# noahares/raxtax

Measured on AMD Instinct MI355X. Metric: classified queries/sec (whole node), higher is better.
Workload: dtype u32 bit-planes + f64

## Files before the change

### include/raxtax_hip.h

```cpp
#ifndef RAXTAX_HIP_H
#define RAXTAX_HIP_H

#include <stddef.h>
#include <stdint.h>

#ifdef __cplusplus
extern "C" {
#endif

#define RTX_ABI_VERSION 6
#define RTX_NUM_KMERS 65536u
#define RTX_MAX_DEPTH 32u

#define RTX_OK 0
#define RTX_ERR_INVALID (-1)
#define RTX_ERR_HIP (-2)
#define RTX_ERR_NO_DEVICE (-3)
#define RTX_ERR_OOM (-4)
#define RTX_ERR_PARSE (-5)
#define RTX_ERR_DEPTH (-6)
#define RTX_ERR_STATE (-7)
#define RTX_ERR_TOO_LONG (-8)
#define RTX_ERR_SENDER (-9)
#define RTX_RETRY_CHUNK 1
// ... 76 lines not shown
                                    uint32_t n_nodes, const uint32_t *node_begin, const uint32_t *node_end,
                                    const uint32_t *node_first_child, const uint32_t *node_n_children,
                                    const uint8_t *node_type, rtx_index **out);
int rtx_index_create_from_tree(int device, const rtx_tree *tree, rtx_index **out);
void rtx_index_destroy(rtx_index *index);
uint64_t rtx_index_num_refs(const rtx_index *index);
uint64_t rtx_index_device_bytes(const rtx_index *index);
uint64_t rtx_index_workspace_bytes(const rtx_index *index);
int rtx_index_workspace_parts(const rtx_index *index, uint64_t out[9]);
int rtx_index_set_batch(rtx_index *index, uint32_t sub_batch);
#define RTX_OPT_SUB_BATCH 1
#define RTX_OPT_PROB_MODE 2
#define RTX_OPT_STAGE_TIMING 6
#define RTX_OPT_DEBUG_TAPS 14
#define RTX_OPT_DEVICE_EXACT 15
#define RTX_OPT_CLUSTER 7
#define RTX_OPT_PACKED_COUNTS 8
#define RTX_OPT_HIT_PAIR 11
#define RTX_OPT_TILE_SKIP 10
#define RTX_OPT_LOCATOR 12
#define RTX_OPT_TILE_PRUNE 13
#define RTX_OPT_FINE_BOUNDS 17
#define RTX_OPT_RECORDS 18
#define RTX_OPT_OVERLAP 19
#define RTX_OPT_MIN_SUB_BATCHES 20
#define RTX_OPT_TWO_LEVEL_BOUNDS 21
#define RTX_OPT_PRUNE_SELF_SAMPLE 22
#define RTX_OPT_RUN_AHEAD 23
#define RTX_OPT_DEVICE_TEXT 24
#define RTX_OPT_STRAND 25
#define RTX_OPT_NEAREST 26
#define RTX_NO_REF 0xFFFFFFFFu
#define RTX_OPT_IDENTITY 28
#define RTX_NO_DIST 0xFFFFFFFFu
#define RTX_IDENTITY_MAX_QUERY 4096u
#define RTX_OPT_DEREP 27
int rtx_index_set_option(rtx_index *index, int option, uint64_t value);

int rtx_index_self_sample(rtx_index *index, const uint8_t *seq_bytes, const uint64_t *seq_off, uint64_t n_refs, uint32_t n_sample, double *live_fraction);
int rtx_index_prune_verdict(const rtx_index *index, int *pruning, double *live_fraction);
int rtx_index_run_ahead_stats(const rtx_index *index, uint64_t *enqueued_ahead, uint64_t *abandoned);
#define RTX_DEFAULT_SEGMENT_CLASSES 1
#define RTX_DEFAULT_EXACT_HASH_MASK 2
#define RTX_DEFAULT_DEREP_HASH_MASK 3
int rtx_set_default_option(int option, uint64_t value);

typedef struct {
    uint32_t n_queries;
    uint64_t n_rows;
    const uint32_t *t;
    const uint8_t *status;
    const double *global_signal;
    const uint64_t *row_begin;
    const uint32_t *row_count;
    const uint32_t *row_lineage;
    const uint32_t *row_node;
    const uint32_t *row_depth;
    const double *row_conf;
    const double *row_local_signal;
    uint32_t row_conf_stride;
    const uint8_t *row_depth_u8;
    const uint8_t *row_conf_hundredths;
} rtx_result_view;

int rtx_batch_prefetch(rtx_index *index, uint64_t n_queries, const uint8_t *bases, const uint64_t *base_off,
                       const uint32_t *exact_ids, const uint64_t *exact_off);
// ... 431 lines not shown
int rtx_shard_prob(rtx_index *index, uint32_t sub_batch_idx);
int rtx_shard_walk(rtx_index *index, uint32_t sub_batch_idx, const double *prefix_global );
int rtx_shard_info(const rtx_index *index, uint64_t *ref_lo, uint64_t *ref_hi, uint32_t *n_bnd_global,
                   uint32_t *n_bnd_local, uint32_t *first_bnd);
int rtx_device_buffer(rtx_index *index, int which, void **device_ptr, uint64_t *row_stride_elems);
#define RTX_BUF_COUNTS 3
#define RTX_BUF_BEST 4
int rtx_shard_buffer(rtx_index *index, uint32_t sub_batch_idx, int which, void **device_ptr, uint64_t *row_stride_elems);
int rtx_shard_rehist(rtx_index *index, uint32_t sub_batch_idx);
int rtx_index_stream(rtx_index *index, void **hip_stream);

#define RTX_STAGE_KMER_EXTRACT 0
#define RTX_STAGE_HIT_COUNT 1
#define RTX_STAGE_PROB_TABLE 2
#define RTX_STAGE_TAXON_PREFIX 3
#define RTX_STAGE_LINEAGE_WALK 4
#define RTX_STAGE_TILE_BOUNDS 5
#define RTX_STAGE_TILE_PRUNE 6
#define RTX_STAGE_EXACT_MATCH 7
#define RTX_STAGE_ORDER 8
#define RTX_STAGE_PAIR_UNION 9
#define RTX_NUM_STAGES 10
int rtx_batch_stage_times(rtx_index *index, float ms[RTX_NUM_STAGES], uint32_t launches[RTX_NUM_STAGES]);
int rtx_batch_work(rtx_index *index, uint64_t *sum_hits, uint64_t *sum_query_bytes,
                   uint64_t *bitmap_bytes_read);
int rtx_batch_work_split(rtx_index *index, uint64_t *live_bytes, uint64_t *bounds_bytes);
int rtx_batch_prob_work(rtx_index *index, uint64_t *sum_grid_points, uint64_t *sum_distinct_counts);

int rtx_debug_kmers(rtx_index *index, uint64_t query, uint16_t *kmers , uint32_t *t);
int rtx_debug_hit_counts(rtx_index *index, uint64_t query, uint16_t *counts );
int rtx_debug_prob_table(rtx_index *index, uint64_t query, double *table_over_z , double *z);
int rtx_debug_probs(rtx_index *index, uint64_t query, double *probs );
int rtx_debug_tile_bounds(rtx_index *index, uint64_t query, uint16_t *tile_ub );
int rtx_debug_order(rtx_index *index, uint32_t *perm );
int rtx_batch_sub_batch(const rtx_index *index, uint32_t *sub_batch, uint32_t *n_sub_batches);
int rtx_batch_last_sub_batch(const rtx_index *index, uint64_t *first, uint32_t *n);
int rtx_batch_classes(const rtx_index *index, uint32_t *n_classes, uint64_t out[20]);
int rtx_debug_prune_stats(rtx_index *index, uint64_t *out );
int rtx_debug_pruned_prob_table(rtx_index *index, uint64_t query, double *table_over_z , double *z, uint32_t *threshold);
int rtx_debug_run_counts(rtx_index *index, uint64_t query, uint16_t *counts , uint8_t *tile_live ,
                         uint32_t *hist , uint32_t *threshold, uint32_t *i1);
int rtx_debug_run_mode(rtx_index *index, uint64_t query, uint32_t *n_segments);
int rtx_debug_prune_detail(rtx_index *index, uint64_t query, uint32_t *out );
int rtx_debug_evaluate(rtx_index *index, const double *probs , rtx_result_view *out);
int rtx_debug_evaluate_mode(rtx_index *index, const double *probs , uint32_t mode, rtx_result_view *out, uint32_t *table_in_lds);
int rtx_debug_ln_factorial(uint32_t n, double *out );
int rtx_debug_prob_hist(rtx_index *index, uint32_t n_q, const uint32_t *t , const uint32_t *hist , uint32_t hstride,
                        uint64_t n_refs, uint32_t kernel, const uint16_t *prune_thr , const uint16_t *prune_i1 ,
                        double *table_over_z , double *z , double *gs , uint8_t *status ,
                        uint32_t *ndist );

int64_t rtx_format_query(const rtx_tree *tree, const rtx_result_view *res, uint64_t q,
                         const char *label, const uint8_t *seq, uint64_t seq_len,
                         const uint32_t *exact_ids, uint64_t n_exact, uint32_t flags, char *out_buf,
                         uint64_t out_cap, char *tsv_buf, uint64_t tsv_cap, int64_t *tsv_len);

int64_t rtx_result_pack(const rtx_result_view *res, uint8_t *buf, uint64_t cap);

#define RTX_NEED_BASE 1024
int64_t rtx_records_format(const rtx_tree *tree, const uint8_t *records, uint64_t n_bytes, const char *const *labels,
                           const uint32_t *exact_one, uint32_t flags, char *out, uint64_t cap, uint64_t *line_off, uint32_t threads);

typedef int (*rtx_sender_fn)(void *ctx, const char *label, const char *out_lines, const char *tsv_lines);
int rtx_raxtax(rtx_index *index, const rtx_tree *tree, uint64_t n_queries, const char *const *labels,
               const uint8_t *bases, const uint64_t *base_off, int skip_exact_matches, int raw_confidence,
               uint64_t chunk_size, rtx_sender_fn sender, void *sender_ctx, int tsv);
// ... 65 lines not shown
```

### raxtax_amd/_lib.py

```python
from __future__ import annotations

import ctypes as C
from pathlib import Path

import numpy as np

PKG = Path(__file__).resolve().parent
import os as _os

LIB_PATH = Path(_os.environ.get("RTX_LIB_PATH") or PKG / "libraxtax_hip.so")

RTX_MAX_DEPTH = 32
RTX_NUM_KMERS = 65536
RTX_OK = 0
RTX_ERR_INVALID, RTX_ERR_HIP, RTX_ERR_NO_DEVICE, RTX_ERR_OOM = -1, -2, -3, -4
RTX_ERR_PARSE, RTX_ERR_DEPTH, RTX_ERR_STATE, RTX_ERR_TOO_LONG = -5, -6, -7, -8
RTX_SKIP_EXACT_MATCHES = 1
RTX_RAW_CONFIDENCE = 2
RTX_TEXT_TSV = 4
RTX_Q_OK, RTX_Q_NO_KMERS, RTX_Q_ALL_KMERS = 0, 1, 2
RTX_OPT_DEREP = 27
RTX_DEFAULT_DEREP_HASH_MASK = 3
RTX_DEFAULT_TALLY_HASH_MASK = 4
RTX_DEFAULT_OTU_HASH_MASK = 5
RTX_DEFAULT_CHIMERA_SLICE = 6
RTX_DEFAULT_UNOISE_SLICE = 8
RTX_UNOISE_MAX_DIFFS = 16
RTX_UNOISE_ZOTU, RTX_UNOISE_ABSORBED, RTX_UNOISE_LEFT, RTX_UNOISE_LONG = 0, 1, 2, 3
RTX_OTU_MAX_LEN = 4096
RTX_LIN_UNCLASSIFIABLE, RTX_LIN_UNCLASSIFIED, RTX_LIN_CLASSIFIED = 0, 1, 2
STAGES = ("kmer_extract", "hit_count", "prob_table", "taxon_prefix", "lineage_walk", "tile_bounds", "tile_prune", "exact_match", "order", "pair_union")

RTX_TRIM_5P, RTX_TRIM_3P = 0, 1
RTX_TRIM_MAX_PATTERNS, RTX_TRIM_MAX_PATTERN, RTX_TRIM_MAX_WINDOW, RTX_TRIM_NO_PATTERN = 8, 64, 256, 0xFF

RTX_DEMUX_MAX_TAGS, RTX_DEMUX_MAX_TAG, RTX_DEMUX_MAX_OFFSET, RTX_DEMUX_MAX_MISMATCHES = 1024, 32, 15, 8
RTX_DEMUX_NO_TAG, RTX_DEMUX_NONE = 0xFFFF, 0xFFFFFFFF
RTX_PROFILE_MAX_SAMPLE_COUNTERS = 1 << 28
RTX_DEMUX_NAMES = ("ok", "no_tag5", "no_tag3", "ambiguous", "unknown_pair")

RTX_QUAL_MAX_READ, RTX_QUAL_TABLE = 1 << 20, 94
RTX_QC_NAMES = ("bad_quality", "short_for_trunc_len", "too_short", "too_long", "too_many_n", "max_ee", "max_ee_rate")

RTX_SCREEN_K, RTX_SCREEN_NONE, RTX_SCREEN_MAX_READ, RTX_SCREEN_MAX_BASES, RTX_SCREEN_CONTAMINANT = 16, 0xFFFFFFFF, 1 << 20, 1 << 26, 1

RTX_MERGE_MAX_READ, RTX_MERGE_MISMATCH_COST = 1024, 5
RTX_MG_NAMES = ("bad_quality", "too_long", "too_short", "no_overlap")

RTX_CHIMERA_MAX_QUERY, RTX_CHIMERA_MAX_SEGMENTS, RTX_CHIMERA_DEFAULT_SEGMENTS, RTX_CHIMERA_DEFAULT_MINDELTA = 4096, 32, 16, 24
RTX_CHIM_OK, RTX_CHIM_NO_KMER, RTX_CHIM_TOO_LONG = 0, 1, 2
RTX_DENOVO_NO_PARENT = 3
RTX_DENOVO_DEFAULT_ABSKEW = 2
RTX_DENOVO_DEFAULT_MAX_PARENTS = 262144
# ... 186 lines not shown
    "rtx_index_num_refs": (C.c_uint64, [C.c_void_p]),
    "rtx_index_device_bytes": (C.c_uint64, [C.c_void_p]),
    "rtx_index_workspace_bytes": (C.c_uint64, [C.c_void_p]),
    "rtx_index_workspace_parts": (C.c_int, [C.c_void_p, u64p]),
    "rtx_index_set_batch": (C.c_int, [C.c_void_p, C.c_uint32]),
    "rtx_set_default_option": (C.c_int, [C.c_int, C.c_uint64]),
    "rtx_index_set_option": (C.c_int, [C.c_void_p, C.c_int, C.c_uint64]),
    "rtx_index_self_sample": (C.c_int, [C.c_void_p, C.c_void_p, C.c_void_p, C.c_uint64, C.c_uint32, C.POINTER(C.c_double)]),
    "rtx_index_prune_verdict": (C.c_int, [C.c_void_p, C.POINTER(C.c_int), C.POINTER(C.c_double)]),
    "rtx_index_run_ahead_stats": (C.c_int, [C.c_void_p, C.POINTER(C.c_uint64), C.POINTER(C.c_uint64)]),
    "rtx_classify_batch": (C.c_int, [C.c_void_p, C.c_uint64, u8p, u64p, u32p, u64p, C.c_uint32,
                                     C.POINTER(ResultView)]),
    "rtx_index_has_exact_lookup": (C.c_int, [C.c_void_p]),
    "rtx_batch_exact_matches": (C.c_int, [C.c_void_p, C.POINTER(u64p), C.POINTER(u32p)]),
    "rtx_batch_upload": (C.c_int, [C.c_void_p, C.c_uint64, u8p, u64p, u32p, u64p]),
    "rtx_batch_run": (C.c_int, [C.c_void_p, C.c_uint32]),
    "rtx_batch_sync": (C.c_int, [C.c_void_p]),
    "rtx_batch_download": (C.c_int, [C.c_void_p, C.POINTER(ResultView)]),
    "rtx_batch_download_then_run": (C.c_int, [C.c_void_p, C.POINTER(ResultView), C.c_uint32]),
    "rtx_index_text_setup": (C.c_int, [C.c_void_p, C.c_void_p, C.c_uint32]),
    "rtx_batch_prefetch_labels": (C.c_int, [C.c_void_p, C.c_uint64, C.POINTER(C.c_char_p)]),
    "rtx_batch_text": (C.c_int, [C.c_void_p, C.POINTER(TextView)]),
    "rtx_batch_stage_times": (C.c_int, [C.c_void_p, f32p, u32p]),
    "rtx_batch_work": (C.c_int, [C.c_void_p, u64p, u64p, u64p]),
    "rtx_batch_prob_work": (C.c_int, [C.c_void_p, u64p, u64p]),
    "rtx_batch_work_split": (C.c_int, [C.c_void_p, u64p, u64p]),
    "rtx_debug_kmers": (C.c_int, [C.c_void_p, C.c_uint64, u16p, u32p]),
    "rtx_debug_hit_counts": (C.c_int, [C.c_void_p, C.c_uint64, u16p]),
    "rtx_debug_prob_table": (C.c_int, [C.c_void_p, C.c_uint64, f64p, f64p]),
    "rtx_debug_pruned_prob_table": (C.c_int, [C.c_void_p, C.c_uint64, f64p, f64p, u32p]),
    "rtx_debug_probs": (C.c_int, [C.c_void_p, C.c_uint64, f64p]),
    "rtx_debug_order": (C.c_int, [C.c_void_p, u32p]),
    "rtx_debug_tile_bounds": (C.c_int, [C.c_void_p, C.c_uint64, u16p]),
    "rtx_debug_prune_stats": (C.c_int, [C.c_void_p, u64p]),
    "rtx_debug_run_counts": (C.c_int, [C.c_void_p, C.c_uint64, u16p, u8p, u32p, u32p, u32p]),
    "rtx_debug_run_mode": (C.c_int, [C.c_void_p, C.c_uint64, u32p]),
    "rtx_batch_last_sub_batch": (C.c_int, [C.c_void_p, u64p, u32p]),
    "rtx_batch_classes": (C.c_int, [C.c_void_p, u32p, u64p]),
    "rtx_debug_prune_detail": (C.c_int, [C.c_void_p, C.c_uint64, u32p]),
    "rtx_debug_evaluate": (C.c_int, [C.c_void_p, f64p, C.POINTER(ResultView)]),
    "rtx_debug_evaluate_mode": (C.c_int, [C.c_void_p, f64p, C.c_uint32, C.POINTER(ResultView), u32p]),
    "rtx_debug_ln_factorial": (C.c_int, [C.c_uint32, f64p]),
    "rtx_debug_prob_hist": (C.c_int, [C.c_void_p, C.c_uint32, u32p, u32p, C.c_uint32, C.c_uint64, C.c_uint32, u16p, u16p, f64p, f64p, f64p, u8p, u32p]),
    "rtx_result_pack": (C.c_int64, [C.POINTER(ResultView), u8p, C.c_uint64]),
    "rtx_records_format": (C.c_int64, [C.c_void_p, u8p, C.c_uint64, C.POINTER(C.c_char_p), u32p, C.c_uint32, C.c_char_p, C.c_uint64, u64p, C.c_uint32]),
    "rtx_format_query": (C.c_int64, [C.c_void_p, C.POINTER(ResultView), C.c_uint64, C.c_char_p, u8p, C.c_uint64,
                                     u32p, C.c_uint64, C.c_uint32, C.c_char_p, C.c_uint64, C.c_char_p, C.c_uint64,
                                     C.POINTER(C.c_int64)]),
    "rtx_raxtax": (C.c_int, None),
    "rtx_raxtax_multi": (C.c_int, None),
    "rtx_raxtax_multi_ex": (C.c_int, None),
    "rtx_batch_strands": (C.c_int, [C.c_void_p, C.POINTER(u8p), C.POINTER(u32p)]),
    "rtx_revcomp": (C.c_int, [u8p, C.c_uint64, u8p]),
    "rtx_raxtax_multi_ex2": (C.c_int, None),
    "rtx_batch_nearest": (C.c_int, [C.c_void_p, C.POINTER(u32p), C.POINTER(u32p)]),
    "rtx_batch_nearest_time": (C.c_int, [C.c_void_p, C.POINTER(C.c_float), C.POINTER(C.c_uint32)]),
    "rtx_raxtax_multi_ex3": (C.c_int, None),
    "rtx_batch_identity": (C.c_int, [C.c_void_p, C.POINTER(u32p), C.POINTER(u32p)]),
    "rtx_batch_identity_time": (C.c_int, [C.c_void_p, C.POINTER(C.c_float), C.POINTER(C.c_uint32)]),
    "rtx_semiglobal_distance": (C.c_int, [u8p, C.c_uint64, u8p, C.c_uint64, C.POINTER(C.c_uint32)]),
    "rtx_index_profile_begin": (C.c_int, [C.c_void_p, C.c_uint32, C.c_uint32]),
    "rtx_index_profile_read": (C.c_int, [C.c_void_p, C.POINTER(ProfileView)]),
    "rtx_index_profile_reset": (C.c_int, [C.c_void_p]),
    "rtx_index_profile_end": (C.c_int, [C.c_void_p]),
    "rtx_index_profile_time": (C.c_int, [C.c_void_p, C.POINTER(C.c_float), C.POINTER(C.c_uint32)]),
    "rtx_profile_merge": (C.c_int, [C.POINTER(C.POINTER(ProfileView)), C.c_uint32, u64p, u64p, u64p, u64p]),
# ... 168 lines not shown
```

### raxtax_amd/api.py

```python
from __future__ import annotations

import ctypes as C
from dataclasses import dataclass
from typing import Callable, List, Optional, Sequence, Tuple

import numpy as np

from . import _lib
from ._lib import (RTX_MAX_DEPTH, RTX_RAW_CONFIDENCE, RTX_SKIP_EXACT_MATCHES, NodesView, ResultView, RtxError, check,
                   f32p, f64p, ptr, u8p, u16p, u32p, u64p)


def _flatten(seqs: Sequence[np.ndarray]) -> Tuple[np.ndarray, np.ndarray]:
    off = np.zeros(len(seqs) + 1, dtype=np.uint64)
    if len(seqs):
        off[1:] = np.cumsum([len(s) for s in seqs], dtype=np.uint64)
    flat = np.zeros(max(int(off[-1]), 1), dtype=np.uint8)
    for i, s in enumerate(seqs):
        flat[int(off[i]):int(off[i + 1])] = np.asarray(s, dtype=np.uint8)
    return flat, off


class Tree:

# ... 263 lines not shown
    check(_lib.load().rtx_sample_profile_merge(arr, len(views), ptr(direct if direct.size else np.zeros(1, np.uint64), u64p), ptr(totals, u64p)))
    return SampleProfile(profiles[0].cutoff, profiles[0].flags, direct, totals)


def sample_table_text(tree: Tree, names: Sequence[str], profile: SampleProfile) -> str:
    lib = _lib.load()
    direct = np.ascontiguousarray(profile.direct, dtype=np.uint64)
    totals = np.ascontiguousarray(profile.totals, dtype=np.uint64)
    if len(names) != direct.shape[0] or totals.shape != (direct.shape[0], 4):
        raise ValueError(f"sample_table_text: {len(names)} names, counters of shape {direct.shape} and {totals.shape}")
    cn = (C.c_char_p * max(len(names), 1))(*[n.encode() for n in names])
    args = [tree._h, len(names), cn, ptr(direct if direct.size else np.zeros(1, np.uint64), u64p), ptr(totals, u64p), int(profile.cutoff)]
    n = check(lib.rtx_sample_table_format(*args, None, 0))
    buf = C.create_string_buffer(max(n, 1))
    check(lib.rtx_sample_table_format(*args, buf, n))
    return buf.raw[:n].decode()


DEFAULT_SEGMENT_CLASSES = 1


class Index:

    identity_on = False
    nearest_on = False

    def __init__(self, tree: Tree, device: int = 0, sub_batch: int = 0, prob_mode: int = 0,
                 stage_timing: bool = False, cluster: Optional[bool] = None, segment_classes=None,
                 packed_counts: Optional[bool] = None,
                 tile_skip: Optional[bool] = None, hit_pair=None, locator: Optional[bool] = None, tile_prune: Optional[bool] = None,
                 debug_taps: bool = False, device_exact: Optional[bool] = None, fine_bounds: Optional[bool] = None,
                 records: Optional[int] = None, overlap: Optional[bool] = None, two_level: Optional[int] = None,
                 prune_self_sample: Optional[bool] = None, device_text: bool = False, strand: str = "plus",
                 nearest: bool = False, derep: bool = False, identity: bool = False, primers=None, quality=None, chimera=None, tags=None, contaminants=None, tally=None):
        self._lib = _lib.load()
        self.tree = tree
        self._tally = None
        if segment_classes is None:
            segment_classes = DEFAULT_SEGMENT_CLASSES
        check(self._lib.rtx_set_default_option(1, int(segment_classes)))
        h = C.c_void_p()
        check(self._lib.rtx_index_create_from_tree(device, tree._h, C.byref(h)))
        self._h = h
        self.n_refs = self._lib.rtx_index_num_refs(self._h)
        if sub_batch:
            check(self._lib.rtx_index_set_batch(self._h, sub_batch))
        if prob_mode:
            check(self._lib.rtx_index_set_option(self._h, 2, prob_mode))
        if stage_timing:
            check(self._lib.rtx_index_set_option(self._h, 6, 1))
        if cluster is not None:
            check(self._lib.rtx_index_set_option(self._h, 7, int(cluster)))
        if packed_counts is not None:
            check(self._lib.rtx_index_set_option(self._h, 8, int(packed_counts)))
        if tile_skip is not None:
            check(self._lib.rtx_index_set_option(self._h, 10, int(tile_skip)))
        if hit_pair is not None:
            check(self._lib.rtx_index_set_option(self._h, 11, int(hit_pair)))
        if locator is not None:
            check(self._lib.rtx_index_set_option(self._h, 12, int(locator)))
        if tile_prune is not None:
            check(self._lib.rtx_index_set_option(self._h, 13, int(tile_prune)))
            if tile_prune and prune_self_sample is None:
                check(self._lib.rtx_index_set_option(self._h, 22, 0))
        if debug_taps:
            check(self._lib.rtx_index_set_option(self._h, 14, 1))
        if device_exact is not None:
# ... 3 lines not shown
        if fine_bounds is not None:
            check(self._lib.rtx_index_set_option(self._h, 17, int(fine_bounds)))
        if records is not None:
            check(self._lib.rtx_index_set_option(self._h, 18, int(records)))
        if overlap is not None:
            check(self._lib.rtx_index_set_option(self._h, 19, int(overlap)))
        if two_level is not None:
            check(self._lib.rtx_index_set_option(self._h, 21, int(two_level)))
        if prune_self_sample is not None:
            check(self._lib.rtx_index_set_option(self._h, 22, int(prune_self_sample)))
        if strand not in ("plus", "both"):
            raise ValueError(f"strand must be 'plus' or 'both', not {strand!r}")
        self.strand = strand
        if strand == "both":
            check(self._lib.rtx_index_set_option(self._h, 25, 1))
        self.nearest_on = bool(nearest) or bool(identity)
        if self.nearest_on:
            check(self._lib.rtx_index_set_option(self._h, 26, 1))
        self.identity_on = bool(identity)
        if identity:
            check(self._lib.rtx_index_set_option(self._h, 28, 1))
        if derep:
            check(self._lib.rtx_index_set_option(self._h, _lib.RTX_OPT_DEREP, 1))
        if primers:
            self.set_primers(primers)
        if tags:
            self.set_tags(*tags)
        if quality is not None:
            self.set_quality(quality)
        if chimera is not None:
            self.set_chimera(ChimeraParams() if chimera is True else chimera)
        if contaminants is not None:
            self.set_screen(*(contaminants if isinstance(contaminants, tuple) else (contaminants,)))
        if tally is not None:
            self.set_tally(tally)
        self._view = ResultView()
        self._keep = None

    def set_tally(self, tally) -> None:
        check(self._lib.rtx_index_set_tally(self._h, tally._h if tally is not None else None))
        self._tally = tally

    @property
    def tally(self):
        return self._tally if self._lib.rtx_index_tally(self._h) else None

    def set_screen(self, sset, params=None) -> None:
        if sset is None:
            check(self._lib.rtx_index_set_screen(self._h, None, None))
        else:
            check(self._lib.rtx_index_set_screen(self._h, sset._h, C.byref((params or ScreenParams())._c())))

    @property
    def screen(self):
        c, on, fp = _lib.ScreenParams(), C.c_int(), C.c_uint64()
        check(self._lib.rtx_index_screen(self._h, C.byref(c), C.byref(on), C.byref(fp)))
        return (ScreenParams(c.min_hits, c.min_pct), int(fp.value)) if on.value else None

    def set_quality(self, params) -> None:
        check(self._lib.rtx_index_set_quality(self._h, C.byref(params._c()) if params is not None else None))

    @property
    def quality(self):
        c, on = _lib.QualParams(), C.c_int()
        check(self._lib.rtx_index_quality(self._h, C.byref(c), C.byref(on)))
        return QualParams._of(c) if on.value else None

    def set_chimera(self, params) -> None:
        check(self._lib.rtx_index_set_chimera(self._h, C.byref(params._c()) if params is not None else None))

# ... 275 lines not shown
        return out

    def debug_prune_detail(self, q: int) -> dict:
        out = np.zeros(72, dtype=np.uint32)
        check(self._lib.rtx_debug_prune_detail(self._h, q, ptr(out, u32p)))
        return dict(block=int(out[0]), M=int(out[1]), threshold=int(out[2]), i1=int(out[3]), largest_bound=int(out[4]), t=int(out[5]),
                    block_counts=out[8:72].copy())

    def debug_probs(self, q: int) -> np.ndarray:
        out = np.zeros(self.n_refs, dtype=np.float64)
        check(self._lib.rtx_debug_probs(self._h, q, ptr(out, f64p)))
        return out

    def sub_batch_size(self) -> int:
        b, n = C.c_uint32(), C.c_uint32()
        check(self._lib.rtx_batch_sub_batch(self._h, C.byref(b), C.byref(n)))
        return int(b.value)

    def last_sub_batch(self):
        first, n = C.c_uint64(), C.c_uint32()
        check(self._lib.rtx_batch_last_sub_batch(self._h, C.byref(first), C.byref(n)))
        return int(first.value), int(n.value)

    def batch_classes(self) -> list:
        n = C.c_uint32()
        out = np.zeros(20, dtype=np.uint64)
        check(self._lib.rtx_batch_classes(self._h, C.byref(n), ptr(out, u64p)))
        res = []
        for c in range(int(n.value)):
            f = int(out[4 * c + 3])
            res.append(dict(queries=int(out[4 * c]), longest=int(out[4 * c + 1]), sub_batch=int(out[4 * c + 2]), planes=f & 0xFF, tables=bool(f >> 8 & 1),
                            pair=bool(f >> 9 & 1), prune=bool(f >> 10 & 1), records=bool(f >> 11 & 1), global_memory_forms=bool(f >> 12 & 1)))
        return res

    def debug_order(self, n_queries: int) -> np.ndarray:
        out = np.zeros(n_queries, dtype=np.uint32)
        check(self._lib.rtx_debug_order(self._h, ptr(out, u32p)))
        return out

    def debug_prune_stats(self) -> dict:
        out = np.zeros(16, dtype=np.uint64)
        check(self._lib.rtx_debug_prune_stats(self._h, ptr(out, u64p)))
        pairs, nq = max(int(out[1]), 1), max(int(out[5]), 1)
        counted = int(out[12]) if int(out[11]) or int(out[12]) else int(out[0])
        return {"live_tiles_per_pair": counted / pairs, "live_tiles_per_pair_first_stage": int(out[0]) / pairs,
                "fine_blocks_per_pair": int(out[11]) / pairs, "fine_cleared_per_query": int(out[10]) / nq, "pairs": int(out[1]), "mean_best_hit_lower_bound": int(out[2]) / nq,
                "mean_threshold": int(out[3]) / nq, "mean_largest_tile_bound": int(out[4]) / nq, "bound_violations": int(out[6]), "live_tiles_per_query": int(out[7]) / nq,
                "tiles_above_threshold_per_query": int(out[8]) / max(int(out[9]), 1), "queries_with_threshold": int(out[9]),
                "record_queries": int(out[14]), "records_per_record_query": int(out[13]) / max(int(out[14]), 1), "record_slow_path_queries": int(out[15])}

    def debug_evaluate(self, probs, mode: int = 0) -> Result:
        probs = np.ascontiguousarray(probs, dtype=np.float64)
        assert len(probs) == self.n_refs
        in_lds = C.c_uint32()
        check(self._lib.rtx_debug_evaluate_mode(self._h, ptr(probs, f64p), mode, C.byref(self._view), C.byref(in_lds)))
        self.last_evaluate_table_in_lds = bool(in_lds.value)
        return Result(self._view)

    def debug_prob_hist(self, ts, hists, n_refs: int, kernel: int, thr=None, i1=None) -> dict:
        ts = np.ascontiguousarray(ts, dtype=np.uint32)
        hists = np.ascontiguousarray(hists, dtype=np.uint32)
        assert hists.ndim == 2 and hists.shape[0] == len(ts)
        n_q, hstride = hists.shape
        tz = np.zeros((n_q, hstride), dtype=np.float64)
        z = np.zeros(n_q, dtype=np.float64)
        gs = np.zeros(n_q, dtype=np.float64)
# ... 1275 lines not shown
```

### raxtax_amd/csrc/rtx_api_batch.hip

```cpp
#include "rtx_index.hpp"

#ifndef RTX_B2_HEAVY_PER_ATILE
#define RTX_B2_HEAVY_PER_ATILE 4u
#endif

namespace rtxi {

int bind(rtx_index *ix) {
    if (!ix) { set_error("null index handle"); return RTX_ERR_INVALID; }
    RTX_HIP(hipSetDevice(ix->device));
    return RTX_OK;
}

int ensure_events(rtx_index *ix, size_t count) {
    while (ix->events.size() < count) {
        hipEvent_t e;
        RTX_HIP(hipEventCreate(&e));
        ix->events.push_back(e);
    }
    return RTX_OK;
}


SubBatch sub_batch_of(rtx_index *ix, uint32_t sb, bool timed) {
// ... 55 lines not shown
    kp.list_len = ix->d_list_len.p;
    kp.row_len = ix->d_row_len.p;
    kp.zero_row = ix->n_rows;
    kp.kmers = sc.d_kmers.p;
    kp.kstride = k.kstride;
    kp.seginfo = ix->d_seginfo.p;
    kp.seg_stride = ix->seg_stride;
    kp.segcls = ix->d_segcls.p;
    kp.cls_stride = ix->cls_stride;
    kp.ntiles = ix->ntiles;
    kp.seg_dbits = ix->d_seg_dbits.p;
    kp.seg_sbits = ix->d_seg_sbits.p;
    kp.seg_sbase = ix->d_seg_sbase.p;
    kp.seg_blocks = ix->seg_blocks;
    kp.rows = sc.d_rows.p;
    kp.rstride = k.rstride;
    kp.dmask = sc.d_dmask.p;
    kp.srows = sc.d_srows.p;
    kp.nsparse = sc.d_nsparse.p;
    kp.t = sc.d_t.p;
    kp.nrows = sc.d_nrows.p;
    kp.hq = r.d_hq.p;
    kp.t_all = r.d_t_all.p;
    kp.nrows_all = r.d_nrows_all.p;
    kp.hist = sc.d_hist.p;
    kp.hstride = k.hstride;
    return kp;
}

static bool run_prunes(const rtx_index *ix, const rtx_index::BatchClass &k) { return k.prune && !ix->dbg_full_run; }
static bool on_records_path(const rtx_index *ix, const rtx_index::BatchClass &k, const rtx_index::Scratch &sc) { return run_prunes(ix, k) && k.rec && sc.d_rec.p != nullptr; }
static bool on_diet(const rtx_index *ix, const rtx_index::BatchClass &k, const rtx_index::Scratch &sc) { return on_records_path(ix, k, sc) && k.diet && sc.d_cnt_row.p != nullptr; }

static RecordRef record_ref(const rtx_index *ix, const rtx_index::Scratch &sc, const rtx_index::ResultSet &r) { return RecordRef{sc.d_rec_nslots.p, sc.d_rec_slots.p, sc.d_rec_cnt.p, sc.d_rec.p, ix->rec_slots(), ix->rec_seg_len, r.d_flags.p}; }
static ProbTables prob_tables(const rtx_index *ix) { return ProbTables{ix->d_tab_cmf.p, ix->d_tab_ratio.p, ix->d_tab_off.p, ix->d_tab_moff.p, ix->d_tab_ilo.p, ix->d_tab_sat.p, ix->tab_tmax}; }

int enqueue_kmer(rtx_index *ix, const SubBatch &b, hipStream_t s) {
    KmerParams kp = kmer_params(ix, b);
    kp.mode = run_prunes(ix, *b.cls) && ix->seg_blocks ? 1u : 0u;
    if (run_prunes(ix, *b.cls)) {
        rtx_index::Scratch &sc = ix->sc[b.set];
        const ItemsLayout items(b.nq, ix->ntiles);
        const FineItemsLayout fine(b.nq, ix->f_ntiles);
        if (sc.d_items.p) { kp.zero[0] = items.count(sc.d_items.p); kp.zero_n[0] = 9u; }
        if (sc.d_fine_items.p) { kp.zero[1] = fine.count(sc.d_fine_items.p); kp.zero_n[1] = 9u + ix->f_ntiles; }
        if (sc.d_cnt_cursor.p) { kp.zero[2] = sc.d_cnt_cursor.p; kp.zero_n[2] = 1u; }
    }
    if (b.timed_all) RTX_HIP(hipEventRecord(stage_event(ix, b, RTX_STAGE_KMER_EXTRACT, 0), s));
    launch_kmer_extract(s, kp, b.nq);
    if (b.timed_all) RTX_HIP(hipEventRecord(stage_event(ix, b, RTX_STAGE_KMER_EXTRACT, 1), s));
    return RTX_OK;
}

static HitParams hit_params(rtx_index *ix, const SubBatch &b, uint32_t flags) {
    rtx_index::Scratch &sc = ix->sc[b.set];
    rtx_index::ResultSet &r = ix->res();
    const rtx_index::BatchClass &k = *b.cls;
    HitParams hp{};
    hp.bitmap = ix->d_bitmap.p;
    hp.stride_bytes = ix->stride_bytes;
    hp.n_rows1 = ix->n_rows + 1;
    hp.n_refs = ix->n_refs;
    hp.ref_base = ix->ref_lo;
    hp.rows = sc.d_rows.p;
    hp.rstride = k.rstride;
    hp.dmask = sc.d_dmask.p;
    hp.nrows = sc.d_nrows.p;
    hp.zero_row = ix->n_rows;
    hp.srows = sc.d_srows.p;
    hp.nsparse = sc.d_nsparse.p;
    hp.segslots = ix->d_segslots.p;
    hp.ntiles = ix->ntiles;
    hp.t = sc.d_t.p;
    hp.counts = sc.d_counts.p;
    hp.counts_lo = ix->packs(k.planes) ? counts_lo(ix, sc) : nullptr;
    hp.counts_hi = ix->packs(k.planes) ? counts_hi(ix, k, sc) : nullptr;
    hp.npad = ix->npad;
    hp.hist = sc.d_hist.p;
    hp.hstride = k.hstride;
    hp.tile_max = sc.d_tilemax.p;
    hp.flags = flags;
    hp.q0 = b.q0;
    hp.perm = r.d_perm.p;
    hp.exact = ExactRef{ix->in[ix->cur_in].d_exact_ids.p, ix->in[ix->cur_in].d_exact_off.p, r.dev_exact ? r.d_exact_grp.p : nullptr, ix->d_em_goff.p, ix->d_em_gids.p};
    hp.nq = b.nq;
    hp.group_rows = k.pair ? ix->d_group_rows.p : nullptr;
    hp.group_base = b.sb * ix->groups_per_sub;
    hp.pair_urec = sc.d_urec.p;
    hp.pair_nu = sc.d_nu.p;
    hp.pair_ustride = 2u * k.rstride;
    return hp;
}

static HitParams bounds_params(const rtx_index *ix, const rtx_index::Scratch &sc, const HitParams &hp) {
    HitParams up = hp;
    up.bitmap = ix->d_ubitmap.p;
    up.stride_bytes = ix->u_stride_bytes;
    up.n_refs = ix->u_nblocks;
    up.dmask = nullptr;
    up.nsparse = nullptr;
    up.ntiles = ix->u_ntiles;
    up.counts = nullptr;
    up.counts_lo = nullptr;
    up.counts_hi = nullptr;
    up.hist = nullptr;
    up.tile_max = nullptr;
    up.bounds_tile_ub = sc.d_tile_ub.p;
    up.bounds_tile_stride = ix->ntiles;
    up.bounds_ntiles = ix->ntiles;
    up.bounds_best = sc.d_best_key.p;
    up.flags = 0;
    up.group_base = hp.group_base + ix->n_groups_run;
    return up;
}

static Bounds2Params bounds2_params(const rtx_index *ix, const rtx_index::Scratch &sc, const HitParams &up, bool heavy) {
    Bounds2Params bp{};
    bp.abitmap = ix->d_abitmap.p;
    bp.bbitmap = ix->d_bbitmap.p;
    bp.n_rows1 = ix->n_rows + 1;
    bp.n_atiles = ix->n_atiles;
    bp.ntiles = ix->ntiles;
    bp.zero_row = ix->n_rows;
    bp.pair_urec = sc.d_urec.p;
    bp.pair_nu = sc.d_nu.p;
    bp.pair_ustride = up.pair_ustride;
    bp.nq = up.nq;
    bp.t = sc.d_t.p;
    bp.tile_ub = sc.d_tile_ub.p;
    bp.tile_ub_stride = ix->ntiles;
    bp.best_key = sc.d_best_key.p;
    bp.delta_ct = ix->b2_delta[0];
    bp.delta_cm = ix->b2_delta[1];
    bp.delta_lo = ix->b2_delta[2];
    bp.delta_hi = ix->b2_delta[3];
    bp.group_rows = up.group_rows;
    bp.group_base = up.group_base;
    bp.heavy = heavy ? sc.d_heavy.p : nullptr;
    bp.heavy_max = std::max<uint32_t>(1u, std::min<uint32_t>(RTX_B2_HEAVY_PER_ATILE * ix->n_atiles, ix->n_btiles / 2u));
    return bp;
}

static PruneParams prune_params(rtx_index *ix, const SubBatch &b, uint32_t flags, int part, const ExactRef &exact) {
    rtx_index::Scratch &sc = ix->sc[b.set];
    const rtx_index::BatchClass &k = *b.cls;
    PruneParams pr{};
    pr.tile_ub = sc.d_tile_ub.p;
    pr.best_key = sc.d_best_key.p;
    pr.tile_ub_stride = ix->ntiles;
    pr.ntiles = ix->ntiles;
    pr.nq = b.nq;
    pr.n_refs = ix->n_refs;
    pr.n_total = ix->n_total;
    pr.ref_base = ix->ref_lo;
    pr.phase = (uint32_t)part;
    pr.best = part ? sc.d_best.p : nullptr;
    pr.bitmap = ix->d_bitmap.p;
    pr.cbitmap = part == 0 && (ix->two_level_used || (k.planes > kBounds2MaxPlanes && ix->two_level_opt && ix->n_refs == ix->n_total)) ? reinterpret_cast<const uint2 *>(ix->d_cbitmap.p) : nullptr;
    pr.n_rows1 = ix->n_rows + 1;
    pr.stride_bytes = ix->stride_bytes;
    pr.rows = sc.d_rows.p;
    pr.rstride = k.rstride;
    pr.nrows = sc.d_nrows.p;
    pr.t = sc.d_t.p;
    pr.flags = flags;
    pr.q0 = b.q0;
    pr.perm = ix->res().d_perm.p;
    pr.exact = exact;
    pr.lnfact = ix->d_lnfact.p;
    pr.inv = ix->d_inv.p;
    pr.nlf = std::min<uint32_t>(kLnFactLen, k.tmax + k.tmax / 2 + 2);
    pr.hist = sc.d_hist.p;
    pr.hstride = k.hstride;
    pr.live = sc.d_live.p;
    pr.live_words = LiveLayout{ix->ntiles}.words();
    pr.pair_live = ItemsLayout(b.nq, ix->ntiles).pair_live(sc.d_items.p);
    pr.thr_out = sc.d_prune_thr.p;
    pr.i1_out = sc.d_prune_i1.p;
    pr.stats = ix->d_prune_stats.p;
    pr.detail = ix->debug_taps && ix->d_prune_detail.n >= (size_t)b.nq * kPruneDetailWords ? ix->d_prune_detail.p : nullptr;
    return pr;
}
// ... 27 lines not shown
    HitParams hp = hit_params(ix, b, flags);
    const bool prune = run_prunes(ix, k);
    if (k.pair && part != 2) {
        if (b.timed_all) RTX_HIP(hipEventRecord(stage_event(ix, b, RTX_STAGE_PAIR_UNION, 0), s));
        launch_pair_union(s, sc.d_rows.p, sc.d_nrows.p, k.rstride, b.nq, sc.d_urec.p, sc.d_nu.p, 2u * k.rstride);
        if (b.timed_all) RTX_HIP(hipEventRecord(stage_event(ix, b, RTX_STAGE_PAIR_UNION, 1), s));
    }
    if (b.timed && !prune) RTX_HIP(hipEventRecord(stage_event(ix, b, RTX_STAGE_HIT_COUNT, 0), s));
    if (part != 0 && !prune) { set_error("internal: a split run without tile pruning"); return RTX_ERR_STATE; }
    if (prune) {
        if (part != 2) {
            const HitParams up = bounds_params(ix, sc, hp);
            if (b.timed) RTX_HIP(hipEventRecord(stage_event(ix, b, RTX_STAGE_TILE_BOUNDS, 0), s));
            ix->two_level_used = part == 0 && ix->two_level_opt && ix->d_abitmap.p && ix->d_bbitmap.p && ix->n_refs == ix->n_total && k.planes <= kBounds2MaxPlanes;
            if (ix->two_level_used) {
                const bool heavy_ok = sc.d_heavy.p && sc.d_heavy_items.p && sc.d_heavy_items.n >= HeavyItemsLayout(b.nq, ix->u_ntiles).total();
                launch_bounds2(s, bounds2_params(ix, sc, up, heavy_ok), b.nq, k.planes, up, ix->u_ntiles, heavy_ok ? sc.d_heavy_items.p : nullptr);
            } else {
                RTX_HIP(hipMemsetAsync(sc.d_best_key.p, 0, (size_t)b.nq * 4, s));
                launch_hit_count_pair_bounds(s, up, b.nq, ix->u_ntiles, k.planes);
            }
            if (b.timed) RTX_HIP(hipEventRecord(stage_event(ix, b, RTX_STAGE_TILE_BOUNDS, 1), s));
        }
        if (s_mid && s_mid != s && part == 0) {
            RTX_HIP(hipEventRecord(ix->ev_mid[b.sb], s));
            RTX_HIP(hipStreamWaitEvent(s_mid, ix->ev_mid[b.sb], 0));
            s = s_mid;
        }
        if (b.timed && part != 1) RTX_HIP(hipEventRecord(stage_event(ix, b, RTX_STAGE_TILE_PRUNE, 0), s));
        PruneParams pr = prune_params(ix, b, flags, part, hp.exact);
        const bool records = part == 0 && on_records_path(ix, k, sc), diet = part == 0 && on_diet(ix, k, sc);
        const RecordRef rr = record_ref(ix, sc, r);
        if (records) { pr.rec = rr; pr.rec_max_slots = rr.stride; }
        if (k.diet && !diet) { set_error("internal: the counts buffer is on its diet without the records path"); return RTX_ERR_STATE; }
        if (diet) {
            pr.cnt_row = sc.d_cnt_row.p;
            pr.cnt_cursor = sc.d_cnt_cursor.p;
            pr.cnt_cap = k.cnt_rows;
            pr.dense_q = sc.d_dense_q.p;
            pr.flags_out = r.d_flags.p;
            hp.cnt_row = sc.d_cnt_row.p;
        }
        launch_prune(s, pr, prob_tables(ix), b.nq);
        if (part == 1) { RTX_HIP(hipGetLastError()); return RTX_OK; }
        if (part == 0 && ix->fine_opt && ix->d_fbitmap.p && k.pair && sc.d_fine_items.p) {
            const FineItemsLayout fine(b.nq, ix->f_ntiles);
            uint32_t *const fi = sc.d_fine_items.p;
            launch_fine_bounds(s, fine_params(ix, sc, hp), b.nq, ix->f_ntiles, pr.pair_live, fine.cursors(fi), fine.items(fi), fine.count(fi), k.planes);
        }
        RTX_HIP(hipMemsetAsync(sc.d_tilemax.p, 0, (size_t)b.nq * ix->ntiles * 2, s));
        hp.live = sc.d_live.p;
        hp.live_words = pr.live_words;
        hp.prune_thr = sc.d_prune_thr.p;
        if (records) hp.rec = rr;
        if (k.pair) {
            const ItemsLayout items(b.nq, ix->ntiles);
            launch_live_items(s, sc.d_live.p, pr.live_words, b.nq, ix->ntiles, items.items(sc.d_items.p), items.count(sc.d_items.p),
                              ix->d_prune_stats.p ? ix->d_prune_stats.p + 2 * kPruneStatCopies * 8 : nullptr);
            hp.items = items.items(sc.d_items.p);
            hp.n_items = items.count(sc.d_items.p);
        }
        if (ix->seg_blocks) {
            KmerParams kp = kmer_params(ix, b);
            kp.mode = 2u;
            kp.live = sc.d_live.p;
            kp.live_words = pr.live_words;
            launch_kmer_extract(s, kp, b.nq);
        }
        if (b.timed) {
            RTX_HIP(hipEventRecord(stage_event(ix, b, RTX_STAGE_TILE_PRUNE, 1), s));
            RTX_HIP(hipEventRecord(stage_event(ix, b, RTX_STAGE_HIT_COUNT, 0), s));
        }
    }
    if (k.pair) launch_hit_count_pair(s, hp, b.nq, ix->ntiles, k.planes);
    else launch_hit_count(s, hp, b.nq, ix->ntiles, k.planes);
    if (b.timed) RTX_HIP(hipEventRecord(stage_event(ix, b, RTX_STAGE_HIT_COUNT, 1), s));
    ix->hit_stream = s;
    return RTX_OK;
}

int enqueue_count(rtx_index *ix, const SubBatch &b, uint32_t flags, hipStream_t s_mid) {
    int rc = enqueue_kmer(ix, b, b.s);
    return rc ? rc : enqueue_hit(ix, b, flags, b.s, 0, s_mid);
}

static WalkParams walk_params(rtx_index *ix, const SubBatch &b, const double *prefix);
static int reset_sub_alloc(rtx_index *ix, hipStream_t s);
// ... 782 lines not shown
        for (uint32_t c = 0; c < ix->n_cls; c++) any_side = any_side || ix->cls[c].side;
        if (any_side) { if ((rc = alloc_scratch_set(ix, kSideSet))) return rc; }
        else ix->sc[kSideSet].release_all();
    }
    for (uint32_t k = 1; k <= 2u; k++) {
        if (k < n_sets && ix->n_sub_total() > 1) {
            if (alloc_scratch_set(ix, k)) ix->sc[k].d_kmers.release();
        } else if (ix->n_refs == ix->n_total) {
            ix->sc[k].release_all();
        }
    }
    return RTX_OK;
}

int alloc_scratch_set(rtx_index *ix, uint32_t k) {
    int rc;
    rtx_index::Scratch &sc = ix->sc[k];
    const ScratchNeed n = scratch_set_need(ix, k);
    if ((rc = sc.d_kmers.alloc(n.kmers)) || (rc = sc.d_rows.alloc(n.rows)) || (rc = sc.d_dmask.alloc(n.dmask)) || (rc = sc.d_nsparse.alloc(n.nsparse)) || (rc = sc.d_srows.alloc(n.srows)) ||
        (rc = sc.d_t.alloc(n.t)) || (rc = sc.d_nrows.alloc(n.nrows)) || (rc = sc.d_counts.alloc(n.counts)) || (rc = sc.d_hist.alloc(n.hist)) || (rc = sc.d_table_z.alloc(n.hist)) ||
        (rc = sc.d_prefix.alloc(n.prefix)) || (rc = sc.d_order.alloc(n.order)) || (rc = sc.d_tilemax.alloc(n.tilemax)) || (rc = sc.d_urec.alloc(n.urec)) || (rc = sc.d_nu.alloc(n.nu)))
        return rc;
    if (n.prob_scratch && (rc = ix->d_prob_scratch.alloc(std::max(n.prob_scratch, ix->d_prob_scratch.n)))) return rc;
    if (ix->pruning() && ix->d_ubitmap.p && (ix->n_refs == ix->n_total || ix->shard_prune_opt)) {
        if ((rc = sc.d_tile_ub.alloc(n.tile_ub)) || (rc = sc.d_best_key.alloc(n.best_key)) || (rc = sc.d_prune_thr.alloc(n.prune_thr)) || (rc = sc.d_prune_i1.alloc(n.prune_i1)) ||
            (rc = sc.d_best.alloc(n.best)) || (rc = sc.d_live.alloc(n.live)) || (rc = sc.d_items.alloc(n.items)))
            return rc;
        if (ix->d_abitmap.p && (sc.d_heavy.alloc(n.heavy) || sc.d_heavy_items.alloc(n.heavy_items))) { sc.d_heavy.release(); sc.d_heavy_items.release(); }
        if (ix->d_fbitmap.p && sc.d_fine_items.alloc(n.fine_items)) sc.d_fine_items.release();
        if (ix->rec_opt && ix->n_refs == ix->n_total) {
            if (sc.d_rec_nslots.alloc(n.rec_nslots) || sc.d_rec_slots.alloc(n.rec_slots) || sc.d_rec_cnt.alloc(n.rec_cnt) ||
                sc.d_rec.alloc(n.rec) || sc.d_cnt_row.alloc(n.cnt_row) || sc.d_cnt_cursor.alloc(n.cnt_cursor) || sc.d_dense_q.alloc(n.dense_q))
                sc.d_rec.release();
        }
    }
    return RTX_OK;
}

}

extern "C" {

int rtx_batch_prefetch(rtx_index *ix, uint64_t n_queries, const uint8_t *bases, const uint64_t *base_off,
                       const uint32_t *exact_ids, const uint64_t *exact_off) {
    int rc = bind(ix);
    if (rc) return rc;
    rtx_index::Inputs &in = ix->in[ix->cur_in ^ 1u];
    const bool with_labels = in.labels_pending && in.n_labels == n_queries;
    in.labels_pending = in.has_labels = false;
    const bool with_weights = in.weights_pending && in.n_weights == n_queries;
    in.weights_pending = in.has_weights = false;
    const bool with_samples = in.samples_pending && in.n_samples == n_queries;
    in.samples_pending = in.has_samples = false;
    if (n_queries == 0 || !base_off || (!bases && base_off[n_queries])) {
        set_error("rtx_batch_upload: invalid argument");
        return RTX_ERR_INVALID;
    }
    const bool both = ix->strand_opt != 0u;
    if (both) {
        if (exact_off || exact_ids) { set_error("RTX_OPT_STRAND: exact-match ids cannot be passed in (those of the reverse complements must come from the same lookup: pass NULL)"); return RTX_ERR_INVALID; }
        if (!rtx_index_has_exact_lookup(ix) || ix->n_refs != ix->n_total) { set_error("RTX_OPT_STRAND needs the exact-match lookup of the device (a handle built from the reference sequences, RTX_OPT_DEVICE_EXACT on)"); return RTX_ERR_STATE; }
        if (n_queries > 0x7FFFFFFFull) { set_error("RTX_OPT_STRAND: too many queries in one batch"); return RTX_ERR_INVALID; }
    }
    const uint64_t n_dev = both ? 2 * n_queries : n_queries;
    if (!ix->h2d_stream) RTX_HIP(hipStreamCreateWithFlags(&ix->h2d_stream, hipStreamNonBlocking));
    if (!in.ready) RTX_HIP(hipEventCreateWithFlags(&in.ready, hipEventDisableTiming));
// ... 130 lines not shown
```

### raxtax_amd/csrc/rtx_api_debug.hip

```cpp
#include "rtx_index.hpp"

extern "C" {

int rtx_batch_stage_times(rtx_index *ix, float ms[RTX_NUM_STAGES], uint32_t launches[RTX_NUM_STAGES]) {
    int rc = bind(ix);
    if (rc) return rc;
    if (!ix->synced) { set_error("rtx_batch_stage_times: batch not synchronised"); return RTX_ERR_STATE; }
    for (int s = 0; s < RTX_NUM_STAGES; s++) { ms[s] = 0.f; launches[s] = 0; }
    for (uint32_t sb = 0; sb < ix->n_sub_last; sb++) {
        const rtx_index::BatchClass &kc = ix->cls[ix->plan[sb].cls];
        for (int s = 0; s < RTX_NUM_STAGES; s++) {
            if (s == RTX_STAGE_EXACT_MATCH) {
                if (sb != 0 || !ix->dev_exact_used || !ix->stage_timing) continue;
            } else if (s == RTX_STAGE_ORDER) {
                if (sb != 0 || !ix->stage_timing) continue;
            } else if (s == RTX_STAGE_PAIR_UNION) {
                if (!kc.pair || !ix->stage_timing) continue;
            } else if (s == RTX_STAGE_TILE_BOUNDS || s == RTX_STAGE_TILE_PRUNE ? !kc.prune : (s != RTX_STAGE_HIT_COUNT && !ix->stage_timing)) continue;
            float t = 0.f;
            RTX_HIP(hipEventElapsedTime(&t, ix->events[((size_t)sb * RTX_NUM_STAGES + s) * 2],
                                        ix->events[((size_t)sb * RTX_NUM_STAGES + s) * 2 + 1]));
            ms[s] += t;
            launches[s]++;
        }
// ... 296 lines not shown
int rtx_debug_run_mode(rtx_index *ix, uint64_t query, uint32_t *n_segments) {
    uint32_t slot;
    int rc = debug_slot_as_run(ix, query, &slot);
    if (rc) return rc;
    if (!n_segments) { set_error("null argument"); return RTX_ERR_INVALID; }
    uint16_t n_seg = 0;
    rtx_index::Scratch &sc = ix->sc[ix->last_set];
    if (ix->last_cls().prune && ix->last_cls().rec && sc.d_rec_nslots.p) RTX_HIP(hipMemcpy(&n_seg, sc.d_rec_nslots.p + slot, 2, hipMemcpyDeviceToHost));
    *n_segments = n_seg;
    return RTX_OK;
}

int rtx_debug_prune_detail(rtx_index *ix, uint64_t query, uint32_t *out) {
    uint32_t slot;
    int rc = debug_slot_as_run(ix, query, &slot);
    if (rc) return rc;
    if (!out) { set_error("null argument"); return RTX_ERR_INVALID; }
    if (!ix->last_cls().prune || !ix->debug_taps || ix->d_prune_detail.n < (size_t)(slot + 1) * kPruneDetailWords) {
        set_error("rtx_debug_prune_detail: the last run did not prune, or RTX_OPT_DEBUG_TAPS was off");
        return RTX_ERR_STATE;
    }
    RTX_HIP(hipMemcpy(out, ix->d_prune_detail.p + (size_t)slot * kPruneDetailWords, kPruneDetailWords * 4, hipMemcpyDeviceToHost));
    return RTX_OK;
}

int rtx_debug_tile_bounds(rtx_index *ix, uint64_t query, uint16_t *tile_ub) {
    uint32_t slot;
    int rc = debug_slot_as_run(ix, query, &slot);
    if (rc) return rc;
    if (!tile_ub) { set_error("null argument"); return RTX_ERR_INVALID; }
    rtx_index::Scratch &sc = ix->sc[ix->last_set];
    if (!ix->last_cls().prune || sc.d_tile_ub.n < (size_t)(slot + 1) * ix->ntiles) { set_error("rtx_debug_tile_bounds: the last run did not prune"); return RTX_ERR_STATE; }
    RTX_HIP(hipMemcpy(tile_ub, sc.d_tile_ub.p + (size_t)slot * ix->ntiles, (size_t)ix->ntiles * 2, hipMemcpyDeviceToHost));
    return RTX_OK;
}

int rtx_debug_prune_stats(rtx_index *ix, uint64_t *out) {
    if (!ix || !out) { set_error("null argument"); return RTX_ERR_INVALID; }
    std::memset(out, 0, 128);
    if (!ix->any_prune || !ix->d_prune_stats.p) return RTX_OK;
    RTX_HIP(hipStreamSynchronize(ix->stream));
    unsigned long long h[kPruneStatCopies * 32];
    RTX_HIP(hipMemcpy(h, ix->d_prune_stats.p, sizeof(h), hipMemcpyDeviceToHost));
    for (uint32_t c = 0; c < kPruneStatCopies; c++) {
        for (uint32_t k = 0; k < 8; k++) out[k] += h[c * 8 + k];
        for (uint32_t k = 0; k < 2; k++) out[8 + k] += h[(kPruneStatCopies + c) * 8 + k];
        for (uint32_t k = 0; k < 3; k++) out[10 + k] += h[(2 * kPruneStatCopies + c) * 8 + k];
        out[13] += h[(3 * kPruneStatCopies + c) * 8 + 0];
        out[14] += h[(3 * kPruneStatCopies + c) * 8 + 1];
        out[15] += h[(3 * kPruneStatCopies + c) * 8 + 3];
    }
    return RTX_OK;
}

int rtx_batch_sub_batch(const rtx_index *ix, uint32_t *sub_batch, uint32_t *n_sub) {
    if (!ix) { set_error("null index handle"); return RTX_ERR_INVALID; }
    if (!ix->uploaded || ix->n_cls == 0 || ix->cls[ix->n_cls - 1].sub_batch == 0) { set_error("rtx_batch_sub_batch: no batch has been uploaded"); return RTX_ERR_STATE; }
    if (sub_batch) *sub_batch = ix->cls[ix->n_cls - 1].sub_batch;
    if (n_sub) *n_sub = ix->n_sub_total();
    return RTX_OK;
}

int rtx_batch_last_sub_batch(const rtx_index *ix, uint64_t *first, uint32_t *n) {
    if (!ix) { set_error("null index handle"); return RTX_ERR_INVALID; }
    if (!ix->uploaded) { set_error("rtx_batch_last_sub_batch: no batch has been uploaded"); return RTX_ERR_STATE; }
    if (first) *first = ix->plan.back().q0;
// ... 229 lines not shown
```

### raxtax_amd/csrc/rtx_api_index.hip

```cpp
#include "rtx_stage.hpp"

namespace rtx {
int index_device(const rtx_index *index) { return index ? index->device : -1; }
void index_set_shared_device(rtx_index *index, bool shared) { if (index) index->shared_device = shared; }
uint32_t index_swap_min_subs(rtx_index *index, uint32_t v) { if (!index) return 0; const uint32_t old = index->min_subs; index->min_subs = v; return old; }
bool index_strand(const rtx_index *index) { return index && index->strand_opt != 0u; }
bool index_nearest(const rtx_index *index) { return index && index->nearest_opt != 0u; }
bool index_identity(const rtx_index *index) { return index && index->identity_opt != 0u; }
bool index_profile(const rtx_index *index, uint32_t *cutoff_hundredths, uint32_t *flags) {
    if (!index || !index->prof.on) return false;
    if (cutoff_hundredths) *cutoff_hundredths = index->prof.cutoff;
    if (flags) *flags = index->prof.flags;
    return true;
}
bool index_device_text(const rtx_index *index) { return index && index->device_text_opt != 0u; }
bool index_derep(const rtx_index *index) { return index && index->derep_opt != 0u; }
uint32_t index_swap_run_ahead(rtx_index *index, uint32_t v) {
    if (!index) return 0;
    const uint32_t old = index->run_ahead_opt;
    (void)rtx_index_set_option(index, RTX_OPT_RUN_AHEAD, v);
    return old;
}
}

// ... 119 lines not shown
        auto up = [&](void *d, const void *h, size_t bytes) { if (e == hipSuccess) e = hipMemcpy(d, h, bytes, hipMemcpyHostToDevice); };
        up(ix->d_noderec.p, noderec.data(), (size_t)n_nodes * sizeof(uint4));
        up(ix->d_bnd_bits.p, bits.data(), nchunk);
        up(ix->d_bnd_rank.p, rank.data(), nchunk * 4);
        if (e != hipSuccess) { set_error("taxonomy upload failed: %s", hipGetErrorString(e)); return fail(RTX_ERR_HIP); }
    }
    {
        std::vector<double> lf;
        fill_ln_factorial(lf);
        if ((rc = ix->d_lnfact.alloc(lf.size()))) return fail(rc);
        if (hipMemcpy(ix->d_lnfact.p, lf.data(), lf.size() * 8, hipMemcpyHostToDevice) != hipSuccess) {
            set_error("lnfact upload failed");
            return fail(RTX_ERR_HIP);
        }
        std::vector<double> inv(lf.size(), 0.0);
        for (size_t x = 1; x < inv.size(); x++) inv[x] = 1.0 / (double)x;
        if ((rc = ix->d_inv.alloc(inv.size()))) return fail(rc);
        if (hipMemcpy(ix->d_inv.p, inv.data(), inv.size() * 8, hipMemcpyHostToDevice) != hipSuccess) {
            set_error("reciprocal table upload failed");
            return fail(RTX_ERR_HIP);
        }
    }
    ix->stride_bytes = (uint32_t)align_up((n_refs + 7) / 8, 1024);
    ix->npad = (uint64_t)ix->stride_bytes * 8;
    ix->ntiles = (ix->stride_bytes + 1023) / 1024;
    if ((rc = ix->res().d_cursor.alloc(2)) || (rc = ix->res().d_flags.alloc(1))) return fail(rc);
    *out = ix;
    return RTX_OK;
}

static bool prepare_union_bitmap(rtx_index *ix);
static bool prepare_fine_bitmap(rtx_index *ix);
static void build_two_level(rtx_index *ix);

static uint64_t g_em_hash_mask = ~0ull;
static uint64_t em_hash_bytes(const uint8_t *s, uint64_t len) {
    uint64_t sum = 0;
    for (uint64_t j = 0; j * 8 < len; j++) {
        uint64_t w = 0;
        std::memcpy(&w, s + 8 * j, (size_t)std::min<uint64_t>(8, len - 8 * j));
        sum += em_mix_word(w, j);
    }
    return em_finish(sum, len);
}
static void build_exact_table(rtx_index *ix, const uint8_t *seq_bytes, const uint64_t *seq_off,
                              std::vector<const std::vector<uint32_t> *> &groups) {
    if (ix->n_refs != ix->n_total || groups.empty()) return;
    std::sort(groups.begin(), groups.end(), [](const std::vector<uint32_t> *a, const std::vector<uint32_t> *b) { return (*a)[0] < (*b)[0]; });
    const uint32_t G = (uint32_t)groups.size();
    uint32_t bits = 4;
    while ((1ull << bits) < 2ull * G) bits++;
    std::vector<uint64_t> rep_off(G + 1, 0);
    std::vector<uint32_t> goff(G + 1, 0), gids;
    gids.reserve(ix->n_total);
    for (uint32_t g = 0; g < G; g++) {
        const uint32_t rep = (*groups[g])[0];
        rep_off[g + 1] = rep_off[g] + (seq_off[rep + 1] - seq_off[rep]);
        gids.insert(gids.end(), groups[g]->begin(), groups[g]->end());
        goff[g + 1] = (uint32_t)gids.size();
    }
    std::vector<uint8_t> rep_bytes(rep_off[G] + 16, 0);
    std::vector<uint64_t> hashes(G);
    {
        const unsigned nt = rtx::host_threads(8u);
        std::vector<std::thread> th;
        for (unsigned k = 0; k < nt; k++)
// ... 173 lines not shown
        ix->n_rows = nr;
        const size_t words = (size_t)(nr + 1) * (ix->stride_bytes / 4);
        const uint64_t total = offsets[RTX_NUM_KMERS];
        DevBuf<uint64_t> d_off;
        DevBuf<uint32_t> d_post;
        if ((rc = ix->d_bitmap.alloc(words)) || (rc = ix->d_row_of.alloc(RTX_NUM_KMERS)) ||
            (rc = ix->d_list_len.alloc(RTX_NUM_KMERS)) || (rc = d_off.alloc(RTX_NUM_KMERS + 1)) ||
            (rc = d_post.alloc(total)))
            return fail(rc);
        hipError_t e = hipMemset(ix->d_bitmap.p, 0, words * 4);
        if (e == hipSuccess) e = hipMemcpy(ix->d_row_of.p, row_of.data(), RTX_NUM_KMERS * 4, hipMemcpyHostToDevice);
        if (e == hipSuccess) e = hipMemcpy(ix->d_list_len.p, list_len.data(), RTX_NUM_KMERS * 4, hipMemcpyHostToDevice);
        if (e == hipSuccess) e = hipMemcpy(d_off.p, offsets, (RTX_NUM_KMERS + 1) * 8, hipMemcpyHostToDevice);
        if (e == hipSuccess && total) e = hipMemcpy(d_post.p, postings, total * 4, hipMemcpyHostToDevice);
        if (e == hipSuccess) {
            launch_bitmap_build(ix->stream, d_off.p, d_post.p, ix->d_row_of.p, ix->d_bitmap.p, ix->stride_bytes / 4, nr + 1,
                                (uint32_t)ref_lo, (uint32_t)ref_hi);
            e = hipStreamSynchronize(ix->stream);
        }
        if (e != hipSuccess) { set_error("bitmap build failed: %s", hipGetErrorString(e)); return fail(RTX_ERR_HIP); }
        if (prepare_union_bitmap(ix)) {
            launch_bitmap_build(ix->stream, d_off.p, d_post.p, ix->d_row_of.p, ix->d_ubitmap.p, ix->u_stride_bytes / 4, nr + 1, (uint32_t)ref_lo,
                                (uint32_t)ref_hi, kPruneShift);
            if (hipStreamSynchronize(ix->stream) != hipSuccess) { (void)hipGetLastError(); ix->d_ubitmap.release(); }
            build_two_level(ix);
        }
        if (prepare_fine_bitmap(ix)) {
            launch_bitmap_build(ix->stream, d_off.p, d_post.p, ix->d_row_of.p, ix->d_fbitmap.p, ix->f_stride_bytes / 4, nr + 1, (uint32_t)ref_lo,
                                (uint32_t)ref_hi, kFineShift);
            if (hipStreamSynchronize(ix->stream) != hipSuccess) { (void)hipGetLastError(); ix->d_fbitmap.release(); }
        }
    }
    if ((rc = build_segments(ix))) return fail(rc);
    *out = ix;
    return RTX_OK;
}

static bool prepare_union_bitmap(rtx_index *ix) {
    if (ix->ntiles < RTX_PRUNE_MIN_TILES) return false;
    ix->u_nblocks = (ix->n_refs + (1ull << kPruneShift) - 1) >> kPruneShift;
    if (ix->u_nblocks > 0xFFFFFull) return false;
    ix->u_ntiles = (uint32_t)((ix->u_nblocks + 8191) / 8192);
    ix->u_stride_bytes = ix->u_ntiles * 1024u;
    const size_t words = (size_t)(ix->n_rows + 1) * (ix->u_stride_bytes / 4);
    if (ix->d_ubitmap.alloc(words)) { ix->d_ubitmap.release(); return false; }
    if (hipMemsetAsync(ix->d_ubitmap.p, 0, words * 4, ix->stream) != hipSuccess) { (void)hipGetLastError(); ix->d_ubitmap.release(); return false; }
    return true;
}

static bool prepare_fine_bitmap(rtx_index *ix) {
    if (!ix->d_ubitmap.p || ix->ntiles < kFineMinTiles || ix->n_refs != ix->n_total) return false;
    ix->f_nblocks = (ix->n_refs + (1ull << kFineShift) - 1) >> kFineShift;
    ix->f_ntiles = (uint32_t)((ix->f_nblocks + 8191) / 8192);
    ix->f_stride_bytes = ix->f_ntiles * 1024u;
    const size_t words = (size_t)(ix->n_rows + 1) * (ix->f_stride_bytes / 4);
    if (ix->d_fbitmap.alloc(words)) { ix->d_fbitmap.release(); return false; }
    if (hipMemsetAsync(ix->d_fbitmap.p, 0, words * 4, ix->stream) != hipSuccess) { (void)hipGetLastError(); ix->d_fbitmap.release(); return false; }
    return true;
}

static void build_two_level(rtx_index *ix) {
    if (!ix->d_ubitmap.p || ix->n_refs != ix->n_total || ix->ntiles < kTwoLevelMinTiles) return;
    static_assert(kPruneShift == 6, "level B of the two-level bounds pass holds the blocks of the union bitmap");
    ix->n_btiles = (uint32_t)((ix->u_nblocks + 511) / 512);
    ix->n_atiles = (uint32_t)((ix->u_nblocks + 8191) / 8192);
    const size_t rows1 = (size_t)ix->n_rows + 1;
    if (rows1 * 256u > 0xFFFFFFFFull) return;
    if ((uint64_t)ix->u_ntiles * rows1 * 256u > 0xFFFFFFFFull) return;
    if ((size_t)ix->n_atiles * 256u + 32768u > 160u * 1024u) { ix->n_atiles = ix->n_btiles = 0; return; }
    if (ix->d_abitmap.alloc((size_t)ix->n_atiles * rows1 * 64) || ix->d_bbitmap.alloc((size_t)ix->n_btiles * rows1 * 64)) {
        ix->d_abitmap.release();
        ix->d_bbitmap.release();
        return;
    }
    hipError_t e = hipMemsetAsync(ix->d_abitmap.p, 0, (size_t)ix->n_atiles * rows1 * 256, ix->stream);
    if (e == hipSuccess) e = hipMemsetAsync(ix->d_bbitmap.p, 0, (size_t)ix->n_btiles * rows1 * 64, ix->stream);
    if (e == hipSuccess) {
        launch_bounds2_build(ix->stream, ix->d_ubitmap.p, (uint32_t)rows1, ix->u_ntiles, ix->d_bbitmap.p, ix->d_abitmap.p);
        e = hipGetLastError();
        if (e == hipSuccess) e = hipStreamSynchronize(ix->stream);
    }
    if (e != hipSuccess) { (void)hipGetLastError(); ix->d_abitmap.release(); ix->d_bbitmap.release(); return; }
    const size_t cbytes = (size_t)((ix->n_refs + 63) / 64) * rows1 * 8;
    size_t free_b = 0, total_b = 0;
    if (hipMemGetInfo(&free_b, &total_b) != hipSuccess || cbytes > free_b / 4 || cbytes > total_b / 16 || ix->d_cbitmap.alloc(cbytes)) {
        (void)hipGetLastError();
        ix->d_cbitmap.release();
        return;
    }
    e = hipMemsetAsync(ix->d_cbitmap.p, 0, cbytes, ix->stream);
    if (e == hipSuccess) {
        launch_block_major_build(ix->stream, ix->d_bitmap.p, (uint32_t)rows1, ix->ntiles, ix->stride_bytes, ix->d_cbitmap.p);
        e = hipGetLastError();
        if (e == hipSuccess) e = hipStreamSynchronize(ix->stream);
    }
    if (e != hipSuccess) { (void)hipGetLastError(); ix->d_cbitmap.release(); }
}

static void build_locator(rtx_index *ix, const uint8_t *d_seq, const uint64_t *d_off, uint64_t n_refs) {
    if (ix->n_refs != ix->n_total || n_refs < 256) return;
    DevBuf<uint32_t> d_cnt;
    if (ix->d_loc_table.alloc(kLocTableEntries) || d_cnt.alloc(kLocTableEntries)) { ix->d_loc_table.release(); return; }
    hipError_t e = hipMemsetAsync(ix->d_loc_table.p, 0xFF, (size_t)kLocTableEntries * 4, ix->stream);
    if (e == hipSuccess) e = hipMemsetAsync(d_cnt.p, 0, (size_t)kLocTableEntries * 4, ix->stream);
    if (e == hipSuccess) {
        launch_loc_mark(ix->stream, d_seq, d_off, n_refs, ix->d_loc_table.p, d_cnt.p);
        launch_loc_finish(ix->stream, ix->d_loc_table.p, d_cnt.p);
        e = hipStreamSynchronize(ix->stream);
    }
    if (e != hipSuccess) { (void)hipGetLastError(); ix->d_loc_table.release(); }
}

static thread_local bool g_from_tree = false;

int rtx_index_create_from_sequences(int device, uint64_t n_refs, const uint8_t *seq_bytes, const uint64_t *seq_off,
                                    uint32_t n_nodes, const uint32_t *node_begin, const uint32_t *node_end,
                                    const uint32_t *node_first_child, const uint32_t *node_n_children,
                                    const uint8_t *node_type, rtx_index **out) {
    if (!seq_off || (!seq_bytes && n_refs && seq_off[n_refs])) { set_error("rtx_index_create_from_sequences: null sequences"); return RTX_ERR_INVALID; }
    rtx_index *ix = nullptr;
    int rc = create_common(device, n_refs, 0, n_refs, nullptr, 0, n_nodes, node_begin, node_end, node_first_child,
                           node_n_children, node_type, &ix);
    if (rc) return rc;
    auto fail = [&](int code) { delete ix; return code; };
    const uint64_t total = seq_off[n_refs] - seq_off[0];
    DevBuf<uint8_t> d_seq;
    DevBuf<uint64_t> d_off;
    DevBuf<uint32_t> d_present;
    if ((rc = d_seq.alloc(total + 16)) || (rc = d_off.alloc(n_refs + 1)) || (rc = d_present.alloc(2048)) ||
// ... 7 lines not shown
    if (e == hipSuccess) {
        launch_ref_kmer_mark(ix->stream, d_seq.p, d_off.p, n_refs, d_present.p);
        e = hipStreamSynchronize(ix->stream);
    }
    std::vector<uint32_t> present(2048, 0), row_of(RTX_NUM_KMERS, kEmptyRow);
    if (e == hipSuccess) e = hipMemcpy(present.data(), d_present.p, 2048 * 4, hipMemcpyDeviceToHost);
    if (e != hipSuccess) { set_error("k-mer marking failed: %s", hipGetErrorString(e)); return fail(RTX_ERR_HIP); }
    uint32_t nr = 0;
    for (uint32_t k = 0; k < RTX_NUM_KMERS; k++)
        if (present[k >> 5] & (1u << (k & 31u))) row_of[k] = nr++;
    ix->n_rows = nr;
    const size_t words = (size_t)(nr + 1) * (ix->stride_bytes / 4);
    if ((rc = ix->d_bitmap.alloc(words))) return fail(rc);
    e = hipMemset(ix->d_bitmap.p, 0, words * 4);
    if (e == hipSuccess) e = hipMemcpy(ix->d_row_of.p, row_of.data(), RTX_NUM_KMERS * 4, hipMemcpyHostToDevice);
    if (e == hipSuccess) {
        launch_ref_bitmap_set(ix->stream, d_seq.p, d_off.p, n_refs, ix->d_row_of.p, ix->d_bitmap.p, ix->stride_bytes / 4, nr + 1);
        launch_row_popcount(ix->stream, ix->d_row_of.p, ix->d_bitmap.p, ix->stride_bytes / 4, nr + 1, ix->d_list_len.p);
        e = hipStreamSynchronize(ix->stream);
    }
    if (e != hipSuccess) { set_error("bitmap build from sequences failed: %s", hipGetErrorString(e)); return fail(RTX_ERR_HIP); }
    if ((rc = build_segments(ix))) return fail(rc);
    build_locator(ix, d_seq.p, d_off.p, n_refs);
    if (!g_from_tree) build_exact_table_from_sequences(ix, n_refs, seq_bytes, seq_off);
    if (prepare_union_bitmap(ix)) {
        launch_ref_bitmap_set(ix->stream, d_seq.p, d_off.p, n_refs, ix->d_row_of.p, ix->d_ubitmap.p, ix->u_stride_bytes / 4, nr + 1, kPruneShift);
        if (hipStreamSynchronize(ix->stream) != hipSuccess) { (void)hipGetLastError(); ix->d_ubitmap.release(); }
        build_two_level(ix);
    }
    if (prepare_fine_bitmap(ix)) {
        launch_ref_bitmap_set(ix->stream, d_seq.p, d_off.p, n_refs, ix->d_row_of.p, ix->d_fbitmap.p, ix->f_stride_bytes / 4, nr + 1, kFineShift);
        if (hipStreamSynchronize(ix->stream) != hipSuccess) { (void)hipGetLastError(); ix->d_fbitmap.release(); }
    }
    *out = ix;
    if (!g_from_tree) (void)rtx_index_self_sample(ix, seq_bytes, seq_off, n_refs, 0, nullptr);
    return RTX_OK;
}

static void exact_table_from_tree(rtx_index *ix, const rtx_tree *tree) {
    if (tree->seq_off.size() != tree->num_tips + 1) return;
    std::vector<const std::vector<uint32_t> *> groups;
    groups.reserve(tree->sequences.size());
    for (const auto &kv : tree->sequences)
        if (!kv.second.empty()) groups.push_back(&kv.second);
    build_exact_table(ix, tree->seq_bytes.data(), tree->seq_off.data(), groups);
}

int rtx_index_create_from_tree(int device, const rtx_tree *tree, rtx_index **out) {
    if (!tree || !out) { set_error("null argument"); return RTX_ERR_INVALID; }
    const FlatNodes &f = tree->flat;
    if (tree->csr_off.empty()) {
        g_from_tree = true;
        const int rc = rtx_index_create_from_sequences(device, tree->num_tips, tree->seq_bytes.data(), tree->seq_off.data(), f.size(),
                                                       f.begin.data(), f.end.data(), f.first_child.data(), f.n_children.data(),
                                                       f.type.data(), out);
        g_from_tree = false;
        if (rc == RTX_OK) {
            exact_table_from_tree(*out, tree);
            (void)rtx_index_self_sample(*out, tree->seq_bytes.data(), tree->seq_off.data(), tree->num_tips, 0, nullptr);
        }
        return rc;
    }
    int rc = rtx_index_create(device, tree->num_tips, tree->csr_off.data(), tree->postings.data(), f.size(), f.begin.data(),
                              f.end.data(), f.first_child.data(), f.n_children.data(), f.type.data(), out);
    if (rc != RTX_OK) return rc;
    exact_table_from_tree(*out, tree);
// ... 44 lines not shown
    ix->debug_taps = taps_was;
    ix->uploaded = ix->ran = ix->synced = false;
    if (rc != RTX_OK) return RTX_OK;
    if (st[5] != 0) {
        ix->self_live = (double)st[7] / ((double)st[5] * (double)ix->ntiles);
        ix->prune_pays = ix->self_live < kSelfSampleOff;
    }
    if (live_fraction) *live_fraction = ix->self_live;
    return RTX_OK;
}
int rtx_index_prune_verdict(const rtx_index *ix, int *pruning, double *live_fraction) {
    if (!ix) { set_error("null index handle"); return RTX_ERR_INVALID; }
    if (pruning) *pruning = ix->pruning() ? 1 : 0;
    if (live_fraction) *live_fraction = ix->self_live;
    return RTX_OK;
}

int rtx_index_run_ahead_stats(const rtx_index *ix, uint64_t *enqueued_ahead, uint64_t *abandoned) {
    if (!ix) { set_error("null index handle"); return RTX_ERR_INVALID; }
    if (enqueued_ahead) *enqueued_ahead = ix->n_run_ahead;
    if (abandoned) *abandoned = ix->n_run_ahead_retry;
    return RTX_OK;
}

void rtx_index_destroy(rtx_index *index) {
    if (!index) return;
    (void)hipSetDevice(index->device);
    delete index;
}

uint64_t rtx_index_num_refs(const rtx_index *index) { return index ? index->n_total : 0; }
uint64_t rtx_index_device_bytes(const rtx_index *index) {
    if (!index) return 0;
    return index->d_seg_dbits.n * 8 + index->d_seg_sbits.n * 8 + index->d_seg_sbase.n * 4 + index->d_seginfo.n * 4 + index->d_segcls.n * 4 + index->d_segslots.n * 2 + index->d_bitmap.n * 4 + index->d_row_of.n * 4 + index->d_row_len.n * 8 + index->d_list_len.n * 4 + index->d_loc_table.n * 4 + index->d_ubitmap.n * 4 + index->d_fbitmap.n * 4 + index->d_abitmap.n * 4 + index->d_bbitmap.n + index->d_cbitmap.n + index->d_em_table.n * 8 + index->d_em_rep_off.n * 8 + index->d_em_rep_bytes.n + index->d_em_goff.n * 4 + index->d_em_gids.n * 4 + index->d_lnfact.n * 8 +
           index->d_noderec.n * 16 + index->d_bnd_bits.n + index->d_bnd_rank.n * 4;
}
uint64_t rtx_index_workspace_bytes(const rtx_index *ix) {
    if (!ix) return 0;
    uint64_t b = (ix->d_tab_cmf.n + ix->d_tab_ratio.n) * 8 + ix->d_tab_off.n * 8 + ix->d_tab_moff.n * 4 + (ix->d_tab_ilo.n + ix->d_tab_sat.n) * 2 + ix->d_node_depth.n + ix->d_node_sig0.n + ix->d_node_begin.n * 4 + ix->d_node_eb.n * 8;
    for (const auto &sc : ix->sc) b += sc.bytes();
    for (const auto &in : ix->in) b += in.d_packed.n + (in.d_base_off.n + in.d_exact_off.n) * 8 + in.d_exact_ids.n * 4;
    b += ix->d_bases.n + ix->d_prob_scratch.n * 8 + (ix->d_skey_in.n + ix->d_skey_out.n) * 8 + ix->d_sidx.n * 4 + ix->d_sort_tmp.n + ix->d_group_rows.n * 4;
    for (const auto &r : ix->rs) {
        const rtx_index::ResultSet::Bytes s = r.bytes();
        b += s.order + s.groups + s.rest;
    }
    return b;
}
int rtx_index_workspace_parts(const rtx_index *ix, uint64_t out[9]) {
    if (!ix || !out) { set_error("null argument"); return RTX_ERR_INVALID; }
    for (int i = 0; i < 9; i++) out[i] = 0;
    out[0] = (ix->d_tab_cmf.n + ix->d_tab_ratio.n) * 8 + ix->d_tab_off.n * 8 + ix->d_tab_moff.n * 4 + (ix->d_tab_ilo.n + ix->d_tab_sat.n) * 2;
    for (const auto &sc : ix->sc) {
        if (!sc.d_kmers.p) continue;
        out[8]++;
        out[1] += sc.d_counts.bytes();
        out[2] += sc.d_rec.bytes() + sc.d_rec_cnt.bytes() + sc.d_rec_nslots.bytes() + sc.d_rec_slots.bytes();
        out[3] += sc.d_prefix.bytes();
        out[4] += sc.d_dmask.bytes() + sc.d_srows.bytes() + sc.d_nsparse.bytes();
    }
    out[6] = ix->d_bases.n + (ix->d_skey_in.n + ix->d_skey_out.n) * 8 + ix->d_sidx.n * 4 + ix->d_sort_tmp.n;
    for (const auto &in : ix->in) out[6] += in.d_packed.n + (in.d_base_off.n + in.d_exact_off.n) * 8 + in.d_exact_ids.n * 4;
    for (const auto &r : ix->rs) {
        const rtx_index::ResultSet::Bytes s = r.bytes();
        out[6] += s.order;
        out[7] += s.rest;
    }
// ... 92 lines not shown
            index->uploaded = index->ran = index->synced = false;
            index->in[0].staged = index->in[1].staged = false;
            index->ws_valid = false;
            index->strand_opt = (uint32_t)value;
            return RTX_OK;
        case RTX_OPT_NEAREST:
            if (value > 1) break;
            if (value && index->n_refs != index->n_total) { set_error("RTX_OPT_NEAREST: not on a reference-shard handle (the peak of a query is spread over the shards)"); return RTX_ERR_INVALID; }
            if (!value && index->identity_opt) { set_error("RTX_OPT_NEAREST cannot be switched off while RTX_OPT_IDENTITY is on"); return RTX_ERR_STATE; }
            index->uploaded = index->ran = index->synced = false;
            index->in[0].staged = index->in[1].staged = false;
            index->ws_valid = false;
            index->nearest_opt = (uint32_t)value;
            return RTX_OK;
        case RTX_OPT_IDENTITY:
            if (value > 1) break;
            if (value && index->n_refs != index->n_total) { set_error("RTX_OPT_IDENTITY: not on a reference-shard handle"); return RTX_ERR_INVALID; }
            if (value && !index->nearest_opt) { set_error("RTX_OPT_IDENTITY needs RTX_OPT_NEAREST (the reference a query is aligned to)"); return RTX_ERR_STATE; }
            if (value && (!index->d_em_rep_bytes.p || !index->d_em_goff.p || !index->em_groups)) { set_error("RTX_OPT_IDENTITY needs the reference sequences on the device (a handle built from a tree or from sequences)"); return RTX_ERR_STATE; }
            if (value && !index->d_em_ref_grp.p) {
                int rc = bind(index);
                if (rc) return rc;
                if ((rc = index->d_em_ref_grp.alloc(index->n_refs))) return rc;
                RTX_HIP(hipMemsetAsync(index->d_em_ref_grp.p, 0, index->n_refs * 4, index->stream));
                rtx::launch_ref_group(index->stream, index->d_em_goff.p, index->d_em_gids.p, index->em_groups, (uint32_t)index->n_refs, index->d_em_ref_grp.p);
                RTX_HIP(hipGetLastError());
                RTX_HIP(hipStreamSynchronize(index->stream));
            }
            index->uploaded = index->ran = index->synced = false;
            index->in[0].staged = index->in[1].staged = false;
            index->ws_valid = false;
            index->identity_opt = (uint32_t)value;
            return RTX_OK;
        case RTX_OPT_TWO_LEVEL_BOUNDS:
            index->two_level_opt = value ? 1u : 0u;
            if (value > 1) {
                index->b2_delta[0] = (uint32_t)(value & 0xFFFFu);
                index->b2_delta[1] = (uint32_t)((value >> 16) & 0xFFFFu);
                index->b2_delta[2] = (uint32_t)((value >> 32) & 0xFFFFu);
                index->b2_delta[3] = (uint32_t)((value >> 48) & 0xFFFFu);
            }
            return RTX_OK;
        case RTX_OPT_MIN_SUB_BATCHES:
            if (value < 1 || value > 64) break;
            index->uploaded = index->ran = index->synced = false;
            index->min_subs = (uint32_t)value;
            return RTX_OK;
        case RTX_OPT_OVERLAP:
            index->uploaded = index->ran = index->synced = false;
            if (value > 2) break;
            index->overlap_opt = (uint32_t)value;
            return RTX_OK;
        case RTX_OPT_RECORDS:
            if (value > kRecMaxSlots) break;
            index->uploaded = index->ran = index->synced = false;
            index->rec_opt = (uint32_t)value;
            return RTX_OK;
        case RTX_OPT_PROB_MODE:
            if (value > 2) break;
            index->prob_mode = (int)value;
            return RTX_OK;
        default: break;
    }
    set_error("rtx_index_set_option: unknown option %d / value %llu", option, (unsigned long long)value);
    return RTX_ERR_INVALID;
}
// ... 3 lines not shown
```

### raxtax_amd/csrc/rtx_bounds2.hip

```cpp
#include <hip/hip_runtime.h>

#include <algorithm>
#include <type_traits>

#include "rtx_hit_common.hpp"

namespace rtx {

constexpr uint32_t kB2Pad = 256u;
constexpr uint32_t b2_cap(int planes) { return planes > 10 ? 2048u : 1024u; }
constexpr uint32_t b2_lds_dw(int planes) { return 3u * b2_cap(planes); }

template <int SHIFT>
__device__ __forceinline__ void load_unit(uint4 (&buf)[8], __amdgpu_buffer_rsrc_t rsrc, const uint32_t *unit, uint32_t grp, uint32_t col) {
    const uint4 i0 = reinterpret_cast<const uint4 *>(unit)[grp * 2u], i1 = reinterpret_cast<const uint4 *>(unit)[grp * 2u + 1u];
    const uint32_t id[8] = {i0.x, i0.y, i0.z, i0.w, i1.x, i1.y, i1.z, i1.w};
#pragma unroll
    for (int j = 0; j < 8; j++) {
        const u32x4_t v = __builtin_amdgcn_raw_buffer_load_b128(rsrc, (id[j] << SHIFT) + col, 0, 0);
        buf[j] = make_uint4(v.x, v.y, v.z, v.w);
    }
}

template <int NP, int MODE, int R, int NB, int SHIFT>
__device__ __forceinline__ void fold_list(uint32_t (&pa)[4][NP], uint32_t (&pb)[4][NP], uint4 (&buf)[4][8], const uint32_t *list, uint32_t ng,
                                          const uint32_t *next, uint32_t grp, uint32_t col, __amdgpu_buffer_rsrc_t rsrc) {
    constexpr uint32_t kUnit = 8u * (uint32_t)R, kGroup = kUnit * (uint32_t)NB;
    auto group = [&](auto load_tag, const uint32_t *src) {
        constexpr bool kLoad = decltype(load_tag)::value;
        uint4 c[NB];
#pragma unroll
        for (int b = 0; b < NB; b++) {
            c[b] = MODE == 1 ? tree8<NP>(pa, buf[b]) : tree8<NP>(pb, buf[b]);
            if constexpr (kLoad) load_unit<SHIFT>(buf[b], rsrc, src + (uint32_t)b * kUnit, grp, col);
        }
        if (MODE == 1) {
            if constexpr (NB == 4) ripple4<NP, 5>(pa, csa_plane<NP, 4>(pa, csa_plane<NP, 3>(pa, c[0], c[1]), csa_plane<NP, 3>(pa, c[2], c[3])));
            else ripple4<NP, 4>(pa, csa_plane<NP, 3>(pa, c[0], c[1]));
        } else {
            if constexpr (NB == 4) ripple4<NP, 5>(pb, csa_plane<NP, 4>(pb, csa_plane<NP, 3>(pb, c[0], c[1]), csa_plane<NP, 3>(pb, c[2], c[3])));
            else ripple4<NP, 4>(pb, csa_plane<NP, 3>(pb, c[0], c[1]));
        }
    };
    const uint32_t n_loop = next ? ng : ng - 1u;
    for (uint32_t g = 0; g < n_loop; g++) group(std::true_type{}, g + 1 < ng ? list + (g + 1) * kGroup : next);
    if (!next) group(std::false_type{}, nullptr);
}

template <int NP>
__device__ __forceinline__ void reduce_rows(const uint32_t (&pl)[4][NP], uint32_t lane, uint32_t (&out)[NP]) {
    const bool hi = (lane & 32u) != 0u, mid = (lane & 16u) != 0u;
    uint32_t k0[NP], k1[NP];
    {
        uint32_t s0[NP], s1[NP];
#pragma unroll
        for (int p = 0; p < NP; p++) {
            k0[p] = hi ? pl[2][p] : pl[0][p];
            k1[p] = hi ? pl[3][p] : pl[1][p];
            s0[p] = (uint32_t)__shfl_xor((int)(hi ? pl[0][p] : pl[2][p]), 32, 64);
            s1[p] = (uint32_t)__shfl_xor((int)(hi ? pl[1][p] : pl[3][p]), 32, 64);
        }
        planes_add<NP>(k0, s0);
        planes_add<NP>(k1, s1);
    }
    uint32_t s[NP];
#pragma unroll
    for (int p = 0; p < NP; p++) {
        out[p] = mid ? k1[p] : k0[p];
        s[p] = (uint32_t)__shfl_xor((int)(mid ? k0[p] : k1[p]), 16, 64);
    }
    planes_add<NP>(out, s);
}

__device__ __forceinline__ uint32_t umax(uint32_t a, uint32_t b) { return a > b ? a : b; }

template <int NP>
__global__ __launch_bounds__(64, 2) void bounds2_kernel(Bounds2Params p) {
    extern __shared__ uint32_t b2_lds[];
    const uint32_t lane = threadIdx.x;
    const uint32_t np8 = gridDim.x >> 3;
    const uint32_t pair = blockIdx.x < np8 * 8u ? (blockIdx.x & 7u) * np8 + (blockIdx.x >> 3) : blockIdx.x;
    const uint32_t qa = pair * 2u, qb = qa + 1u;
    const bool has_b = qb < p.nq;
    constexpr uint32_t kB2Cap = b2_cap(NP);
    uint32_t *l_both = b2_lds, *l_a = b2_lds + kB2Cap, *l_b = b2_lds + 2u * kB2Cap;
    uint16_t *l_keep = reinterpret_cast<uint16_t *>(b2_lds + b2_lds_dw(NP));

    const uint2 *urec = p.pair_urec + (size_t)pair * p.pair_ustride;
    const uint32_t n_u = std::min<uint32_t>(p.pair_nu[pair], p.pair_ustride);
    const unsigned long long lt_mask = (1ull << lane) - 1ull;
    uint32_t n_both = 0, n_a = 0, n_b = 0;
    for (uint32_t u0 = 0; u0 < n_u; u0 += 512u) {
        uint2 rec[8];
#pragma unroll
        for (int c = 0; c < 8; c++) {
            const uint32_t i = u0 + (uint32_t)c * 64u + lane;
            rec[c] = urec[i < p.pair_ustride ? i : p.pair_ustride - 1u];
        }
#pragma unroll
        for (int c = 0; c < 8; c++) {
            const uint32_t i = u0 + (uint32_t)c * 64u + lane;
            const bool in = i < n_u;
            const bool ia = in && (rec[c].x & (1u << 30)), ib = in && (rec[c].x & (1u << 31)) && has_b;
            const uint32_t row = rec[c].x & 0x3FFFFFFFu;
            const bool sh = ia && ib, oa = ia && !ib, ob = ib && !ia;
            const unsigned long long bs = __ballot(sh), ba = __ballot(oa), bo = __ballot(ob);
            const uint32_t ps = n_both + (uint32_t)__popcll(bs & lt_mask), pa_ = n_a + (uint32_t)__popcll(ba & lt_mask), pb_ = n_b + (uint32_t)__popcll(bo & lt_mask);
// ... 29 lines not shown
        const uint32_t g_both = (n_both + kGroup - 1u) / kGroup, g_a = need_a ? (n_a + kGroup - 1u) / kGroup : 0u, g_b = need_b ? (n_b + kGroup - 1u) / kGroup : 0u;
        const uint32_t *first = g_both ? l_both : (g_a ? l_a : (g_b ? l_b : nullptr));
        if (!first) return;
#pragma unroll
        for (int b = 0; b < NB; b++) load_unit<SHIFT>(buf[b], rsrc, first + (uint32_t)b * 8u * (uint32_t)R, grp, col);
        const uint32_t *after_a = g_b ? l_b : nullptr, *after_both = g_a ? l_a : after_a;
        if (g_both) {
            fold_list<NP, 1, R, NB, SHIFT>(pa, pb, buf, l_both, g_both, after_both, grp, col, rsrc);
#pragma unroll
            for (int w = 0; w < 4; w++)
#pragma unroll
                for (int b = 0; b < NP; b++) pb[w][b] = pa[w][b];
        }
        if (g_a) fold_list<NP, 1, R, NB, SHIFT>(pa, pb, buf, l_a, g_a, after_a, grp, col, rsrc);
        if (g_b) fold_list<NP, 2, R, NB, SHIFT>(pa, pb, buf, l_b, g_b, nullptr, grp, col, rsrc);
        n_instr += (g_both + g_a + g_b) * 8u * (uint32_t)NB;
    };

    uint32_t best_a = 0xFFFFFu, best_b = 0xFFFFFu;
    const uint32_t row4 = lane >> 4;
    uint32_t max_a = 0, max_b = 0;
    for (uint32_t at = 0; at < p.n_atiles; at++) {
        const char *base = reinterpret_cast<const char *>(p.abitmap) + (size_t)at * p.n_rows1 * 256u;
        const __amdgpu_buffer_rsrc_t rsrc = __builtin_amdgcn_make_buffer_rsrc(const_cast<char *>(base), 0, p.n_rows1 * 256u, 0x00027000);
        fold_level(std::integral_constant<int, 4>{}, std::integral_constant<int, 4>{}, std::integral_constant<int, 8>{}, rsrc, row4, (lane & 15u) * 16u, true, has_b);
        uint32_t ra[NP], rb[NP], cand;
        reduce_rows<NP>(pa, lane, ra);
        reduce_rows<NP>(pb, lane, rb);
        const uint32_t T = at * 64u + (lane & 15u) * 4u + row4;
        const uint32_t ma = planes_max<NP>(ra, cand), mb = planes_max<NP>(rb, cand);
        if (T < p.ntiles) {
            tub_a[T] = (uint16_t)ma;
            if (has_b) tub_b[T] = (uint16_t)mb;
        }
        max_a = umax(max_a, ma);
        max_b = umax(max_b, mb);
        l_keep[at * 128u + lane] = (uint16_t)ma;
        l_keep[at * 128u + 64u + lane] = (uint16_t)mb;
    }
    max_a = wave_max_u32(max_a);
    max_b = wave_max_u32(max_b);
    wave_lds_sync();
    auto delta_of = [&](uint32_t t, uint32_t mx) -> uint32_t {
        const uint32_t up = p.delta_ct * t, dn = p.delta_cm * mx;
        const uint32_t d = up > dn ? (up - dn) >> 8 : 0u, lo = (p.delta_lo * t) >> 8, hi = (p.delta_hi * t) >> 8;
        return d < lo ? lo : (d > hi ? hi : d);
    };
    const uint32_t dl_a = umax(delta_of(t_a, max_a), 1u), dl_b = umax(delta_of(t_b, max_b), 1u);

    const uint32_t sub4 = lane & 3u, grp16 = lane >> 2;
    auto wanted = [&](uint32_t at, uint32_t &mask_a, uint32_t &mask_b) {
        uint32_t ma = l_keep[at * 128u + lane], mb = l_keep[at * 128u + 64u + lane];
        ma = umax(ma, (uint32_t)__shfl_xor((int)ma, 16, 64));
        ma = umax(ma, (uint32_t)__shfl_xor((int)ma, 32, 64));
        mb = umax(mb, (uint32_t)__shfl_xor((int)mb, 16, 64));
        mb = umax(mb, (uint32_t)__shfl_xor((int)mb, 32, 64));
        mask_a = (uint32_t)(__ballot(ma + dl_a > max_a && ma != 0u && lane < 16u) & 0xFFFFull);
        mask_b = has_b ? (uint32_t)(__ballot(mb + dl_b > max_b && mb != 0u && lane < 16u) & 0xFFFFull) : 0u;
    };
    bool heavy_a = false, heavy_b = false;
    if (p.heavy) {
        uint32_t na = 0, nb = 0;
        for (uint32_t at = 0; at < p.n_atiles; at++) {
            uint32_t mask_a, mask_b;
            wanted(at, mask_a, mask_b);
            na += (uint32_t)__popc(mask_a);
            nb += (uint32_t)__popc(mask_b);
        }
        heavy_a = na > p.heavy_max;
        heavy_b = nb > p.heavy_max;
        if (lane == 0u) {
            p.heavy[qa] = heavy_a ? 1u : 0u;
            if (has_b) p.heavy[qb] = heavy_b ? 1u : 0u;
        }
    }
    for (uint32_t at = 0; at < p.n_atiles; at++) {
        uint32_t mask_a, mask_b;
        wanted(at, mask_a, mask_b);
        mask_a = heavy_a ? 0u : mask_a;
        mask_b = heavy_b ? 0u : mask_b;
        uint32_t todo = mask_a | mask_b;
        while (todo) {
            const uint32_t s = (uint32_t)__builtin_ctz(todo);
            todo &= todo - 1u;
            const uint32_t bt = at * 16u + s;
            if (bt * 4u >= p.ntiles) break;
            const bool for_a = (mask_a >> s) & 1u, for_b = (mask_b >> s) & 1u;
            const char *base = reinterpret_cast<const char *>(p.bbitmap) + (size_t)bt * p.n_rows1 * 64u;
            const __amdgpu_buffer_rsrc_t rsrc = __builtin_amdgcn_make_buffer_rsrc(const_cast<char *>(base), 0, p.n_rows1 * 64u, 0x00027000);
            fold_level(std::integral_constant<int, 16>{}, std::integral_constant<int, 2>{}, std::integral_constant<int, 6>{}, rsrc, grp16, sub4 * 16u, for_a, for_b);
            const uint32_t T = bt * 4u + sub4;
            const bool real = T < p.ntiles;
            auto finish = [&](const uint32_t (&pl)[4][NP], uint16_t *tub, uint32_t &best) {
                uint32_t r[NP];
                reduce_rows<NP>(pl, lane, r);
#pragma unroll
                for (int k = 0; k < 2; k++) {
                    uint32_t sh[NP];
#pragma unroll
                    for (int pp = 0; pp < NP; pp++)
                        sh[pp] = k == 0 ? (uint32_t)__builtin_amdgcn_update_dpp(0, (int)r[pp], 0x124, 0xF, 0xF, true)
                                        : (uint32_t)__builtin_amdgcn_update_dpp(0, (int)r[pp], 0x128, 0xF, 0xF, true);
                    planes_add<NP>(r, sh);
                }
                uint32_t c;
                const uint32_t w = planes_max<NP>(r, c);
                uint32_t key = (w << 8) | (127u - (row4 * 32u + (uint32_t)__builtin_ctz(c)));
                key = umax(key, (uint32_t)__shfl_xor((int)key, 16, 64));
                key = umax(key, (uint32_t)__shfl_xor((int)key, 32, 64));
                if (real && lane < 4u) tub[T] = (uint16_t)(key >> 8);
                const uint32_t g = real ? ((key >> 8) << 20) | (0xFFFFFu - (T * 128u + (127u - (key & 0xFFu)))) : 0u;
                best = umax(best, wave_max_u32(g));
            };
            if (for_a) finish(pa, tub_a, best_a);
            if (for_b) finish(pb, tub_b, best_b);
        }
    }
    if (lane == 0u) {
        p.best_key[qa] = heavy_a ? 0u : best_a;
        if (has_b) p.best_key[qb] = heavy_b ? 0u : best_b;
        if (p.group_rows) atomicAdd(&p.group_rows[p.group_base + pair], n_instr);
    }
}

__global__ __launch_bounds__(1024) void heavy_items_kernel(const uint8_t *__restrict__ heavy, uint32_t nq, uint32_t u_ntiles, uint32_t *__restrict__ items,
                                                           uint32_t *__restrict__ n_items) {
    __shared__ uint32_t wsum[2][16];
    const uint32_t tid = threadIdx.x, lane = tid & 63u, wave = tid >> 6, np = (nq + 1u) / 2u;
    constexpr uint32_t kPer = 32;
    uint32_t carry = 0, buf = 0;
    for (uint32_t base = 0; base < np; base += 1024u * kPer, buf ^= 1u) {
        const uint32_t p0 = base + tid * kPer;
        uint32_t bits = 0;
        if (p0 < np) {
            if (p0 + kPer <= np && 2u * (p0 + kPer) <= nq) {
                const uint4 *f = reinterpret_cast<const uint4 *>(heavy + (size_t)p0 * 2u);
                const uint4 v[4] = {f[0], f[1], f[2], f[3]};
#pragma unroll
                for (int k = 0; k < 4; k++) {
                    const uint32_t w[4] = {v[k].x, v[k].y, v[k].z, v[k].w};
#pragma unroll
                    for (int j = 0; j < 4; j++) {
                        if (w[j] & 0x0000FFFFu) bits |= 1u << (k * 8 + j * 2);
                        if (w[j] & 0xFFFF0000u) bits |= 1u << (k * 8 + j * 2 + 1);
                    }
                }
            } else {
                for (uint32_t j = 0; j < kPer && p0 + j < np; j++) {
// ... 74 lines not shown
```

### raxtax_amd/csrc/rtx_emul.cpp

```cpp
#include <algorithm>
#include <cmath>
#include <cstdint>
#include <cstring>
#include <array>
#include <vector>

#include "rtx_math.hpp"

using namespace rtx;

template <int NP>
static void emul_fold(uint32_t (&pl)[NP], const uint32_t *rows, uint32_t n_rows, int sched) {
    auto t8 = [&](const uint32_t *r) { return planes_tree8<NP>(pl, r[0], r[1], r[2], r[3], r[4], r[5], r[6], r[7]); };
    uint32_t r = 0;
    if (sched == 24) {
        std::vector<uint32_t> padded(rows, rows + n_rows);
        padded.resize((n_rows + 23u) / 24u * 24u, 0u);
        for (; r + 24 <= padded.size(); r += 24) {
            const uint32_t c3a = t8(&padded[r]), c3b = t8(&padded[r + 8]), c3c = t8(&padded[r + 16]);
            uint32_t c4a, c5;
            csa(pl[3], c3a, c3b, pl[3], c4a);
            const uint32_t c4b = pl[3] & c3c;
            pl[3] ^= c3c;
            csa(pl[4], c4a, c4b, pl[4], c5);
// ... 536 lines not shown
        };
        uint32_t lo2 = u_max, hi2 = h_min - 1u;
        while (lo2 < hi2) {
            const uint32_t mid = (lo2 + hi2 + 1u) >> 1;
            if (crit(mid)) lo2 = mid; else hi2 = mid - 1u;
        }
        u_max = lo2;
    }
    *u_out = u_max;
    *i1_out = u_max ? i1 : 0u;
}

void emul_prune_threshold(uint32_t t, uint64_t n_refs, const uint32_t *hm_in, const double *lf, uint32_t tab_tmax, uint32_t *u_out,
                          uint32_t *i1_out) {
    emul_prune_threshold_x(t, n_refs, hm_in, lf, tab_tmax, 0, nullptr, nullptr, u_out, i1_out);
}
void emul_prune_threshold_tiles(uint32_t t, uint64_t n_refs, const uint32_t *hm_in, const double *lf, uint32_t tab_tmax, uint32_t ntiles,
                                const uint16_t *tile_ub, uint32_t *u_out, uint32_t *i1_out) {
    const uint32_t per = (ntiles + 63u) / 64u, ng = (ntiles + per - 1u) / per;
    std::vector<uint32_t> gub(ng, 0);
    std::vector<uint64_t> gn(ng, 0);
    for (uint32_t T = 0; T < ntiles; T++) {
        const uint32_t g = T / per;
        gub[g] = std::max<uint32_t>(gub[g], tile_ub[T]);
        const uint64_t lo = (uint64_t)T * 8192u, hi = std::min<uint64_t>(lo + 8192u, n_refs);
        gn[g] += hi > lo ? hi - lo : 0u;
    }
    emul_prune_threshold_x(t, n_refs, hm_in, lf, tab_tmax, ng, gub.data(), gn.data(), u_out, i1_out);
}

void emul_ref_slot(uint32_t r, uint32_t stride_bytes, uint32_t *word, uint32_t *bit) { ref_slot(r, stride_bytes, *word, *bit); }
uint32_t emul_slot_ref(uint32_t tile, uint32_t lane, uint32_t g, uint32_t j, uint32_t stride_bytes) {
    return tile * 8192u + (g * tile_lanes(stride_bytes, tile) + lane) * 8u + j;
}

void emul_merge_bytes(const uint32_t *sb, uint32_t *st) {
    st[0] += (sb[0] & 0xFFu) | ((sb[0] & 0xFF00u) << 8);
    st[1] += ((sb[0] >> 16) & 0xFFu) | ((sb[0] >> 24) << 16);
    st[2] += (sb[1] & 0xFFu) | ((sb[1] & 0xFF00u) << 8);
    st[3] += ((sb[1] >> 16) & 0xFFu) | ((sb[1] >> 24) << 16);
}

void emul_transpose64(const unsigned long long *in, unsigned long long *out) {
    unsigned long long x[64], y[64];
    for (int l = 0; l < 64; l++) x[l] = in[l];
    for (int s = 32; s >= 1; s >>= 1) {
        const unsigned long long m = s == 32 ? 0x00000000FFFFFFFFull : s == 16 ? 0x0000FFFF0000FFFFull : s == 8 ? 0x00FF00FF00FF00FFull
                                   : s == 4 ? 0x0F0F0F0F0F0F0F0Full : s == 2 ? 0x3333333333333333ull : 0x5555555555555555ull;
        for (int l = 0; l < 64; l++) y[l] = x[l ^ s];
        for (int l = 0; l < 64; l++) x[l] = (l & s) ? (((y[l] >> s) & m) | (x[l] & ~m)) : ((x[l] & m) | ((y[l] & m) << s));
    }
    for (int l = 0; l < 64; l++) out[l] = x[l];
}

uint32_t emul_finalise_rows(uint32_t n, uint32_t D, const uint8_t *k, const uint32_t *depth, const uint32_t *size, double n_total, uint32_t *rank,
                            double *local) {
    const uint32_t kw = (D + 3u) / 4u;
    std::vector<uint32_t> words((size_t)n * kw, 0u);
    for (uint32_t r = 0; r < n; r++)
        for (uint32_t w = 0; w < kw; w++) {
            uint32_t v = 0;
            for (uint32_t b = 0; b < 4u; b++) {
                const uint32_t d = 4u * w + b;
                v |= (uint32_t)(d < depth[r] && d < D ? k[(size_t)r * D + d] : 0u) << (8u * b);
            }
            words[(size_t)r * kw + w] = fin_be32(v);
// ... 417 lines not shown
```

### raxtax_amd/csrc/rtx_hit_common.hpp

```cpp
#pragma once

#include <hip/hip_runtime.h>

#include "rtx_kernels.hpp"
#include "rtx_math.hpp"
#include "rtx_wave.hpp"

namespace rtx {

__device__ __forceinline__ void wave_lds_sync() {
    __builtin_amdgcn_fence(__ATOMIC_ACQ_REL, "wavefront");
    __builtin_amdgcn_wave_barrier();
}

typedef uint32_t u32x4_t __attribute__((ext_vector_type(4)));

__device__ __forceinline__ __amdgpu_buffer_rsrc_t tile_rsrc(const uint32_t *bitmap, uint32_t n_rows1, uint32_t tile) {
    const char *base = reinterpret_cast<const char *>(bitmap) + (size_t)tile * n_rows1 * 1024u;
    return __builtin_amdgcn_make_buffer_rsrc(const_cast<char *>(base), 0, n_rows1 * 1024u, 0x00027000);
}

__device__ __forceinline__ void load8v_at(uint4 (&buf)[8], __amdgpu_buffer_rsrc_t rsrc, uint32_t voff, uint32_t idv, int o) {
#pragma unroll
    for (int j = 0; j < 8; j++) {
// ... 99 lines not shown
    const uint32_t ng = n8 / NB, nt = n8 - ng * NB;
    uint32_t idv = list[lane];
    uint4 buf[NB][8];
#pragma unroll
    for (int b = 0; b < NB; b++) load8v_at(buf[b], rsrc, voff, idv, b * 8);
    for (uint32_t g = 0; g < ng; g++) {
        const uint32_t idn = list[(g + 1) * GR + lane];
        uint4 ca[NB], cb[NB];
#pragma unroll
        for (int b = 0; b < NB; b++) {
            ca[b] = tree8<NP>(pa, buf[b]);
            cb[b] = tree8<NP>(pb, buf[b]);
            load8v_at(buf[b], rsrc, voff, idn, b * 8);
        }
        {
            const uint4 c4a = csa_plane<NP, 3>(pa, ca[0], ca[1]);
            const uint4 c4b = NB == 3 ? half_plane<NP, 3>(pa, ca[2]) : csa_plane<NP, 3>(pa, ca[2], ca[NB - 1]);
            ripple4<NP, 5>(pa, csa_plane<NP, 4>(pa, c4a, c4b));
        }
        {
            const uint4 c4a = csa_plane<NP, 3>(pb, cb[0], cb[1]);
            const uint4 c4b = NB == 3 ? half_plane<NP, 3>(pb, cb[2]) : csa_plane<NP, 3>(pb, cb[2], cb[NB - 1]);
            ripple4<NP, 5>(pb, csa_plane<NP, 4>(pb, c4a, c4b));
        }
        idv = idn;
    }
#pragma unroll
    for (int b = 0; b < NB - 1; b++)
        if ((uint32_t)b < nt) {
            ripple4<NP, 3>(pa, tree8<NP>(pa, buf[b]));
            ripple4<NP, 3>(pb, tree8<NP>(pb, buf[b]));
        }
}

constexpr int kSparseIt = (kSegMaxSparseRows + 63) / 64, kSparseV = kSegSlotEntries / 8;

__device__ __forceinline__ void sparse_prefetch(const HitParams &p, uint32_t lane, uint32_t ns, const uint32_t *sid_src,
                                                uint4 (&pre)[kSparseIt][kSparseV]) {
    uint32_t sid[kSparseIt];
#pragma unroll
    for (int it = 0; it < kSparseIt; it++) sid[it] = (uint32_t)it * 64u + lane < ns ? sid_src[(uint32_t)it * 64u + lane] : 0xFFFFFFFFu;
#pragma unroll
    for (int it = 0; it < kSparseIt; it++)
#pragma unroll
        for (int i = 0; i < kSparseV; i++) {
            const uint32_t pw = seg_pad(2u * lane) | (seg_pad(2u * lane + 1u) << 16);
            pre[it][i] = make_uint4(pw, pw, pw, pw);
            if (sid[it] != 0xFFFFFFFFu) pre[it][i] = reinterpret_cast<const uint4 *>(p.segslots + (size_t)sid[it] * kSegSlotEntries)[i];
        }
}

__device__ __forceinline__ uint32_t pk_max_u16(uint32_t a, uint32_t b) {
    typedef unsigned short u16x2 __attribute__((ext_vector_type(2)));
    u16x2 x, y;
    __builtin_memcpy(&x, &a, 4);
    __builtin_memcpy(&y, &b, 4);
    const u16x2 m = __builtin_elementwise_max(x, y);
    uint32_t r;
    __builtin_memcpy(&r, &m, 4);
    return r;
}

template <int NP, bool kPacked, bool kPrefetch, bool kFullTile, bool kPreLoaded, bool kGlobalHist = false>
__device__ __forceinline__ void hit_epilogue_x(const HitParams &p, uint32_t (&pl)[4][NP], uint32_t q, uint32_t tile, uint32_t lane,
                                               uint32_t t, bool active, uint32_t *hist_lds, uint32_t *cnt8, uint32_t ns,
                                               const uint32_t *srows, uint4 (&pre)[kSparseIt][kSparseV], uint32_t h_thr) {
// ... 462 lines not shown
__device__ __forceinline__ void bounds_epilogue(const HitParams &p, uint32_t (&pl)[4][NP], uint32_t q, uint32_t utile, uint32_t lane) {
    static_assert(kPruneShift == 6, "128 blocks per tile of the database = one group of 8 per lane of a DPP row");
    typedef unsigned short u16x2 __attribute__((ext_vector_type(2)));
    auto pkmax = [](uint32_t a, uint32_t b) -> uint32_t {
        u16x2 x, y;
        __builtin_memcpy(&x, &a, 4);
        __builtin_memcpy(&y, &b, 4);
        const u16x2 m = __builtin_elementwise_max(x, y);
        uint32_t r;
        __builtin_memcpy(&r, &m, 4);
        return r;
    };
    uint32_t best = 0;
    uint16_t *tub = p.bounds_tile_ub + (size_t)q * p.bounds_tile_stride;
#pragma unroll
    for (int w = 0; w < 4; w++) {
#pragma unroll
        for (int g2 = 0; g2 < 4; g2++) {
            const uint32_t gi = (uint32_t)(w * 4 + g2);
            uint32_t lo0, hi0, lo1, hi1;
            planes_unpack8<NP>(pl[w], g2, lo0, hi0, lo1, hi1);
            const uint32_t vx = (__builtin_amdgcn_perm(hi0, lo0, 0x05010400u) << 3) | 0x00060007u;
            const uint32_t vy = (__builtin_amdgcn_perm(hi0, lo0, 0x07030602u) << 3) | 0x00040005u;
            const uint32_t vz = (__builtin_amdgcn_perm(hi1, lo1, 0x05010400u) << 3) | 0x00020003u;
            const uint32_t vw = (__builtin_amdgcn_perm(hi1, lo1, 0x07030602u) << 3) | 0x00000001u;
            const uint32_t m2 = pkmax(pkmax(vx, vy), pkmax(vz, vw));
            const uint32_t m = (m2 & 0xFFFFu) > (m2 >> 16) ? (m2 & 0xFFFFu) : (m2 >> 16);
            const uint32_t blk0 = utile * 8192u + gi * 512u + lane * 8u;
            const uint32_t key = ((m >> 3) << 20) | (0xFFFFFu - blk0 - 7u + (m & 7u));
            best = key > best ? key : best;
            const uint32_t tmax = row16_max_u32(m >> 3);
            const uint32_t T = utile * 64u + gi * 4u + (lane >> 4);
            if ((lane & 15u) == 0u && T < p.bounds_ntiles) tub[T] = (uint16_t)tmax;
        }
    }
    best = wave_max_u32(best);
    if (lane == 0) atomicMax(&p.bounds_best[q], best);
}

template <int NP>
__device__ __forceinline__ void fine_epilogue(const HitParams &p, uint32_t (&pl)[4][NP], uint32_t q, uint32_t utile, uint32_t lane, uint32_t bits) {
    const uint32_t u = (uint32_t)__builtin_amdgcn_readfirstlane((int)p.prune_thr[q]);
    if (u == 0u || bits == 0u) return;
    uint32_t above = 0;
#pragma unroll
    for (int w = 0; w < 4; w++) {
        uint32_t gt = 0, eq = 0xFFFFFFFFu;
#pragma unroll
        for (int b = NP - 1; b >= 0; b--) {
            const uint32_t cb = (u >> b) & 1u ? 0xFFFFFFFFu : 0u;
            gt |= eq & pl[w][b] & ~cb;
            eq &= ~(pl[w][b] ^ cb);
        }
        if (__ballot((gt & 0xFFFFu) != 0u) != 0ull) above |= 1u << (2 * w);
        if (__ballot((gt >> 16) != 0u) != 0ull) above |= 2u << (2 * w);
    }
    uint32_t clear = bits & ~above;
    if (clear == 0u || lane != 0u) return;
    const uint32_t T0 = utile * 8u;
    uint32_t refs = 0, n = 0;
    for (uint32_t k = 0; k < 8u; k++)
        if ((clear >> k) & 1u) {
            const uint64_t lo = (uint64_t)(T0 + k) << 13, hi = lo + 8192u < p.fine_n_refs ? lo + 8192u : p.fine_n_refs;
            refs += (uint32_t)(hi - lo);
            n++;
        }
// ... 16 lines not shown
```

### raxtax_amd/csrc/rtx_hit_pair.hip

```cpp
#include <hip/hip_runtime.h>

#include <algorithm>
#include <type_traits>

#include "rtx_hit_common.hpp"

namespace rtx {

constexpr uint32_t kPairCap = kHitListCap;
constexpr uint32_t kPairListDw = kPairCap + 192u;
constexpr uint32_t kPairMaskWords = 64u;
constexpr uint32_t kPairSidDw = 2u * kSparseIt * 64u;
constexpr uint32_t kPairLdsBytes = 3u * kPairListDw * 4u + 2u * kPairMaskWords * 8u + 32u * 4u + kPairSidDw * 4u;
#ifndef RTX_PAIR_NB
#define RTX_PAIR_NB 3
#endif
#ifndef RTX_PAIR_WAVES
#define RTX_PAIR_WAVES 2
#endif
constexpr int kPairNB = RTX_PAIR_NB;

constexpr uint32_t kUnionMaxRows = 2048u;
__device__ __forceinline__ uint32_t lower_bound_u16(const uint16_t *l, uint32_t n, uint32_t key) {
    uint32_t lo = 0;
// ... 60 lines not shown
    static_assert(NB >= 2 && NB <= 4, "groups of 16, 24 or 32 rows");
    constexpr uint32_t GR = 8u * (uint32_t)NB;
    auto group = [&](auto load_tag, const uint32_t *src) {
        constexpr bool kLoad = decltype(load_tag)::value;
        uint32_t idn = 0;
        if constexpr (kLoad) idn = src[lane < GR ? lane : 0u];
        uint4 ca[NB], cb[NB];
#pragma unroll
        for (int b = 0; b < NB; b++) {
            if (MODE != 2) ca[b] = tree8<NP>(pa, buf[b]);
            if (MODE != 1) cb[b] = tree8<NP>(pb, buf[b]);
            if constexpr (kLoad) load8v_at(buf[b], rsrc, voff, idn, b * 8);
        }
        if (MODE != 2) {
            const uint4 c4a = csa_plane<NP, 3>(pa, ca[0], ca[1]);
            if constexpr (NB == 2) ripple4<NP, 4>(pa, c4a);
            else {
                const uint4 c4b = NB == 3 ? half_plane<NP, 3>(pa, ca[NB - 1]) : csa_plane<NP, 3>(pa, ca[NB - 2], ca[NB - 1]);
                ripple4<NP, 5>(pa, csa_plane<NP, 4>(pa, c4a, c4b));
            }
        }
        if (MODE != 1) {
            const uint4 c4a = csa_plane<NP, 3>(pb, cb[0], cb[1]);
            if constexpr (NB == 2) ripple4<NP, 4>(pb, c4a);
            else {
                const uint4 c4b = NB == 3 ? half_plane<NP, 3>(pb, cb[NB - 1]) : csa_plane<NP, 3>(pb, cb[NB - 2], cb[NB - 1]);
                ripple4<NP, 5>(pb, csa_plane<NP, 4>(pb, c4a, c4b));
            }
        }
    };
    const uint32_t n_loop = next ? ng : ng - 1u;
    for (uint32_t g = 0; g < n_loop; g++) group(std::true_type{}, g + 1 < ng ? list + (g + 1) * GR : next);
    if (!next) group(std::false_type{}, nullptr);
}

template <int NP, bool kPacked, int kBounds>
__device__ __forceinline__ void pair_tile_block(const HitParams &p, uint32_t *lds_dw, const uint32_t pair, const uint32_t tile, const uint32_t lane) {
    const uint32_t qa = pair * 2u, qb = qa + 1u;
    bool has_a = true, has_b = qb < p.nq;
    uint32_t fine_a = 0, fine_b = 0;
    if (kBounds == 2) {
        const uint32_t T0 = tile * 8u;
        const uint32_t *lw = p.live + (size_t)qa * p.live_words + (T0 >> 5);
        fine_a = (lw[0] >> (T0 & 31u)) & 0xFFu;
        fine_b = has_b ? (lw[p.live_words] >> (T0 & 31u)) & 0xFFu : 0u;
        has_a = fine_a != 0u;
        has_b = fine_b != 0u;
        if (!has_a && !has_b) return;
    }
    if (kBounds == 1 && p.bounds_heavy) {
        has_a = p.bounds_heavy[qa] != 0u;
        has_b = has_b && p.bounds_heavy[qb] != 0u;
        if (!has_a && !has_b) return;
    }
    if (!kBounds && p.live) {
        const uint32_t *lw = p.live + (size_t)qa * p.live_words + (tile >> 5);
        has_a = (lw[0] >> (tile & 31u)) & 1u;
        has_b = has_b && ((lw[p.live_words] >> (tile & 31u)) & 1u);
        if (!has_a && !has_b) return;
    }
    uint32_t *l_both = lds_dw, *l_a = lds_dw + kPairListDw, *l_b = lds_dw + 2u * kPairListDw;
    unsigned long long *m_a = reinterpret_cast<unsigned long long *>(lds_dw + 3u * kPairListDw), *m_b = m_a + kPairMaskWords;
    constexpr bool kLookAhead = NP > 10;
    uint32_t *l_zero = reinterpret_cast<uint32_t *>(m_b + kPairMaskWords);
    if (kLookAhead && lane < 32u) l_zero[lane] = p.zero_row << 10;
    uint32_t *l_sid = l_zero + 32;
// ... 117 lines not shown
    }
    uint32_t *hist_lds = lds_dw;
    uint32_t *cnt8 = lds_dw + (NP > 10 ? 2048u : 1024u);
    uint4 pre_a[kSparseIt][kSparseV], pre_b[kSparseIt][kSparseV];
    auto thr_of = [&](uint32_t q) -> uint32_t { return p.prune_thr ? (uint32_t)__builtin_amdgcn_readfirstlane((int)p.prune_thr[q]) : 0u; };
    if (ns_a) sparse_prefetch(p, lane, ns_a, l_sid, pre_a);
    if (ns_b) sparse_prefetch(p, lane, ns_b, l_sid + kSparseIt * 64u, pre_b);
    if (has_a) {
        const uint32_t ka = rec_slot_of(p, qa, tile, lane);
        if (ka != 0xFFFFFFFFu) rec_epilogue<NP>(p, pa, qa, tile, lane, p.t[qa], active, hist_lds, cnt8, ns_a, pre_a, thr_of(qa), ka, p.rec.stride);
        else hit_epilogue_x<NP, kPacked, true, true, true>(p, pa, qa, tile, lane, p.t[qa], active, hist_lds, cnt8, ns_a, srows_a, pre_a, thr_of(qa));
    }
    if (has_b) {
        wave_lds_sync();
        const uint32_t kb = rec_slot_of(p, qb, tile, lane);
        if (kb != 0xFFFFFFFFu) rec_epilogue<NP>(p, pb, qb, tile, lane, p.t[qb], active, hist_lds, cnt8, ns_b, pre_b, thr_of(qb), kb, p.rec.stride);
        else hit_epilogue_x<NP, kPacked, true, true, true>(p, pb, qb, tile, lane, p.t[qb], active, hist_lds, cnt8, ns_b, srows_b, pre_b, thr_of(qb));
    }
}

template <int NP, bool kPacked, int kBounds, bool kItems>
__global__ __launch_bounds__(64, RTX_PAIR_WAVES) void hit_count_pair_kernel(HitParams p) {
    extern __shared__ uint32_t lds_dw[];
    const uint32_t lane = threadIdx.x;
    if (kItems) {
        const uint32_t n_items = (uint32_t)__builtin_amdgcn_readfirstlane((int)p.n_items[0]), g8 = gridDim.x >> 3, x = blockIdx.x & 7u;
        const uint32_t e8 = (n_items + 7u) >> 3, first = x * e8;
        const uint32_t end = first + e8 < n_items ? first + e8 : n_items;
        uint32_t j = first + (blockIdx.x >> 3);
        while (j < end) {
            const uint32_t item = (uint32_t)__builtin_amdgcn_readfirstlane((int)p.items[j]);
            uint32_t lane_v = lane;
            asm volatile("" : "+v"(lane_v));
            pair_tile_block<NP, kPacked, kBounds>(p, lds_dw, item / p.ntiles, item % p.ntiles, lane_v);
            wave_lds_sync();
            if (e8 <= g8) break;
            uint32_t nxt = 0;
            if (lane_v == 0u) nxt = atomicAdd(&p.n_items[1u + x], 1u);
            j = first + g8 + (uint32_t)__builtin_amdgcn_readfirstlane((int)nxt);
        }
        return;
    }
    const uint32_t np8 = gridDim.x >> 3;
    const uint32_t pair = blockIdx.x < np8 * 8u ? (blockIdx.x & 7u) * np8 + (blockIdx.x >> 3) : blockIdx.x;
    pair_tile_block<NP, kPacked, kBounds>(p, lds_dw, pair, blockIdx.y, lane);
}

__global__ __launch_bounds__(1024) void live_items_kernel(const uint32_t *__restrict__ live, uint32_t live_words, uint32_t nq, uint32_t ntiles,
                                                          uint32_t *__restrict__ items, uint32_t *__restrict__ n_items,
                                                          unsigned long long *__restrict__ stats) {
    extern __shared__ uint32_t tl[];
    const uint32_t tid = threadIdx.x, lane = tid & 63u;
    const uint32_t np = (nq + 1u) / 2u, g0 = blockIdx.x * 1024u, pair = g0 + tid;
    for (uint32_t T = tid; T < ntiles; T += 1024) tl[T] = 0;
    __syncthreads();
    const uint32_t nw = (ntiles + 31u) >> 5;
    const bool valid = pair < np;
    const uint32_t *wa = live + (size_t)((valid ? pair : 0u) * 2u) * live_words;
    const bool hb = valid && pair * 2u + 1u < nq;
    if (valid)
        for (uint32_t w = 0; w < nw; w++) {
            uint32_t bits = wa[w] | (hb ? wa[live_words + w] : 0u);
            while (bits) {
                atomicAdd(&tl[w * 32u + (uint32_t)__builtin_ctz(bits)], 1u);
                bits &= bits - 1u;
            }
        }
// ... 18 lines not shown
        uint32_t bits = wa[w] | (hb ? wa[live_words + w] : 0u);
        while (bits) {
            const uint32_t tile = w * 32u + (uint32_t)__builtin_ctz(bits);
            bits &= bits - 1u;
            items[base + atomicAdd(&tl[tile], 1u)] = pair * ntiles + tile;
        }
    }
}

void launch_pair_union(hipStream_t s, const uint32_t *rows, const uint32_t *nrows, uint32_t rstride, uint32_t nq, uint2 *urec,
                       uint32_t *nu, uint32_t ustride) {
    hipLaunchKernelGGL(pair_union_kernel, dim3((nq + 1u) / 2u), dim3(64), 0, s, rows, nrows, rstride, nq, urec, nu, ustride);
}

#ifndef RTX_ITEM_GRID_HALVES
#define RTX_ITEM_GRID_HALVES 4
#endif
template <int NP>
static void launch_hit_count_pair_np(hipStream_t s, const HitParams &p, uint32_t nq, uint32_t ntiles) {
    static_assert(3u * kPairListDw >= 1024u + 2048u + 64u, "histogram (t <= 1023) and byte counters (+ pad words) alias the lists");
    static_assert(kPairLdsBytes >= (2048u + 2048u + 64u) * 4u, "eleven planes: histogram (t <= 2047) and byte counters alias the whole prologue");
    static_assert(kSegMaxSparseRows + 1 >= kSparseIt * 64, "the slot id lists are read without a bound");
    const uint32_t np = (nq + 1u) / 2u;
    const dim3 grid = p.items ? dim3((uint32_t)((std::min<uint64_t>((uint64_t)np * ntiles, std::max<uint64_t>((uint64_t)RTX_ITEM_GRID_HALVES * np / 2u, 2048ull)) + 7u) & ~7ull)) : dim3(np, ntiles);
    if (NP <= 10 && p.counts_lo) {
        if (p.items) hipLaunchKernelGGL((hit_count_pair_kernel<(NP <= 10 ? NP : 10), true, false, true>), grid, dim3(64), kPairLdsBytes, s, p);
        else hipLaunchKernelGGL((hit_count_pair_kernel<(NP <= 10 ? NP : 10), true, false, false>), grid, dim3(64), kPairLdsBytes, s, p);
    } else {
        if (p.items) hipLaunchKernelGGL((hit_count_pair_kernel<NP, false, false, true>), grid, dim3(64), kPairLdsBytes, s, p);
        else hipLaunchKernelGGL((hit_count_pair_kernel<NP, false, false, false>), grid, dim3(64), kPairLdsBytes, s, p);
    }
}
void launch_hit_count_pair(hipStream_t s, const HitParams &p, uint32_t nq, uint32_t ntiles, int planes) {
    if (planes <= 8) launch_hit_count_pair_np<8>(s, p, nq, ntiles);
    else if (planes <= 10) launch_hit_count_pair_np<10>(s, p, nq, ntiles);
    else launch_hit_count_pair_np<11>(s, p, nq, ntiles);
}

void launch_live_items(hipStream_t s, const uint32_t *live, uint32_t live_words, uint32_t nq, uint32_t ntiles, uint32_t *items, uint32_t *n_items,
                       unsigned long long *stats) {
    const uint32_t np = (nq + 1u) / 2u;
    hipLaunchKernelGGL(live_items_kernel, dim3((np + 1023u) / 1024u), dim3(1024), ((size_t)ntiles + 1u) * 4, s, live, live_words, nq, ntiles, items, n_items, stats);
}

void launch_hit_count_pair_bounds(hipStream_t s, const HitParams &p, uint32_t nq, uint32_t u_ntiles, int planes) {
    if (planes <= 8) hipLaunchKernelGGL((hit_count_pair_kernel<8, true, 1, false>), dim3((nq + 1u) / 2u, u_ntiles), dim3(64), kPairLdsBytes, s, p);
    else if (planes <= 10) hipLaunchKernelGGL((hit_count_pair_kernel<10, true, 1, false>), dim3((nq + 1u) / 2u, u_ntiles), dim3(64), kPairLdsBytes, s, p);
    else hipLaunchKernelGGL((hit_count_pair_kernel<11, false, 1, false>), dim3((nq + 1u) / 2u, u_ntiles), dim3(64), kPairLdsBytes, s, p);
}

void launch_hit_count_pair_bounds_items(hipStream_t s, const HitParams &p, uint32_t nq, uint32_t u_ntiles, int planes) {
    const uint32_t np = (nq + 1u) / 2u;
    const dim3 grid((uint32_t)((std::min<uint64_t>((uint64_t)np * u_ntiles, 4096ull) + 7u) & ~7ull));
    if (planes <= 8) hipLaunchKernelGGL((hit_count_pair_kernel<8, true, 1, true>), grid, dim3(64), kPairLdsBytes, s, p);
    else if (planes <= 10) hipLaunchKernelGGL((hit_count_pair_kernel<10, true, 1, true>), grid, dim3(64), kPairLdsBytes, s, p);
    else hipLaunchKernelGGL((hit_count_pair_kernel<11, false, 1, true>), grid, dim3(64), kPairLdsBytes, s, p);
}

__device__ __forceinline__ uint32_t fine_pair_mask(const uint32_t *live, uint32_t live_words, uint32_t pair, uint32_t nq, uint32_t U) {
    const uint32_t T0 = U * 8u;
    const uint32_t *wa = live + (size_t)(pair * 2u) * live_words + (T0 >> 5);
    uint32_t m = (wa[0] >> (T0 & 31u)) & 0xFFu;
    if (pair * 2u + 1u < nq) m |= (wa[live_words] >> (T0 & 31u)) & 0xFFu;
    return m;
}
__global__ __launch_bounds__(256) void fine_count_kernel(const uint32_t *__restrict__ live, uint32_t live_words, const uint32_t *__restrict__ pair_live,
// ... 58 lines not shown
```

### raxtax_amd/csrc/rtx_index.hpp

```cpp
#pragma once

#include <hip/hip_runtime.h>

#include <algorithm>
#include <cmath>
#include <cstdlib>
#include <cstring>
#include <thread>

#include "host_screen.hpp"
#include "rtx_internal.hpp"
#include "rtx_kernels.hpp"
#include "rtx_math.hpp"

using namespace rtx;

namespace rtxi {


constexpr uint32_t kEmptyRow = 0xFFFFFFFFu;
constexpr uint32_t kLnFactLen = 98320;
constexpr size_t kProbTableLdsLimit = 160 * 1024 - 512;

#define RTX_HIP(call)                                                                          \
// ... 94 lines not shown
    const double *ext_prefix = nullptr;
    uint32_t n_rows = 0;
    uint32_t stride_bytes = 0;
    uint64_t npad = 0;
    uint32_t ntiles = 0;
    DevBuf<uint32_t> d_bitmap, d_row_of, d_list_len;
    DevBuf<uint2> d_row_len;
    DevBuf<uint32_t> d_seginfo, d_seg_sbase, d_segcls;
    uint32_t cls_stride = 0;
    DevBuf<unsigned long long> d_seg_dbits, d_seg_sbits;
    uint32_t seg_blocks = 0;
    DevBuf<uint16_t> d_segslots;
    uint64_t n_seg_slots = 0;
    uint32_t seg_stride = 0;
    DevBuf<double> d_lnfact, d_inv;
    int prob_mode = 0;
    uint32_t tab_tmax = 0;
    DevBuf<double> d_tab_cmf, d_tab_ratio;
    DevBuf<uint64_t> d_tab_off;
    DevBuf<uint32_t> d_tab_moff;
    DevBuf<uint16_t> d_tab_ilo, d_tab_sat;
    FlatNodes nodes;
    std::vector<uint32_t> bnd;
    uint32_t n_bnd = 0;
    DevBuf<uint4> d_noderec;
    DevBuf<uint8_t> d_node_depth, d_node_sig0;
    DevBuf<uint32_t> d_node_begin;
    DevBuf<double> d_node_eb;
    uint32_t fin_D = 1;
    DevBuf<uint32_t> d_bnd_rank;
    DevBuf<uint8_t> d_bnd_bits;
    uint32_t dev_exact_opt = 1;
    uint32_t nearest_opt = 0;
    uint32_t identity_opt = 0;
    DevBuf<uint32_t> d_em_ref_grp;
    uint32_t strand_opt = 0;
    bool strand_used = false;
    uint64_t n_user = 0;
    uint32_t em_groups = 0, em_bits = 0;
    uint64_t em_hash_mask = ~0ull;
    DevBuf<uint2> d_em_table;
    DevBuf<uint64_t> d_em_rep_off;
    DevBuf<uint8_t> d_em_rep_bytes;
    DevBuf<uint32_t> d_em_goff, d_em_gids;
    std::vector<uint32_t> h_em_goff, h_em_gids;
    bool dev_exact_used = false;
    struct HostExact {
        std::vector<uint32_t> grp;
        std::vector<uint64_t> off;
        std::vector<uint32_t> ids;
        bool csr_valid = false, valid = false;
    } host_exact[2];
    uint64_t n_q = 0;
    bool uploaded = false, ran = false, synced = false;
    uint32_t last_flags = 0;
    uint32_t cluster = 1;
    uint32_t packed_opt = 1;
    uint32_t tile_skip = 1;
    uint32_t pair_opt = 1;
    uint32_t prune_opt = 1;
    uint32_t self_sample_opt = 1;
    bool prune_pays = true;
    double self_live = -1.0;
    bool pruning() const { return prune_opt != 0u && (prune_pays || self_sample_opt == 0u); }
    bool dbg_full = false;
    bool dbg_full_run = false;
    DevBuf<uint32_t> d_ubitmap;
    uint32_t u_stride_bytes = 0, u_ntiles = 0;
    uint64_t u_nblocks = 0;
    DevBuf<uint32_t> d_fbitmap;
    uint32_t f_stride_bytes = 0, f_ntiles = 0;
    uint64_t f_nblocks = 0;
    uint32_t fine_opt = 1;
    DevBuf<uint32_t> d_abitmap;
    DevBuf<uint8_t> d_bbitmap;
    uint32_t n_atiles = 0, n_btiles = 0;
    DevBuf<uint8_t> d_cbitmap;
    uint32_t two_level_opt = 1;
    uint32_t b2_delta[4] = {283u, 205u, 92u, 128u};
    bool two_level_used = false;
    uint32_t rec_seg_len = 1024;
    uint32_t diet_shift = 3;
    uint32_t rec_opt = 4;
    uint32_t rec_slots() const { return std::min<uint32_t>(rec_opt, kRecMaxSlots); }
    uint32_t overlap_opt = 1;
    uint32_t overlap_used = 0;
    hipStream_t stream2 = nullptr, stream3 = nullptr, hit_stream = nullptr;
    std::vector<hipEvent_t> ev_front, ev_back, ev_mid;
    DevBuf<unsigned long long> d_prune_stats;
    uint32_t shard_prune_opt = 0;
    uint32_t debug_taps = 0;
    DevBuf<uint32_t> d_prune_detail;
    uint32_t locator_opt = 1;
    DevBuf<uint32_t> d_loc_table;
    DevBuf<uint32_t> d_group_rows;
    uint32_t n_groups_run = 0;
    uint32_t groups_per_sub = 0;
    bool packs(int pl) const { return packed_opt && pl <= 10; }
    DevBuf<uint64_t> d_skey_in, d_skey_out;
    DevBuf<uint32_t> d_sidx;
    DevBuf<uint8_t> d_sort_tmp;
    DevBuf<uint8_t> d_bases;
    struct Inputs {
        DevBuf<uint8_t> d_packed;
        DevBuf<uint64_t> d_base_off, d_exact_off;
        DevBuf<uint32_t> d_exact_ids;
        PinBuf<uint8_t> h_packed;
        PinBuf<uint64_t> h_base_off, h_exact_off;
        PinBuf<uint32_t> h_exact_ids;
        uint64_t n_q = 0, total = 0, max_len = 0, n_exact = 0;
// ... 21 lines not shown
    hipEvent_t ev_activated = nullptr;
    uint64_t sum_query_bytes = 0;
    uint32_t sub_batch_req = 0;
    uint32_t min_subs = 4;
    uint64_t ws_key[14] = {0};
    bool ws_valid = false;
    struct BatchClass {
        uint64_t pos0 = 0, n = 0, max_len = 0;
        uint32_t tmax = 0, kstride = 0, rstride = 0, hstride = 0, sub_batch = 0, sb0 = 0, n_sub = 0;
        int planes = 10;
        bool use_tables = false, pair = false, prune = false, rec = false, huge = false, will_prune = false;
        bool side = false;
        bool diet = false;
        uint32_t cnt_rows = 0;
    } cls[5];
    uint32_t n_cls = 0;
    uint64_t key_lim[4] = {~0ull, ~0ull, ~0ull, ~0ull};
    struct SubPlan { uint64_t q0; uint32_t nq, cls; };
    std::vector<SubPlan> plan;
    uint32_t n_sub_total() const { return (uint32_t)plan.size(); }
    uint32_t sub_batch_max = 0;
    bool any_prune = false;
    DevBuf<double> d_prob_scratch;
    struct Scratch {
        DevBuf<uint16_t> d_kmers, d_counts, d_tilemax;
        DevBuf<uint32_t> d_rows, d_t, d_nrows, d_hist, d_order, d_srows, d_nsparse;
        DevBuf<unsigned long long> d_dmask;
        DevBuf<double> d_table_z, d_prefix;
        DevBuf<uint2> d_urec;
        DevBuf<uint32_t> d_nu;
        DevBuf<uint32_t> d_live, d_best_key;
        DevBuf<uint32_t> d_items;
        DevBuf<uint16_t> d_tile_ub, d_prune_thr, d_prune_i1;
        DevBuf<uint32_t> d_best;
        DevBuf<uint8_t> d_heavy;
        DevBuf<uint32_t> d_heavy_items;
        DevBuf<uint32_t> d_fine_items;
        DevBuf<uint16_t> d_rec_nslots, d_rec_slots;
        DevBuf<uint32_t> d_rec_cnt, d_rec;
        DevBuf<uint32_t> d_cnt_row, d_cnt_cursor;
        DevBuf<uint32_t> d_dense_q;
        template <class S, class F>
        static void each(S &s, F &&f) {
            f(s.d_kmers); f(s.d_counts); f(s.d_tilemax); f(s.d_rows); f(s.d_t); f(s.d_nrows); f(s.d_hist); f(s.d_order); f(s.d_srows); f(s.d_nsparse);
            f(s.d_dmask); f(s.d_table_z); f(s.d_prefix); f(s.d_urec); f(s.d_nu); f(s.d_live); f(s.d_best_key); f(s.d_items); f(s.d_tile_ub); f(s.d_prune_thr);
            f(s.d_prune_i1); f(s.d_best); f(s.d_heavy); f(s.d_heavy_items); f(s.d_fine_items); f(s.d_rec_nslots); f(s.d_rec_slots); f(s.d_rec_cnt); f(s.d_rec);
            f(s.d_cnt_row); f(s.d_cnt_cursor); f(s.d_dense_q);
        }
        void release_all() { each(*this, [](auto &b) { b.release(); }); }
        uint64_t bytes() const {
            uint64_t b = 0;
            each(*this, [&](const auto &buf) { b += buf.bytes(); });
            return b - d_cnt_row.bytes() - d_cnt_cursor.bytes();
        }
    } sc[4];
    bool staged = false;
    uint32_t last_set = 0;
    const BatchClass &last_cls() const { return cls[staged ? 0u : plan.back().cls]; }
    DevBuf<double> d_probs_dbg;
    DevBuf<uint16_t> d_counts_dbg;
    DevBuf<unsigned long long> d_sub_alloc;
    struct ResultSet {
        DevBuf<uint8_t> d_status;
        DevBuf<uint32_t> d_t_all, d_nrows_all, d_n_rows, d_flags, d_ndist;
        DevBuf<double> d_gs, d_z;
        DevBuf<unsigned long long> d_hq, d_row_start, d_cursor;
        DevBuf<DevRow> d_arena;
        uint64_t arena_cap = 0;
        uint64_t side_base = 0;
        PinBuf<unsigned long long> h_side_base;
        DevBuf<uint32_t> d_fin_t, d_fin_row_count, d_fin_lineage, d_fin_node, d_fin_depth;
        DevBuf<uint8_t> d_fin_status, d_fin_depth8, d_fin_hund;
        DevBuf<double> d_fin_gs, d_fin_local, d_fin_conf;
        DevBuf<unsigned long long> d_fin_row_begin, d_fin_cursor;
        uint64_t fin_cap = 0;
        DevBuf<uint32_t> d_perm, d_iperm;
        DevBuf<uint32_t> d_exact_grp;
        DevBuf<uint32_t> d_peak2, d_peak, d_sel_t, d_sel_row_count;
        DevBuf<uint8_t> d_strand, d_sel_status;
        DevBuf<double> d_sel_gs;
// ... 193 lines not shown
    uint32_t *items(uint32_t *p) const { return p; }
    uint32_t *count(uint32_t *p) const { return p + cap(); }
};
struct ItemsLayout : ItemList {
    using ItemList::ItemList;
    size_t total() const { return end() + np; }
    uint32_t *pair_live(uint32_t *p) const { return p + end(); }
};
struct FineItemsLayout : ItemList {
    using ItemList::ItemList;
    size_t total() const { return end() + ntiles; }
    uint32_t *cursors(uint32_t *p) const { return p + end(); }
};
struct HeavyItemsLayout : ItemList {
    using ItemList::ItemList;
    size_t total() const { return end(); }
};
struct LiveLayout {
    uint32_t ntiles;
    uint32_t words() const { return (ntiles + 31u) / 32u + 1u; }
    size_t total(size_t B) const { return (B + 1u) * words(); }
};

inline size_t counts_elems(const rtx_index *ix, int planes, size_t rows) { return ix->packs(planes) ? rows * ix->npad * 5 / 8 : rows * ix->npad; }

struct ScratchNeed {
    size_t kmers = 0, rows = 0, dmask = 0, counts = 0, hist = 0 , prefix = 0, urec = 0;
    size_t prob_scratch = 0;
    size_t nsparse = 0, srows = 0, t = 0, nrows = 0, order = 0, tilemax = 0, nu = 0;
    size_t tile_ub = 0, best_key = 0, prune_thr = 0, prune_i1 = 0, best = 0, live = 0, items = 0;
    size_t heavy = 0, heavy_items = 0, fine_items = 0;
    size_t rec_nslots = 0, rec_slots = 0, rec_cnt = 0, rec = 0, cnt_row = 0, cnt_cursor = 0;
    size_t dense_q = 0;
    ScratchNeed &set_queries(const rtx_index *ix, size_t B) {
        const size_t nt = ix->ntiles;
        t = nrows = order = best_key = prune_thr = prune_i1 = rec_nslots = cnt_row = B;
        nsparse = tilemax = tile_ub = B * nt;
        srows = B * nt * (kSegMaxSparseRows + 1);
        nu = (B + 1u) / 2u;
        best = B * kPruneBestWords;
        live = LiveLayout{ix->ntiles}.total(B);
        items = ItemsLayout(B, nt).total();
        heavy = B + 1u;
        heavy_items = HeavyItemsLayout(B, ix->u_ntiles).total();
        fine_items = FineItemsLayout(B, ix->f_ntiles).total();
        rec_slots = rec_cnt = B * kRecMaxSlots;
        rec = B * ix->rec_slots() * ix->rec_seg_len;
        cnt_cursor = 4;
        return *this;
    }
    void add_class(const rtx_index *ix, const rtx_index::BatchClass &kc, size_t B, size_t cnt_rows) {
        auto up = [](size_t &a, size_t v) { a = std::max(a, v); };
        up(kmers, B * kc.kstride);
        up(rows, B * kc.rstride);
        up(dmask, B * ix->ntiles * (kc.rstride / 64));
        up(counts, counts_elems(ix, kc.planes, cnt_rows));
        up(prefix, cnt_rows * ix->n_bnd_local);
        up(dense_q, cnt_rows);
        up(hist, B * kc.hstride);
        up(urec, ((B + 1u) / 2u) * 2u * kc.rstride);
        if (kc.huge) up(prob_scratch, B * ((prob_table_lds_bytes(kc.tmax) + 7) / 8));
    }
};

inline ScratchNeed scratch_set_need(const rtx_index *ix, uint32_t k) {
    ScratchNeed n;
    size_t b_max = 1;
    for (uint32_t c = 0; c < ix->n_cls; c++) {
        const rtx_index::BatchClass &kc = ix->cls[c];
        if (kc.side != (k == kSideSet)) continue;
        const size_t B = kc.sub_batch;
        b_max = std::max(b_max, B);
        const bool diet = kc.will_prune && ix->rec_opt != 0u && ix->n_refs == ix->n_total && ix->n_bnd_local == ix->n_bnd;
        n.add_class(ix, kc, B, diet ? diet_rows(ix, (uint32_t)B) : B);
    }
    return n.set_queries(ix, b_max);
}

inline uint64_t class_per_q(const rtx_index *ix, const rtx_index::BatchClass &k) {
// ... 11 lines not shown
```

### raxtax_amd/csrc/rtx_kernels.hpp

```cpp
#pragma once

#include <hip/hip_runtime.h>

#include <cstdint>

#include "raxtax_hip.h"
#include "rtx_math.hpp"

namespace rtx {

#ifndef RTX_NODE_TYPES_DEFINED
#define RTX_NODE_TYPES_DEFINED
enum NodeType : uint8_t { kInner = 0, kTaxon = 1, kSequence = 2 };
#endif

constexpr uint32_t kWalkMaxRows = 208;
constexpr uint32_t kSegPad = 8192;
__host__ __device__ inline uint32_t seg_pad(uint32_t i) { return kSegPad + ((i & 63u) << 2); }
constexpr uint32_t kKmerFewLive = 8;
constexpr uint32_t kHitListCap = 1024;

struct DevRow {
    uint32_t node;
    uint8_t k[RTX_MAX_DEPTH];
// ... 164 lines not shown
    const unsigned long long *seg_dbits, *seg_sbits;
    const uint32_t *seg_sbase;
    uint32_t seg_blocks;
    const uint32_t *segcls;
    uint32_t cls_stride;
    uint32_t *rows;
    uint32_t rstride;
    unsigned long long *dmask;
    uint32_t *srows;
    uint32_t *nsparse;
    uint32_t *t;
    uint32_t *nrows;
    unsigned long long *hq;
    uint32_t *t_all;
    uint32_t *nrows_all;
    uint32_t *hist;
    uint32_t hstride;
    uint32_t mode;
    const uint32_t *live;
    uint32_t live_words;
    uint32_t *zero[3];
    uint32_t zero_n[3];
};

constexpr uint32_t kRecMaxSlots = 16;
struct RecordRef {
    uint16_t *nslots;
    uint16_t *slots;
    uint32_t *cnt;
    uint32_t *rec;
    uint32_t stride;
    uint32_t seg_len;
    uint32_t *flags_out;
};

struct HitParams {
    const uint32_t *bitmap;
    uint32_t n_rows1;
    uint32_t stride_bytes;
    uint64_t n_refs;
    uint32_t ref_base;
    const uint32_t *rows;
    uint32_t rstride;
    const unsigned long long *dmask;
    const uint32_t *nrows;
    uint32_t zero_row;
    uint32_t lds_cnt8_off;
    const uint32_t *srows;
    const uint32_t *nsparse;
    const uint16_t *segslots;
    uint32_t ntiles;
    const uint32_t *t;
    uint16_t *counts;
    uint8_t *counts_lo;
    uint16_t *counts_hi;
    uint64_t npad;
    uint32_t *hist;
    uint32_t hstride;
    uint16_t *tile_max;
    uint32_t flags;
    uint64_t q0;
    const uint32_t *perm;
    ExactRef exact;
    uint32_t nq;
    uint32_t *group_rows;
    uint32_t group_base;
    const uint2 *pair_urec;
    const uint32_t *pair_nu;
    uint32_t pair_ustride;
    const uint32_t *live;
    uint32_t live_words;
    const uint16_t *prune_thr;
    const uint32_t *items;
    uint32_t *n_items;
    uint16_t *bounds_tile_ub;
    uint32_t bounds_tile_stride, bounds_ntiles;
    uint32_t *bounds_best;
    const uint8_t *bounds_heavy;
    uint64_t fine_n_refs;
    uint32_t fine_ref_ntiles;
    unsigned long long *fine_stats;
    RecordRef rec;
    const uint32_t *cnt_row;
};
struct Bounds2Params {
    const uint32_t *abitmap;
    const uint8_t *bbitmap;
    uint32_t n_rows1, n_atiles, ntiles, zero_row;
    const uint2 *pair_urec;
    const uint32_t *pair_nu;
    uint32_t pair_ustride, nq;
    const uint32_t *t;
    uint16_t *tile_ub;
    uint32_t tile_ub_stride;
    uint32_t *best_key;
    uint32_t delta_ct, delta_cm, delta_lo, delta_hi;
    uint8_t *heavy;
    uint32_t heavy_max;
    uint32_t *group_rows;
    uint32_t group_base;
};
struct HitParams;
void launch_bounds2(hipStream_t s, const Bounds2Params &p, uint32_t nq, int planes, const HitParams &hp, uint32_t u_ntiles, uint32_t *items);
constexpr uint32_t kTwoLevelMinTiles = 16;
void launch_bounds2_build(hipStream_t s, const uint32_t *ubitmap, uint32_t n_rows1, uint32_t u_ntiles, uint8_t *bbitmap, uint32_t *abitmap);
constexpr uint32_t kFineShift = 3;
constexpr uint32_t kFineMinLive = 4;
constexpr uint32_t kFineMinTiles = 16;

constexpr uint32_t kPruneStatCopies = 64;
#ifndef RTX_PRUNE_SHIFT
#define RTX_PRUNE_SHIFT 6
#endif
constexpr uint32_t kPruneShift = RTX_PRUNE_SHIFT;
static_assert(kPruneShift >= 3 && kPruneShift <= 6, "blocks of 8 .. 64 references");
constexpr uint32_t kPruneBestWords = 66;
struct PruneParams {
    const uint16_t *tile_ub;
    const uint32_t *best_key;
    uint32_t tile_ub_stride, ntiles, nq;
    uint64_t n_refs;
    uint64_t n_total;
    uint32_t ref_base;
    uint32_t phase;
    uint32_t *best;
    const uint2 *cbitmap;
    const uint32_t *bitmap;
    uint32_t n_rows1, stride_bytes;
    const uint32_t *rows;
    uint32_t rstride;
    const uint32_t *nrows, *t;
    uint32_t flags;
    uint64_t q0;
    const uint32_t *perm;
    ExactRef exact;
    const double *lnfact, *inv;
    uint32_t nlf;
    uint32_t *hist;
    uint32_t hstride;
    uint32_t *live;
    uint32_t live_words;
    uint32_t *pair_live;
    uint16_t *thr_out;
    uint16_t *i1_out;
    unsigned long long *stats;
    uint32_t *detail;
    RecordRef rec;
    uint32_t rec_max_slots;
    uint32_t *cnt_row;
    uint32_t *cnt_cursor;
    uint32_t cnt_cap;
    uint32_t *dense_q;
    uint32_t *flags_out;
};
constexpr uint32_t kPruneDetailWords = 72;
struct ProbTables;
void launch_prune(hipStream_t s, const PruneParams &p, const ProbTables &tb, uint32_t nq);
void launch_block_major_build(hipStream_t s, const uint32_t *bitmap, uint32_t n_rows1, uint32_t ntiles, uint32_t stride_bytes, uint8_t *cbitmap);

struct ProbTables {
    double *cmf;
    double *ratio;
    const uint64_t *off;
    const uint32_t *moff;
    uint16_t *ilo;
    uint16_t *sat;
    uint32_t tmax;
};


struct ProbParams {
    const uint32_t *order;
    const uint32_t *t;
    const uint32_t *hist;
    uint32_t hstride;
    uint32_t tmax;
    uint32_t n1max;
    const double *lnfact;
    uint64_t n_refs;
    uint64_t q0;
    double *table_z;
    double *z;
    double *gs;
    uint8_t *status;
    uint32_t *ndist;
    const uint16_t *prune_thr;
    const uint16_t *prune_i1;
    double *gscratch;
    uint32_t gstride;
};

// ... 149 lines not shown
```

### raxtax_amd/csrc/rtx_math.hpp

```cpp
#pragma once

#include <cmath>
#include <cstdint>

#if defined(__HIPCC__)
#define RTX_HD __host__ __device__ __forceinline__
#else
#define RTX_HD inline
#endif

namespace rtx {

constexpr uint32_t kSegSlotEntries = 16, kSegSparseMax = 16, kSegMaxSparseRows = 255;


RTX_HD uint32_t tile_lanes(uint32_t stride_bytes, uint32_t tile) {
    const uint32_t rem = stride_bytes - tile * 1024u;
    return rem >= 1024u ? 64u : rem >> 4;
}
RTX_HD size_t bitmap_word(uint32_t row, uint32_t word, uint32_t n_rows1) {
    return ((size_t)(word >> 8) * n_rows1 + row) * 256u + (word & 255u);
}
RTX_HD void ref_slot(uint32_t r, uint32_t stride_bytes, uint32_t &word, uint32_t &bit) {
    const uint32_t tile = r >> 13, rl = r & 8191u;
    const uint32_t L = tile_lanes(stride_bytes, tile);
    const uint32_t c = rl >> 3, l = c % L, g = c / L;
    word = tile * 256u + l * 4u + (g >> 2);
    bit = (g & 3u) * 8u + (rl & 7u);
}

RTX_HD void packed_count_pos(uint32_t rl, uint32_t &byte, uint32_t &hi_word, uint32_t &hi_shift) {
    byte = rl;
    hi_word = rl >> 3;
    hi_shift = (rl & 7u) * 2u;
}
RTX_HD uint32_t nearest_lane_base(uint32_t step, uint32_t lane, uint32_t per_lane) { return (step * 64u + lane) * per_lane; }
RTX_HD uint32_t nearest_match16(const uint32_t (&lo)[4], uint32_t hi2, uint32_t peak, uint32_t base, uint32_t in_tile) {
    uint32_t m = 0;
    for (uint32_t j = 0; j < 16u; j++) {
        uint32_t byte, hw, hs;
        packed_count_pos(base + j, byte, hw, hs);
        byte -= base;
        hw -= base >> 3;
        const uint32_t c = ((lo[byte >> 2] >> ((byte & 3u) * 8u)) & 0xFFu) | (((hi2 >> (hw * 16u + hs)) & 3u) << 8);
        if (c == peak && base + j < in_tile) m |= 1u << j;
    }
    return m;
}
RTX_HD uint32_t nearest_match8(const uint32_t (&w)[4], uint32_t peak, uint32_t base, uint32_t in_tile) {
    uint32_t m = 0;
    for (uint32_t j = 0; j < 8u; j++) {
        const uint32_t c = (w[j >> 1] >> ((j & 1u) * 16u)) & 0xFFFFu;
        if (c == peak && base + j < in_tile) m |= 1u << j;
    }
    return m;
}

struct IdentityBlock {
    uint64_t pv, mv;
    uint64_t plane[4];
// ... 1280 lines not shown
```

### raxtax_amd/csrc/rtx_prune.hip

```cpp
#include <hip/hip_runtime.h>

#include "rtx_kernels.hpp"
#include "rtx_math.hpp"
#include "rtx_wave.hpp"

namespace rtx {

static constexpr double kPruneLnEps = kPruneLnEpsHD;
static constexpr double kPruneHalfEps = kPruneHalfEpsHD;
#ifndef RTX_PRUNE_WAVES
#define RTX_PRUNE_WAVES 4
#endif
#ifndef RTX_PRUNE_TURNS
#define RTX_PRUNE_TURNS 16
#endif
static constexpr uint32_t kPruneWavesPerBlock = 4;

__device__ __forceinline__ uint32_t wave_max_u32p(uint32_t v) { return wave_max_u32(v); }

__global__ __launch_bounds__(64 * kPruneWavesPerBlock, RTX_PRUNE_WAVES) void prune_kernel(PruneParams p, ProbTables tb) {
    extern __shared__ double prune_lds[];
    for (uint32_t i = threadIdx.x; i < p.nlf; i += 64u * kPruneWavesPerBlock) prune_lds[i] = p.lnfact[i];
    __syncthreads();
    const uint32_t lane = threadIdx.x & 63u, pair = blockIdx.x * kPruneWavesPerBlock + (threadIdx.x >> 6);
// ... 344 lines not shown
    if (p.phase == 1u) return;
    __builtin_amdgcn_fence(__ATOMIC_ACQ_REL, "wavefront");
    __builtin_amdgcn_wave_barrier();
    unsigned long long dead_refs[2] = {0, 0};
    uint32_t n_live = 0, n_qlive = 0;
    uint32_t n_rec[2] = {0u, 0u};
    for (uint32_t T0 = 0; T0 < p.ntiles; T0 += 64) {
        const uint32_t T = T0 + lane;
        bool la = false, lb = false;
        if (T < p.ntiles) {
            la = thr[0] == 0u || (uint32_t)ub_lds[T] > thr[0];
            lb = has_b && (thr[1] == 0u || (uint32_t)ub_lds[p.ntiles + T] > thr[1]);
        }
        const unsigned long long ba = __ballot(la), bb2 = __ballot(lb);
        if (lane == 0) {
            uint32_t *wa = p.live + (size_t)(pair * 2u) * p.live_words, *wb = wa + p.live_words;
            wa[T0 >> 5] = (uint32_t)ba;
            if ((T0 >> 5) + 1u < p.live_words) wa[(T0 >> 5) + 1u] = (uint32_t)(ba >> 32);
            if (has_b) {
                wb[T0 >> 5] = (uint32_t)bb2;
                if ((T0 >> 5) + 1u < p.live_words) wb[(T0 >> 5) + 1u] = (uint32_t)(bb2 >> 32);
            }
        }
        if (T < p.ntiles) {
            const uint64_t lo = (uint64_t)T * 8192u, hi = lo + 8192u < p.n_refs ? lo + 8192u : p.n_refs;
            if (!la) dead_refs[0] += hi - lo;
            if (!lb) dead_refs[1] += hi - lo;
        }
        if (p.rec.nslots) {
            const unsigned long long lt = (1ull << lane) - 1ull;
            const uint32_t ka = n_rec[0] + (uint32_t)__popcll(ba & lt), kb = n_rec[1] + (uint32_t)__popcll(bb2 & lt);
            if (la && ka < kRecMaxSlots) p.rec.slots[(size_t)(pair * 2u) * kRecMaxSlots + ka] = (uint16_t)T;
            if (lb && kb < kRecMaxSlots) p.rec.slots[(size_t)(pair * 2u + 1u) * kRecMaxSlots + kb] = (uint16_t)T;
            n_rec[0] += (uint32_t)__popcll(ba);
            n_rec[1] += (uint32_t)__popcll(bb2);
        }
        n_live += (uint32_t)__popcll(ba | bb2);
        n_qlive += (uint32_t)__popcll(ba) + (uint32_t)__popcll(bb2);
    }
    if (p.rec.nslots) {
        const uint32_t cap = p.rec_max_slots < kRecMaxSlots ? p.rec_max_slots : kRecMaxSlots;
        const bool ra = thr[0] != 0u && n_rec[0] != 0u && n_rec[0] <= cap, rb = has_b && thr[1] != 0u && n_rec[1] != 0u && n_rec[1] <= cap;
        if (lane < kRecMaxSlots) {
            p.rec.cnt[(size_t)(pair * 2u) * kRecMaxSlots + lane] = 0u;
            if (has_b) p.rec.cnt[(size_t)(pair * 2u + 1u) * kRecMaxSlots + lane] = 0u;
        }
        if (lane == 0) {
            p.rec.nslots[pair * 2u] = (uint16_t)(ra ? n_rec[0] : 0u);
            if (has_b) p.rec.nslots[pair * 2u + 1u] = (uint16_t)(rb ? n_rec[1] : 0u);
            if (p.cnt_row) {
                auto row_for = [&](bool records, uint32_t q) -> uint32_t {
                    if (records) return 0xFFFFFFFFu;
                    const uint32_t r = atomicAdd(p.cnt_cursor, 1u);
                    if (r < p.cnt_cap) {
                        if (p.dense_q) p.dense_q[r] = q;
                        return r;
                    }
                    atomicOr(p.flags_out, 4u);
                    return 0xFFFFFFFFu;
                };
                p.cnt_row[pair * 2u] = row_for(ra, pair * 2u);
                if (has_b) p.cnt_row[pair * 2u + 1u] = row_for(rb, pair * 2u + 1u);
            }
        }
    }
#pragma unroll
// ... 2 lines not shown
        p.hist[(size_t)(pair * 2u) * p.hstride] = (uint32_t)dead_refs[0];
        if (has_b) p.hist[(size_t)(pair * 2u + 1u) * p.hstride] = (uint32_t)dead_refs[1];
    }
    if (lane == 0 && p.pair_live) p.pair_live[pair] = n_live;
    st[7] = n_qlive;
    if (p.stats) {
        st[0] = n_live; st[1] = 1ull;
        unsigned long long mine = 0;
#pragma unroll
        for (int k = 0; k < 8; k++) mine = lane == (uint32_t)k ? st[k] : mine;
        if (lane < 8u && mine) atomicAdd(&p.stats[(size_t)(pair & (kPruneStatCopies - 1u)) * 8u + lane], mine);
    }
}

__global__ __launch_bounds__(256) void block_major_build_kernel(const uint32_t *__restrict__ bitmap, uint32_t n_rows1, uint32_t stride_bytes,
                                                                uint8_t *__restrict__ cbitmap) {
    const uint32_t row = blockIdx.x, tile = blockIdx.y, word = threadIdx.x;
    const uint32_t v = bitmap[((size_t)tile * n_rows1 + row) * 256u + word];
    if (v == 0u) return;
    const uint32_t l = word >> 2, wi = word & 3u, L = tile_lanes(stride_bytes, tile);
    if (l >= L) return;
#pragma unroll
    for (uint32_t k = 0; k < 4u; k++) {
        const uint32_t byte = (v >> (8u * k)) & 0xFFu;
        if (byte == 0u) continue;
        const uint32_t ref0 = tile * 8192u + ((wi * 4u + k) * L + l) * 8u;
        cbitmap[((size_t)(ref0 >> 6) * n_rows1 + row) * 8u + ((ref0 & 63u) >> 3)] = (uint8_t)byte;
    }
}
void launch_block_major_build(hipStream_t s, const uint32_t *bitmap, uint32_t n_rows1, uint32_t ntiles, uint32_t stride_bytes, uint8_t *cbitmap) {
    hipLaunchKernelGGL(block_major_build_kernel, dim3(n_rows1, ntiles), dim3(256), 0, s, bitmap, n_rows1, stride_bytes, cbitmap);
}

void launch_prune(hipStream_t s, const PruneParams &p, const ProbTables &tb, uint32_t nq) {
    const uint32_t pairs = (nq + 1u) / 2u;
    hipLaunchKernelGGL(prune_kernel, dim3((pairs + kPruneWavesPerBlock - 1u) / kPruneWavesPerBlock), dim3(64 * kPruneWavesPerBlock),
                       (size_t)p.nlf * sizeof(double) + (size_t)kPruneWavesPerBlock * 2 * p.ntiles * sizeof(uint16_t), s, p, tb);
}

}
```

Baseline: 13.29 million.

## Add quarter-tile bounds and quarter-major bitmap to skip dead tile quarters in pair counting

```diff
diff --git a/include/raxtax_hip.h b/include/raxtax_hip.h
--- a/include/raxtax_hip.h
+++ b/include/raxtax_hip.h
@@ -132,6 +132,7 @@
 #define RTX_OPT_NEAREST 26
 #define RTX_NO_REF 0xFFFFFFFFu
 #define RTX_OPT_IDENTITY 28
+#define RTX_OPT_QUARTERS 29
 #define RTX_NO_DIST 0xFFFFFFFFu
 #define RTX_IDENTITY_MAX_QUERY 4096u
 #define RTX_OPT_DEREP 27
@@ -629,6 +630,8 @@
 int rtx_debug_prob_table(rtx_index *index, uint64_t query, double *table_over_z , double *z);
 int rtx_debug_probs(rtx_index *index, uint64_t query, double *probs );
 int rtx_debug_tile_bounds(rtx_index *index, uint64_t query, uint16_t *tile_ub );
+int rtx_debug_quarter_bounds(rtx_index *index, uint64_t query, uint16_t *quarter_ub );
+int rtx_debug_quarter_stats(rtx_index *index, uint64_t out[2]);
 int rtx_debug_order(rtx_index *index, uint32_t *perm );
 int rtx_batch_sub_batch(const rtx_index *index, uint32_t *sub_batch, uint32_t *n_sub_batches);
 int rtx_batch_last_sub_batch(const rtx_index *index, uint64_t *first, uint32_t *n);
diff --git a/raxtax_amd/_lib.py b/raxtax_amd/_lib.py
--- a/raxtax_amd/_lib.py
+++ b/raxtax_amd/_lib.py
@@ -19,6 +19,7 @@
 RTX_RAW_CONFIDENCE = 2
 RTX_TEXT_TSV = 4
 RTX_Q_OK, RTX_Q_NO_KMERS, RTX_Q_ALL_KMERS = 0, 1, 2
+RTX_OPT_QUARTERS = 29
 RTX_OPT_DEREP = 27
 RTX_DEFAULT_DEREP_HASH_MASK = 3
 RTX_DEFAULT_TALLY_HASH_MASK = 4
@@ -271,6 +272,8 @@
     "rtx_debug_probs": (C.c_int, [C.c_void_p, C.c_uint64, f64p]),
     "rtx_debug_order": (C.c_int, [C.c_void_p, u32p]),
     "rtx_debug_tile_bounds": (C.c_int, [C.c_void_p, C.c_uint64, u16p]),
+    "rtx_debug_quarter_bounds": (C.c_int, [C.c_void_p, C.c_uint64, u16p]),
+    "rtx_debug_quarter_stats": (C.c_int, [C.c_void_p, u64p]),
     "rtx_debug_prune_stats": (C.c_int, [C.c_void_p, u64p]),
     "rtx_debug_run_counts": (C.c_int, [C.c_void_p, C.c_uint64, u16p, u8p, u32p, u32p, u32p]),
     "rtx_debug_run_mode": (C.c_int, [C.c_void_p, C.c_uint64, u32p]),
diff --git a/raxtax_amd/api.py b/raxtax_amd/api.py
--- a/raxtax_amd/api.py
+++ b/raxtax_amd/api.py
@@ -319,7 +319,8 @@
                  debug_taps: bool = False, device_exact: Optional[bool] = None, fine_bounds: Optional[bool] = None,
                  records: Optional[int] = None, overlap: Optional[bool] = None, two_level: Optional[int] = None,
                  prune_self_sample: Optional[bool] = None, device_text: bool = False, strand: str = "plus",
-                 nearest: bool = False, derep: bool = False, identity: bool = False, primers=None, quality=None, chimera=None, tags=None, contaminants=None, tally=None):
+                 nearest: bool = False, derep: bool = False, identity: bool = False, primers=None, quality=None, chimera=None, tags=None, contaminants=None, tally=None,
+                 quarters: Optional[bool] = None):
         self._lib = _lib.load()
         self.tree = tree
         self._tally = None
@@ -389,10 +390,15 @@
             self.set_chimera(ChimeraParams() if chimera is True else chimera)
         if contaminants is not None:
             self.set_screen(*(contaminants if isinstance(contaminants, tuple) else (contaminants,)))
+        if quarters is not None:
+            self.set_quarters(quarters)
         if tally is not None:
             self.set_tally(tally)
         self._view = ResultView()
         self._keep = None
+
+    def set_quarters(self, on: bool) -> None:
+        check(self._lib.rtx_index_set_option(self._h, _lib.RTX_OPT_QUARTERS, int(bool(on))))
 
     def set_tally(self, tally) -> None:
         check(self._lib.rtx_index_set_tally(self._h, tally._h if tally is not None else None))
@@ -734,6 +740,16 @@
             res.append(dict(queries=int(out[4 * c]), longest=int(out[4 * c + 1]), sub_batch=int(out[4 * c + 2]), planes=f & 0xFF, tables=bool(f >> 8 & 1),
                             pair=bool(f >> 9 & 1), prune=bool(f >> 10 & 1), records=bool(f >> 11 & 1), global_memory_forms=bool(f >> 12 & 1)))
         return res
+
+    def debug_quarter_bounds(self, q: int) -> np.ndarray:
+        out = np.zeros(4 * ((self.n_refs + 8191) // 8192), dtype=np.uint16)
+        check(self._lib.rtx_debug_quarter_bounds(self._h, q, ptr(out, u16p)))
+        return out.reshape(-1, 4)
+
+    def debug_quarter_stats(self) -> dict:
+        out = np.zeros(2, dtype=np.uint64)
+        check(self._lib.rtx_debug_quarter_stats(self._h, ptr(out, u64p)))
+        return {"quarter_items": int(out[0]), "quarters_folded": int(out[1])}
 
     def debug_order(self, n_queries: int) -> np.ndarray:
         out = np.zeros(n_queries, dtype=np.uint32)
diff --git a/raxtax_amd/csrc/rtx_api_batch.hip b/raxtax_amd/csrc/rtx_api_batch.hip
--- a/raxtax_amd/csrc/rtx_api_batch.hip
+++ b/raxtax_amd/csrc/rtx_api_batch.hip
@@ -111,7 +111,7 @@
 static bool on_records_path(const rtx_index *ix, const rtx_index::BatchClass &k, const rtx_index::Scratch &sc) { return run_prunes(ix, k) && k.rec && sc.d_rec.p != nullptr; }
 static bool on_diet(const rtx_index *ix, const rtx_index::BatchClass &k, const rtx_index::Scratch &sc) { return on_records_path(ix, k, sc) && k.diet && sc.d_cnt_row.p != nullptr; }
 
-static RecordRef record_ref(const rtx_index *ix, const rtx_index::Scratch &sc, const rtx_index::ResultSet &r) { return RecordRef{sc.d_rec_nslots.p, sc.d_rec_slots.p, sc.d_rec_cnt.p, sc.d_rec.p, ix->rec_slots(), ix->rec_seg_len, r.d_flags.p}; }
+static RecordRef record_ref(const rtx_index *ix, const rtx_index::Scratch &sc, const rtx_index::ResultSet &r) { return RecordRef{sc.d_rec_nslots.p, sc.d_rec_slots.p, sc.d_rec_cnt.p, sc.d_rec.p, ix->rec_slots(), ix->rec_seg_len, r.d_flags.p, sc.d_rec_qmask.p}; }
 static ProbTables prob_tables(const rtx_index *ix) { return ProbTables{ix->d_tab_cmf.p, ix->d_tab_ratio.p, ix->d_tab_off.p, ix->d_tab_moff.p, ix->d_tab_ilo.p, ix->d_tab_sat.p, ix->tab_tmax}; }
 
 int enqueue_kmer(rtx_index *ix, const SubBatch &b, hipStream_t s) {
@@ -171,6 +171,10 @@
     return hp;
 }
 
+static bool quarter_scratch_ok(const rtx_index *ix, const rtx_index::Scratch &sc, uint32_t nq) {
+    return ix->d_qbitmap.p && sc.d_quarter_ub.p && sc.d_rec_qmask.p && sc.d_quarter_ub.n >= (size_t)nq * ix->ntiles * 4u && sc.d_rec_qmask.n >= (size_t)nq * kRecMaxSlots;
+}
+
 static HitParams bounds_params(const rtx_index *ix, const rtx_index::Scratch &sc, const HitParams &hp) {
     HitParams up = hp;
     up.bitmap = ix->d_ubitmap.p;
@@ -188,6 +192,7 @@
     up.bounds_tile_stride = ix->ntiles;
     up.bounds_ntiles = ix->ntiles;
     up.bounds_best = sc.d_best_key.p;
+    up.bounds_quarter_ub = quarter_scratch_ok(ix, sc, hp.nq) ? sc.d_quarter_ub.p : nullptr;
     up.flags = 0;
     up.group_base = hp.group_base + ix->n_groups_run;
     return up;
@@ -209,6 +214,7 @@
     bp.tile_ub = sc.d_tile_ub.p;
     bp.tile_ub_stride = ix->ntiles;
     bp.best_key = sc.d_best_key.p;
+    bp.quarter_ub = up.bounds_quarter_ub;
     bp.delta_ct = ix->b2_delta[0];
     bp.delta_cm = ix->b2_delta[1];
     bp.delta_lo = ix->b2_delta[2];
@@ -227,6 +233,7 @@
     pr.tile_ub = sc.d_tile_ub.p;
     pr.best_key = sc.d_best_key.p;
     pr.tile_ub_stride = ix->ntiles;
+    pr.quarter_ub = quarter_scratch_ok(ix, sc, b.nq) ? sc.d_quarter_ub.p : nullptr;
     pr.ntiles = ix->ntiles;
     pr.nq = b.nq;
     pr.n_refs = ix->n_refs;
@@ -320,6 +327,8 @@
         const bool records = part == 0 && on_records_path(ix, k, sc), diet = part == 0 && on_diet(ix, k, sc);
         const RecordRef rr = record_ref(ix, sc, r);
         if (records) { pr.rec = rr; pr.rec_max_slots = rr.stride; }
+        const bool quarters = records && k.pair && quarter_scratch_ok(ix, sc, b.nq);
+        if (!quarters) pr.rec.qmask = nullptr;
         if (k.diet && !diet) { set_error("internal: the counts buffer is on its diet without the records path"); return RTX_ERR_STATE; }
         if (diet) {
             pr.cnt_row = sc.d_cnt_row.p;
@@ -341,6 +350,11 @@
         hp.live_words = pr.live_words;
         hp.prune_thr = sc.d_prune_thr.p;
         if (records) hp.rec = rr;
+        if (!quarters) hp.rec.qmask = nullptr;
+        if (quarters && ix->quarters_opt) {
+            hp.qbitmap = ix->d_qbitmap.p;
+            hp.quarter_stats = ix->d_prune_stats.p ? ix->d_prune_stats.p + 2 * kPruneStatCopies * 8 : nullptr;
+        }
         if (k.pair) {
             const ItemsLayout items(b.nq, ix->ntiles);
             launch_live_items(s, sc.d_live.p, pr.live_words, b.nq, ix->ntiles, items.items(sc.d_items.p), items.count(sc.d_items.p),
@@ -1189,6 +1203,7 @@
             if (sc.d_rec_nslots.alloc(n.rec_nslots) || sc.d_rec_slots.alloc(n.rec_slots) || sc.d_rec_cnt.alloc(n.rec_cnt) ||
                 sc.d_rec.alloc(n.rec) || sc.d_cnt_row.alloc(n.cnt_row) || sc.d_cnt_cursor.alloc(n.cnt_cursor) || sc.d_dense_q.alloc(n.dense_q))
                 sc.d_rec.release();
+            else if (ix->d_qbitmap.p && (sc.d_quarter_ub.alloc(n.quarter_ub) || sc.d_rec_qmask.alloc(n.rec_qmask))) { sc.d_quarter_ub.release(); sc.d_rec_qmask.release(); }
         }
     }
     return RTX_OK;
diff --git a/raxtax_amd/csrc/rtx_api_debug.hip b/raxtax_amd/csrc/rtx_api_debug.hip
--- a/raxtax_amd/csrc/rtx_api_debug.hip
+++ b/raxtax_amd/csrc/rtx_api_debug.hip
@@ -352,6 +352,31 @@
     rtx_index::Scratch &sc = ix->sc[ix->last_set];
     if (!ix->last_cls().prune || sc.d_tile_ub.n < (size_t)(slot + 1) * ix->ntiles) { set_error("rtx_debug_tile_bounds: the last run did not prune"); return RTX_ERR_STATE; }
     RTX_HIP(hipMemcpy(tile_ub, sc.d_tile_ub.p + (size_t)slot * ix->ntiles, (size_t)ix->ntiles * 2, hipMemcpyDeviceToHost));
+    return RTX_OK;
+}
+
+int rtx_debug_quarter_bounds(rtx_index *ix, uint64_t query, uint16_t *quarter_ub) {
+    uint32_t slot;
+    int rc = debug_slot_as_run(ix, query, &slot);
+    if (rc) return rc;
+    if (!quarter_ub) { set_error("null argument"); return RTX_ERR_INVALID; }
+    rtx_index::Scratch &sc = ix->sc[ix->last_set];
+    if (!ix->last_cls().prune || !sc.d_quarter_ub.p || sc.d_quarter_ub.n < (size_t)(slot + 1) * ix->ntiles * 4u) { set_error("rtx_debug_quarter_bounds: the last run did not prune, or the handle keeps no quarter bounds"); return RTX_ERR_STATE; }
+    RTX_HIP(hipMemcpy(quarter_ub, sc.d_quarter_ub.p + (size_t)slot * ix->ntiles * 4u, (size_t)ix->ntiles * 8, hipMemcpyDeviceToHost));
+    return RTX_OK;
+}
+
+int rtx_debug_quarter_stats(rtx_index *ix, uint64_t *out) {
+    if (!ix || !out) { set_error("null argument"); return RTX_ERR_INVALID; }
+    out[0] = out[1] = 0;
+    if (!ix->any_prune || !ix->d_prune_stats.p) return RTX_OK;
+    RTX_HIP(hipStreamSynchronize(ix->stream));
+    unsigned long long h[kPruneStatCopies * 8];
+    RTX_HIP(hipMemcpy(h, ix->d_prune_stats.p + 2 * kPruneStatCopies * 8, sizeof(h), hipMemcpyDeviceToHost));
+    for (uint32_t c = 0; c < kPruneStatCopies; c++) {
+        out[0] += h[c * 8 + 3];
+        out[1] += h[c * 8 + 4];
+    }
     return RTX_OK;
 }
 
diff --git a/raxtax_amd/csrc/rtx_api_index.hip b/raxtax_amd/csrc/rtx_api_index.hip
--- a/raxtax_amd/csrc/rtx_api_index.hip
+++ b/raxtax_amd/csrc/rtx_api_index.hip
@@ -175,6 +175,7 @@
 static bool prepare_union_bitmap(rtx_index *ix);
 static bool prepare_fine_bitmap(rtx_index *ix);
 static void build_two_level(rtx_index *ix);
+static void build_quarter_major(rtx_index *ix);
 
 static uint64_t g_em_hash_mask = ~0ull;
 static uint64_t em_hash_bytes(const uint8_t *s, uint64_t len) {
@@ -414,6 +415,7 @@
         }
     }
     if ((rc = build_segments(ix))) return fail(rc);
+    build_quarter_major(ix);
     *out = ix;
     return RTX_OK;
 }
@@ -477,6 +479,23 @@
         if (e == hipSuccess) e = hipStreamSynchronize(ix->stream);
     }
     if (e != hipSuccess) { (void)hipGetLastError(); ix->d_cbitmap.release(); }
+}
+
+static void build_quarter_major(rtx_index *ix) {
+    if (!ix->d_ubitmap.p || !ix->d_bitmap.p || ix->n_refs != ix->n_total) return;
+    const size_t rows1 = (size_t)ix->n_rows + 1;
+    if (rows1 * 1024u > 0xFFFFFFFFull) return;
+    const size_t qwords = (size_t)ix->ntiles * 4u * rows1 * 64u;
+    size_t free_b = 0, total_b = 0;
+    if (hipMemGetInfo(&free_b, &total_b) != hipSuccess || qwords * 4u > free_b / 4 || qwords * 4u > total_b / 16 || ix->d_qbitmap.alloc(qwords)) {
+        (void)hipGetLastError();
+        ix->d_qbitmap.release();
+        return;
+    }
+    launch_quarter_major_build(ix->stream, ix->d_bitmap.p, (uint32_t)rows1, ix->ntiles, ix->d_qbitmap.p);
+    hipError_t e = hipGetLastError();
+    if (e == hipSuccess) e = hipStreamSynchronize(ix->stream);
+    if (e != hipSuccess) { (void)hipGetLastError(); ix->d_qbitmap.release(); }
 }
 
 static void build_locator(rtx_index *ix, const uint8_t *d_seq, const uint64_t *d_off, uint64_t n_refs) {
@@ -550,6 +569,7 @@
         launch_ref_bitmap_set(ix->stream, d_seq.p, d_off.p, n_refs, ix->d_row_of.p, ix->d_fbitmap.p, ix->f_stride_bytes / 4, nr + 1, kFineShift);
         if (hipStreamSynchronize(ix->stream) != hipSuccess) { (void)hipGetLastError(); ix->d_fbitmap.release(); }
     }
+    build_quarter_major(ix);
     *out = ix;
     if (!g_from_tree) (void)rtx_index_self_sample(ix, seq_bytes, seq_off, n_refs, 0, nullptr);
     return RTX_OK;
@@ -660,7 +680,7 @@
 uint64_t rtx_index_num_refs(const rtx_index *index) { return index ? index->n_total : 0; }
 uint64_t rtx_index_device_bytes(const rtx_index *index) {
     if (!index) return 0;
-    return index->d_seg_dbits.n * 8 + index->d_seg_sbits.n * 8 + index->d_seg_sbase.n * 4 + index->d_seginfo.n * 4 + index->d_segcls.n * 4 + index->d_segslots.n * 2 + index->d_bitmap.n * 4 + index->d_row_of.n * 4 + index->d_row_len.n * 8 + index->d_list_len.n * 4 + index->d_loc_table.n * 4 + index->d_ubitmap.n * 4 + index->d_fbitmap.n * 4 + index->d_abitmap.n * 4 + index->d_bbitmap.n + index->d_cbitmap.n + index->d_em_table.n * 8 + index->d_em_rep_off.n * 8 + index->d_em_rep_bytes.n + index->d_em_goff.n * 4 + index->d_em_gids.n * 4 + index->d_lnfact.n * 8 +
+    return index->d_seg_dbits.n * 8 + index->d_seg_sbits.n * 8 + index->d_seg_sbase.n * 4 + index->d_seginfo.n * 4 + index->d_segcls.n * 4 + index->d_segslots.n * 2 + index->d_bitmap.n * 4 + index->d_row_of.n * 4 + index->d_row_len.n * 8 + index->d_list_len.n * 4 + index->d_loc_table.n * 4 + index->d_ubitmap.n * 4 + index->d_fbitmap.n * 4 + index->d_abitmap.n * 4 + index->d_bbitmap.n + index->d_cbitmap.n + index->d_qbitmap.n * 4 + index->d_em_table.n * 8 + index->d_em_rep_off.n * 8 + index->d_em_rep_bytes.n + index->d_em_goff.n * 4 + index->d_em_gids.n * 4 + index->d_lnfact.n * 8 +
            index->d_noderec.n * 16 + index->d_bnd_bits.n + index->d_bnd_rank.n * 4;
 }
 uint64_t rtx_index_workspace_bytes(const rtx_index *ix) {
@@ -819,6 +839,10 @@
             index->ws_valid = false;
             index->identity_opt = (uint32_t)value;
             return RTX_OK;
+        case RTX_OPT_QUARTERS:
+            if (value > 1) break;
+            index->quarters_opt = (uint32_t)value;
+            return RTX_OK;
         case RTX_OPT_TWO_LEVEL_BOUNDS:
             index->two_level_opt = value ? 1u : 0u;
             if (value > 1) {
diff --git a/raxtax_amd/csrc/rtx_bounds2.hip b/raxtax_amd/csrc/rtx_bounds2.hip
--- a/raxtax_amd/csrc/rtx_bounds2.hip
+++ b/raxtax_amd/csrc/rtx_bounds2.hip
@@ -47,32 +47,25 @@
     if (!next) group(std::false_type{}, nullptr);
 }
 
+__device__ __forceinline__ uint32_t umax(uint32_t a, uint32_t b) { return a > b ? a : b; }
+
 template <int NP>
-__device__ __forceinline__ void reduce_rows(const uint32_t (&pl)[4][NP], uint32_t lane, uint32_t (&out)[NP]) {
-    const bool hi = (lane & 32u) != 0u, mid = (lane & 16u) != 0u;
-    uint32_t k0[NP], k1[NP];
-    {
-        uint32_t s0[NP], s1[NP];
-#pragma unroll
-        for (int p = 0; p < NP; p++) {
-            k0[p] = hi ? pl[2][p] : pl[0][p];
-            k1[p] = hi ? pl[3][p] : pl[1][p];
-            s0[p] = (uint32_t)__shfl_xor((int)(hi ? pl[0][p] : pl[2][p]), 32, 64);
-            s1[p] = (uint32_t)__shfl_xor((int)(hi ? pl[1][p] : pl[3][p]), 32, 64);
-        }
-        planes_add<NP>(k0, s0);
-        planes_add<NP>(k1, s1);
-    }
-    uint32_t s[NP];
-#pragma unroll
-    for (int p = 0; p < NP; p++) {
-        out[p] = mid ? k1[p] : k0[p];
-        s[p] = (uint32_t)__shfl_xor((int)(mid ? k0[p] : k1[p]), 16, 64);
-    }
-    planes_add<NP>(out, s);
-}
-
-__device__ __forceinline__ uint32_t umax(uint32_t a, uint32_t b) { return a > b ? a : b; }
+__device__ __forceinline__ uint2 quarter_max4(const uint32_t (&r)[NP]) {
+    uint32_t m[4];
+#pragma unroll
+    for (int k = 0; k < 4; k++) {
+        uint32_t cand = 0xFFu << (8 * k);
+        m[k] = 0;
+#pragma unroll
+        for (int pp = NP - 1; pp >= 0; pp--) {
+            const uint32_t x = cand & r[pp];
+            const bool nz = x != 0u;
+            cand = nz ? x : cand;
+            m[k] |= nz ? 1u << pp : 0u;
+        }
+    }
+    return make_uint2(m[0] | (m[1] << 16), m[2] | (m[3] << 16));
+}
 
 template <int NP>
 __global__ __launch_bounds__(64, 2) void bounds2_kernel(Bounds2Params p) {
@@ -168,6 +161,10 @@
         if (T < p.ntiles) {
             tub_a[T] = (uint16_t)ma;
             if (has_b) tub_b[T] = (uint16_t)mb;
+            if (p.quarter_ub) {
+                *reinterpret_cast<uint2 *>(p.quarter_ub + ((size_t)qa * p.tile_ub_stride + T) * 4u) = quarter_max4<NP>(ra);
+                if (has_b) *reinterpret_cast<uint2 *>(p.quarter_ub + ((size_t)qb * p.tile_ub_stride + T) * 4u) = quarter_max4<NP>(rb);
+            }
         }
         max_a = umax(max_a, ma);
         max_b = umax(max_b, mb);
@@ -227,7 +224,7 @@
             fold_level(std::integral_constant<int, 16>{}, std::integral_constant<int, 2>{}, std::integral_constant<int, 6>{}, rsrc, grp16, sub4 * 16u, for_a, for_b);
             const uint32_t T = bt * 4u + sub4;
             const bool real = T < p.ntiles;
-            auto finish = [&](const uint32_t (&pl)[4][NP], uint16_t *tub, uint32_t &best) {
+            auto finish = [&](const uint32_t (&pl)[4][NP], uint16_t *tub, uint32_t &best, uint32_t q) {
                 uint32_t r[NP];
                 reduce_rows<NP>(pl, lane, r);
 #pragma unroll
@@ -241,6 +238,7 @@
                 }
                 uint32_t c;
                 const uint32_t w = planes_max<NP>(r, c);
+                if (p.quarter_ub && real && (lane & 15u) < 4u) p.quarter_ub[((size_t)q * p.tile_ub_stride + T) * 4u + row4] = (uint16_t)w;
                 uint32_t key = (w << 8) | (127u - (row4 * 32u + (uint32_t)__builtin_ctz(c)));
                 key = umax(key, (uint32_t)__shfl_xor((int)key, 16, 64));
                 key = umax(key, (uint32_t)__shfl_xor((int)key, 32, 64));
@@ -248,8 +246,8 @@
                 const uint32_t g = real ? ((key >> 8) << 20) | (0xFFFFFu - (T * 128u + (127u - (key & 0xFFu)))) : 0u;
                 best = umax(best, wave_max_u32(g));
             };
-            if (for_a) finish(pa, tub_a, best_a);
-            if (for_b) finish(pb, tub_b, best_b);
+            if (for_a) finish(pa, tub_a, best_a, qa);
+            if (for_b) finish(pb, tub_b, best_b, qb);
         }
     }
     if (lane == 0u) {
diff --git a/raxtax_amd/csrc/rtx_emul.cpp b/raxtax_amd/csrc/rtx_emul.cpp
--- a/raxtax_amd/csrc/rtx_emul.cpp
+++ b/raxtax_amd/csrc/rtx_emul.cpp
@@ -592,6 +592,11 @@
 void emul_ref_slot(uint32_t r, uint32_t stride_bytes, uint32_t *word, uint32_t *bit) { ref_slot(r, stride_bytes, *word, *bit); }
 uint32_t emul_slot_ref(uint32_t tile, uint32_t lane, uint32_t g, uint32_t j, uint32_t stride_bytes) {
     return tile * 8192u + (g * tile_lanes(stride_bytes, tile) + lane) * 8u + j;
+}
+
+void emul_quarter_slot(uint32_t rl, uint32_t *quarter, uint32_t *word, uint32_t *bit) { quarter_slot(rl, *quarter, *word, *bit); }
+void emul_quarter_transpose(const uint32_t *row , uint32_t *out ) {
+    for (uint32_t w = 0; w < 256u; w++) out[(w & 3u) * 64u + quarter_word(w >> 2)] = row[w];
 }
 
 void emul_merge_bytes(const uint32_t *sb, uint32_t *st) {
diff --git a/raxtax_amd/csrc/rtx_hit_common.hpp b/raxtax_amd/csrc/rtx_hit_common.hpp
--- a/raxtax_amd/csrc/rtx_hit_common.hpp
+++ b/raxtax_amd/csrc/rtx_hit_common.hpp
@@ -155,6 +155,32 @@
             ripple4<NP, 3>(pb, tree8<NP>(pb, buf[b]));
         }
 }
+
+template <int NP>
+__device__ __forceinline__ void reduce_rows(const uint32_t (&pl)[4][NP], uint32_t lane, uint32_t (&out)[NP]) {
+    const bool hi = (lane & 32u) != 0u, mid = (lane & 16u) != 0u;
+    uint32_t k0[NP], k1[NP];
+    {
+        uint32_t s0[NP], s1[NP];
+#pragma unroll
+        for (int p = 0; p < NP; p++) {
+            k0[p] = hi ? pl[2][p] : pl[0][p];
+            k1[p] = hi ? pl[3][p] : pl[1][p];
+            s0[p] = (uint32_t)__shfl_xor((int)(hi ? pl[0][p] : pl[2][p]), 32, 64);
+            s1[p] = (uint32_t)__shfl_xor((int)(hi ? pl[1][p] : pl[3][p]), 32, 64);
+        }
+        planes_add<NP>(k0, s0);
+        planes_add<NP>(k1, s1);
+    }
+    uint32_t s[NP];
+#pragma unroll
+    for (int p = 0; p < NP; p++) {
+        out[p] = mid ? k1[p] : k0[p];
+        s[p] = (uint32_t)__shfl_xor((int)(mid ? k0[p] : k1[p]), 16, 64);
+    }
+    planes_add<NP>(out, s);
+}
+
 
 constexpr int kSparseIt = (kSegMaxSparseRows + 63) / 64, kSparseV = kSegSlotEntries / 8;
 
@@ -683,6 +709,13 @@
             const uint32_t tmax = row16_max_u32(m >> 3);
             const uint32_t T = utile * 64u + gi * 4u + (lane >> 4);
             if ((lane & 15u) == 0u && T < p.bounds_ntiles) tub[T] = (uint16_t)tmax;
+            if (p.bounds_quarter_ub) {
+                uint32_t qm = m >> 3, o;
+                o = (uint32_t)__builtin_amdgcn_update_dpp(0, (int)qm, 0xB1, 0xF, 0xF, true); qm = o > qm ? o : qm;
+                o = (uint32_t)__builtin_amdgcn_update_dpp(0, (int)qm, 0x4E, 0xF, 0xF, true); qm = o > qm ? o : qm;
+                if ((lane & 3u) == 0u && T < p.bounds_ntiles)
+                    p.bounds_quarter_ub[((size_t)q * p.bounds_tile_stride + T) * 4u + ((lane & 15u) >> 2)] = (uint16_t)qm;
+            }
         }
     }
     best = wave_max_u32(best);
diff --git a/raxtax_amd/csrc/rtx_hit_pair.hip b/raxtax_amd/csrc/rtx_hit_pair.hip
--- a/raxtax_amd/csrc/rtx_hit_pair.hip
+++ b/raxtax_amd/csrc/rtx_hit_pair.hip
@@ -116,6 +116,258 @@
     const uint32_t n_loop = next ? ng : ng - 1u;
     for (uint32_t g = 0; g < n_loop; g++) group(std::true_type{}, g + 1 < ng ? list + (g + 1) * GR : next);
     if (!next) group(std::false_type{}, nullptr);
+}
+
+#ifndef RTX_QUARTER_NB
+#define RTX_QUARTER_NB 2
+#endif
+constexpr int kQuarterNB = RTX_QUARTER_NB;
+constexpr uint32_t kQuarterDone = 0x80000000u;
+constexpr uint32_t kQuarterGroup = 32u * (uint32_t)kQuarterNB;
+static_assert(kPairListDw >= kPairCap + kQuarterGroup, "a list is padded to whole groups of the quarter mode");
+
+__device__ __forceinline__ void load_qunit(uint4 (&buf)[8], __amdgpu_buffer_rsrc_t rsrc, const uint32_t *unit, uint32_t grp, uint32_t col) {
+    const uint4 i0 = reinterpret_cast<const uint4 *>(unit)[grp * 2u], i1 = reinterpret_cast<const uint4 *>(unit)[grp * 2u + 1u];
+    const uint32_t id[8] = {i0.x, i0.y, i0.z, i0.w, i1.x, i1.y, i1.z, i1.w};
+#pragma unroll
+    for (int j = 0; j < 8; j++) {
+        const u32x4_t v = __builtin_amdgcn_raw_buffer_load_b128(rsrc, (id[j] >> 2) + col, 0, 0);
+        buf[j] = make_uint4(v.x, v.y, v.z, v.w);
+    }
+}
+
+template <int NP, int NB>
+__device__ __forceinline__ void fold_qseg(uint32_t (&pa)[4][NP], uint32_t (&pb)[4][NP], uint4 (&buf)[NB][8], const uint32_t *list, uint32_t ng,
+                                          const uint32_t *next, bool to_b, uint32_t grp, uint32_t col, __amdgpu_buffer_rsrc_t rsrc) {
+    static_assert(NB == 2 || NB == 3, "groups of 64 or 96 rows");
+    auto group = [&](uint32_t (&pl)[4][NP], auto load_tag, const uint32_t *src) {
+        constexpr bool kLoad = decltype(load_tag)::value;
+        uint4 c[NB];
+#pragma unroll
+        for (int b = 0; b < NB; b++) {
+            c[b] = tree8<NP>(pl, buf[b]);
+            if constexpr (kLoad) load_qunit(buf[b], rsrc, src + (uint32_t)b * 32u, grp, col);
+        }
+        const uint4 c4a = csa_plane<NP, 3>(pl, c[0], c[1]);
+        if constexpr (NB == 2) ripple4<NP, 4>(pl, c4a);
+        else ripple4<NP, 5>(pl, csa_plane<NP, 4>(pl, c4a, half_plane<NP, 3>(pl, c[NB - 1])));
+    };
+    const uint32_t n_loop = next ? ng : ng - 1u;
+    for (uint32_t g = 0; g < n_loop; g++) {
+        const uint32_t *src = g + 1 < ng ? list + (g + 1) * (32u * (uint32_t)NB) : next;
+        if (to_b) group(pb, std::true_type{}, src);
+        else group(pa, std::true_type{}, src);
+    }
+    if (!next) {
+        if (to_b) group(pb, std::false_type{}, nullptr);
+        else group(pa, std::false_type{}, nullptr);
+    }
+}
+
+__device__ __forceinline__ bool quarter_masks(const HitParams &p, uint32_t qa, uint32_t qb, bool has_a, bool has_b, uint32_t tile, uint32_t lane,
+                                              uint32_t &qm_a, uint32_t &qm_b) {
+    qm_a = qm_b = 0u;
+    if (!p.qbitmap || !p.rec.qmask || !p.live || (((uint64_t)tile + 1u) << 13) > p.n_refs) return false;
+    const uint32_t ka = has_a ? rec_slot_of(p, qa, tile, lane) : 0u, kb = has_b ? rec_slot_of(p, qb, tile, lane) : 0u;
+    if (ka == 0xFFFFFFFFu || kb == 0xFFFFFFFFu) return false;
+    qm_a = has_a ? (uint32_t)__builtin_amdgcn_readfirstlane((int)p.rec.qmask[(size_t)qa * kRecMaxSlots + ka]) & 15u : 0u;
+    qm_b = has_b ? (uint32_t)__builtin_amdgcn_readfirstlane((int)p.rec.qmask[(size_t)qb * kRecMaxSlots + kb]) & 15u : 0u;
+    return (!has_a || qm_a) && (!has_b || qm_b) && __popc(qm_a | qm_b) <= 2;
+}
+
+template <int NP>
+__device__ __forceinline__ bool quarter_tile_block(const HitParams &p, uint32_t *lds_dw, const uint32_t pair, const uint32_t tile, const uint32_t lane) {
+    const uint32_t qa = pair * 2u, qb = qa + 1u;
+    bool has_a, has_b = qb < p.nq;
+    {
+        const uint32_t *lw = p.live + (size_t)qa * p.live_words + (tile >> 5);
+        has_a = (lw[0] >> (tile & 31u)) & 1u;
+        has_b = has_b && ((lw[p.live_words] >> (tile & 31u)) & 1u);
+        if (!has_a && !has_b) return false;
+    }
+    uint32_t qm_a, qm_b;
+    if (!quarter_masks(p, qa, qb, has_a, has_b, tile, lane, qm_a, qm_b)) return false;
+    uint32_t *l_both = lds_dw, *l_a = lds_dw + kPairListDw, *l_b = lds_dw + 2u * kPairListDw;
+    unsigned long long *m_a = reinterpret_cast<unsigned long long *>(lds_dw + 3u * kPairListDw), *m_b = m_a + kPairMaskWords;
+    uint32_t *l_sid = reinterpret_cast<uint32_t *>(m_b + kPairMaskWords) + 32;
+    const uint32_t mwords = p.rstride >> 6;
+    const uint2 *urec = p.pair_urec + (size_t)pair * p.pair_ustride;
+    constexpr int kRecChunks = 8;
+    auto load_recs = [&](uint2 (&rec)[kRecChunks], uint32_t from) {
+#pragma unroll
+        for (int c = 0; c < kRecChunks; c++) {
+            const uint32_t i = from + (uint32_t)c * 64u + lane;
+            rec[c] = urec[i < p.pair_ustride ? i : p.pair_ustride - 1u];
+        }
+    };
+    uint2 rec[kRecChunks];
+    load_recs(rec, 0);
+    const uint32_t ns_a = has_a ? p.nsparse[(size_t)qa * p.ntiles + tile] : 0u, ns_b = has_b ? p.nsparse[(size_t)qb * p.ntiles + tile] : 0u;
+    {
+        const uint32_t *srows_a = p.srows + ((size_t)qa * p.ntiles + tile) * (kSegMaxSparseRows + 1);
+        const uint32_t *srows_b = p.srows + ((size_t)(has_b ? qb : qa) * p.ntiles + tile) * (kSegMaxSparseRows + 1);
+        const unsigned long long *dm_a = p.dmask + ((size_t)qa * p.ntiles + tile) * mwords;
+        const unsigned long long *dm_b = p.dmask + ((size_t)(has_b ? qb : qa) * p.ntiles + tile) * mwords;
+        uint32_t sa[kSparseIt], sb[kSparseIt];
+#pragma unroll
+        for (int it = 0; it < kSparseIt; it++) {
+            sa[it] = srows_a[(uint32_t)it * 64u + lane];
+            sb[it] = srows_b[(uint32_t)it * 64u + lane];
+        }
+        for (uint32_t i = lane; i < mwords; i += 64) {
+            m_a[i] = has_a ? dm_a[i] : 0ull;
+            m_b[i] = has_b ? dm_b[i] : 0ull;
+        }
+#pragma unroll
+        for (int it = 0; it < kSparseIt; it++) {
+            l_sid[(uint32_t)it * 64u + lane] = sa[it];
+            l_sid[(kSparseIt + (uint32_t)it) * 64u + lane] = sb[it];
+        }
+    }
+    wave_lds_sync();
+    const uint32_t n_u = p.pair_nu[pair];
+    const uint32_t zero_off = p.zero_row << 10;
+    const unsigned long long lt_mask = (1ull << lane) - 1ull;
+    const uint32_t grp = lane >> 4, col = (lane & 15u) * 16u;
+    constexpr int NB = kQuarterNB;
+    constexpr uint32_t GR = kQuarterGroup;
+    const uint32_t qm = qm_a | qm_b;
+    const bool two = (qm & (qm - 1u)) != 0u;
+    uint32_t ca[NP], cb[NP], oa[NP], ob[NP];
+#pragma unroll
+    for (int b = 0; b < NP; b++) { ca[b] = 0; cb[b] = 0; oa[b] = 0; ob[b] = 0; }
+    uint32_t pa[4][NP], pb[4][NP];
+    uint32_t qrows = 0, u0 = 0;
+    bool first_round = true;
+    while (u0 < n_u) {
+        uint32_t n_both = 0, n_a = 0, n_b = 0;
+        bool room = true;
+        while (room && u0 < n_u) {
+            if (u0) load_recs(rec, u0);
+#pragma unroll
+            for (int c = 0; c < kRecChunks; c++) {
+                if (u0 >= n_u) break;
+                if (n_both + 64u > kPairCap || n_a + 64u > kPairCap || n_b + 64u > kPairCap) { room = false; break; }
+                const bool in = u0 + lane < n_u;
+                const uint32_t pos_a = rec[c].y & 0xFFFFu, pos_b = rec[c].y >> 16;
+                const bool da = in && (rec[c].x & (1u << 30)) && ((m_a[pos_a >> 6] >> (pos_a & 63u)) & 1ull);
+                const bool db = in && (rec[c].x & (1u << 31)) && ((m_b[pos_b >> 6] >> (pos_b & 63u)) & 1ull);
+                const uint32_t row = (rec[c].x & 0x3FFFFFFFu) << 10;
+                const bool sh = da && db && first_round, oa_ = da && !sh, ob_ = db && !sh;
+                const unsigned long long bb = __ballot(sh), ba = __ballot(oa_), bo = __ballot(ob_);
+                if (sh) l_both[n_both + (uint32_t)__popcll(bb & lt_mask)] = row;
+                if (oa_) l_a[n_a + (uint32_t)__popcll(ba & lt_mask)] = row;
+                if (ob_) l_b[n_b + (uint32_t)__popcll(bo & lt_mask)] = row;
+                n_both += (uint32_t)__popcll(bb);
+                n_a += (uint32_t)__popcll(ba);
+                n_b += (uint32_t)__popcll(bo);
+                u0 += 64;
+            }
+        }
+        const uint32_t g_both = (n_both + GR - 1u) / GR, g_a = (n_a + GR - 1u) / GR, g_b = (n_b + GR - 1u) / GR;
+        for (uint32_t i = n_both + lane; i < g_both * GR; i += 64) l_both[i] = zero_off;
+        for (uint32_t i = n_a + lane; i < g_a * GR; i += 64) l_a[i] = zero_off;
+        for (uint32_t i = n_b + lane; i < g_b * GR; i += 64) l_b[i] = zero_off;
+        wave_lds_sync();
+        uint32_t todo = qm;
+#pragma nounroll
+        while (todo) {
+            const uint32_t k = (uint32_t)__builtin_ctz(todo);
+            todo &= todo - 1u;
+            const bool need_a = (qm_a >> k) & 1u, need_b = (qm_b >> k) & 1u;
+            if (two) {
+#pragma unroll
+                for (int b = 0; b < NP; b++) {
+                    const uint32_t xa = ca[b], xb = cb[b];
+                    ca[b] = oa[b]; cb[b] = ob[b];
+                    oa[b] = xa; ob[b] = xb;
+                }
+            }
+#pragma unroll
+            for (int w = 0; w < 4; w++)
+#pragma unroll
+                for (int b = 0; b < NP; b++) { pa[w][b] = 0; pb[w][b] = 0; }
+            const char *base = reinterpret_cast<const char *>(p.qbitmap) + ((size_t)tile * 4u + k) * p.n_rows1 * 256u;
+            const __amdgpu_buffer_rsrc_t rsrc = __builtin_amdgcn_make_buffer_rsrc(const_cast<char *>(base), 0, p.n_rows1 * 256u, 0x00027000);
+            const uint32_t ga = need_a ? g_a : 0u, gb = need_b ? g_b : 0u;
+            const uint32_t *first = g_both ? l_both : (ga ? l_a : (gb ? l_b : nullptr));
+            if (first) {
+                uint4 buf[NB][8];
+#pragma unroll
+                for (int b = 0; b < NB; b++) load_qunit(buf[b], rsrc, first + (uint32_t)b * 32u, grp, col);
+                const uint32_t *after_a = gb ? l_b : nullptr, *after_both = ga ? l_a : after_a;
+                if (g_both) {
+                    fold_qseg<NP, NB>(pa, pb, buf, l_both, g_both, after_both, !need_a, grp, col, rsrc);
+                    if (need_a && need_b) {
+#pragma unroll
+                        for (int w = 0; w < 4; w++)
+#pragma unroll
+                            for (int b = 0; b < NP; b++) pb[w][b] = pa[w][b];
+                    }
+                }
+                if (ga) fold_qseg<NP, NB>(pa, pb, buf, l_a, ga, after_a, false, grp, col, rsrc);
+                if (gb) fold_qseg<NP, NB>(pa, pb, buf, l_b, gb, nullptr, true, grp, col, rsrc);
+            }
+            if (need_a) {
+                uint32_t r[NP];
+                reduce_rows<NP>(pa, lane, r);
+                planes_add<NP>(ca, r);
+            }
+            if (need_b) {
+                uint32_t r[NP];
+                reduce_rows<NP>(pb, lane, r);
+                planes_add<NP>(cb, r);
+            }
+            qrows += n_both + (need_a ? n_a : 0u) + (need_b ? n_b : 0u);
+        }
+        wave_lds_sync();
+        first_round = false;
+    }
+    const uint32_t k_hi = 31u - (uint32_t)__builtin_clz(qm), k_lo = two ? (uint32_t)__builtin_ctz(qm) : 4u;
+#pragma unroll
+    for (int w = 0; w < 4; w++)
+#pragma unroll
+        for (int b = 0; b < NP; b++) {
+            pa[w][b] = (uint32_t)w == k_hi ? ca[b] : ((uint32_t)w == k_lo ? oa[b] : 0u);
+            pb[w][b] = (uint32_t)w == k_hi ? cb[b] : ((uint32_t)w == k_lo ? ob[b] : 0u);
+        }
+    if (lane == 0 && p.group_rows) atomicAdd(&p.group_rows[p.group_base + pair], (qrows + 3u) >> 2);
+    if (lane < 2u && p.quarter_stats)
+        atomicAdd(&p.quarter_stats[(size_t)(pair & (kPruneStatCopies - 1u)) * 8u + 3u + lane], lane ? (unsigned long long)__popc(qm) : 1ull);
+
+    uint32_t *hist_lds = lds_dw;
+    uint32_t *cnt8 = lds_dw + 1024u;
+    uint4 pre_a[kSparseIt][kSparseV], pre_b[kSparseIt][kSparseV];
+    auto thr_of = [&](uint32_t q) -> uint32_t { return (uint32_t)__builtin_amdgcn_readfirstlane((int)p.prune_thr[q]); };
+    if (ns_a) sparse_prefetch(p, lane, ns_a, l_sid, pre_a);
+    if (ns_b) sparse_prefetch(p, lane, ns_b, l_sid + kSparseIt * 64u, pre_b);
+    if (has_a) rec_epilogue<NP>(p, pa, qa, tile, lane, p.t[qa], true, hist_lds, cnt8, ns_a, pre_a, thr_of(qa), rec_slot_of(p, qa, tile, lane), p.rec.stride);
+    if (has_b) {
+        wave_lds_sync();
+        rec_epilogue<NP>(p, pb, qb, tile, lane, p.t[qb], true, hist_lds, cnt8, ns_b, pre_b, thr_of(qb), rec_slot_of(p, qb, tile, lane), p.rec.stride);
+    }
+    return true;
+}
+
+__global__ __launch_bounds__(64, RTX_PAIR_WAVES) void quarter_count_kernel(HitParams p) {
+    extern __shared__ uint32_t lds_dw[];
+    const uint32_t lane = threadIdx.x;
+    const uint32_t n_items = (uint32_t)__builtin_amdgcn_readfirstlane((int)p.n_items[0]), g8 = gridDim.x >> 3, x = blockIdx.x & 7u;
+    const uint32_t e8 = (n_items + 7u) >> 3, first = x * e8;
+    const uint32_t end = first + e8 < n_items ? first + e8 : n_items;
+    uint32_t j = first + (blockIdx.x >> 3);
+    while (j < end) {
+        const uint32_t item = (uint32_t)__builtin_amdgcn_readfirstlane((int)p.items[j]);
+        uint32_t lane_v = lane;
+        asm volatile("" : "+v"(lane_v));
+        const bool done = quarter_tile_block<10>(p, lds_dw, item / p.ntiles, item % p.ntiles, lane_v);
+        if (done && lane_v == 0u) const_cast<uint32_t *>(p.items)[j] = item | kQuarterDone;
+        wave_lds_sync();
+        if (e8 <= g8) break;
+        uint32_t nxt = 0;
+        if (lane_v == 0u) nxt = atomicAdd(&p.n_items[1u + x], 1u);
+        j = first + g8 + (uint32_t)__builtin_amdgcn_readfirstlane((int)nxt);
+    }
 }
 
 template <int NP, bool kPacked, int kBounds>
@@ -299,7 +551,7 @@
             const uint32_t item = (uint32_t)__builtin_amdgcn_readfirstlane((int)p.items[j]);
             uint32_t lane_v = lane;
             asm volatile("" : "+v"(lane_v));
-            pair_tile_block<NP, kPacked, kBounds>(p, lds_dw, item / p.ntiles, item % p.ntiles, lane_v);
+            if (!(item & kQuarterDone)) pair_tile_block<NP, kPacked, kBounds>(p, lds_dw, item / p.ntiles, item % p.ntiles, lane_v);
             wave_lds_sync();
             if (e8 <= g8) break;
             uint32_t nxt = 0;
@@ -384,6 +636,14 @@
     }
 }
 void launch_hit_count_pair(hipStream_t s, const HitParams &p, uint32_t nq, uint32_t ntiles, int planes) {
+    if (planes > 8 && planes <= 10 && p.qbitmap && p.items && p.rec.qmask && p.live && p.prune_thr && (uint64_t)((nq + 1u) / 2u) * ntiles < kQuarterDone) {
+        const uint32_t np = (nq + 1u) / 2u;
+        const dim3 grid((uint32_t)((std::min<uint64_t>((uint64_t)np * ntiles, std::max<uint64_t>((uint64_t)RTX_ITEM_GRID_HALVES * np / 2u, 2048ull)) + 7u) & ~7ull));
+        hipLaunchKernelGGL(quarter_count_kernel, grid, dim3(64), kPairLdsBytes, s, p);
+        (void)hipMemsetAsync(p.n_items + 1, 0, 8 * sizeof(uint32_t), s);
+        launch_hit_count_pair_np<10>(s, p, nq, ntiles);
+        return;
+    }
     if (planes <= 8) launch_hit_count_pair_np<8>(s, p, nq, ntiles);
     else if (planes <= 10) launch_hit_count_pair_np<10>(s, p, nq, ntiles);
     else launch_hit_count_pair_np<11>(s, p, nq, ntiles);
diff --git a/raxtax_amd/csrc/rtx_index.hpp b/raxtax_amd/csrc/rtx_index.hpp
--- a/raxtax_amd/csrc/rtx_index.hpp
+++ b/raxtax_amd/csrc/rtx_index.hpp
@@ -150,6 +150,7 @@
     DevBuf<uint8_t> d_bnd_bits;
     uint32_t dev_exact_opt = 1;
     uint32_t nearest_opt = 0;
+    uint32_t quarters_opt = 1;
     uint32_t identity_opt = 0;
     DevBuf<uint32_t> d_em_ref_grp;
     uint32_t strand_opt = 0;
@@ -194,6 +195,7 @@
     DevBuf<uint8_t> d_bbitmap;
     uint32_t n_atiles = 0, n_btiles = 0;
     DevBuf<uint8_t> d_cbitmap;
+    DevBuf<uint32_t> d_qbitmap;
     uint32_t two_level_opt = 1;
     uint32_t b2_delta[4] = {283u, 205u, 92u, 128u};
     bool two_level_used = false;
@@ -281,6 +283,8 @@
         DevBuf<uint32_t> d_live, d_best_key;
         DevBuf<uint32_t> d_items;
         DevBuf<uint16_t> d_tile_ub, d_prune_thr, d_prune_i1;
+        DevBuf<uint16_t> d_quarter_ub;
+        DevBuf<uint8_t> d_rec_qmask;
         DevBuf<uint32_t> d_best;
         DevBuf<uint8_t> d_heavy;
         DevBuf<uint32_t> d_heavy_items;
@@ -294,7 +298,7 @@
             f(s.d_kmers); f(s.d_counts); f(s.d_tilemax); f(s.d_rows); f(s.d_t); f(s.d_nrows); f(s.d_hist); f(s.d_order); f(s.d_srows); f(s.d_nsparse);
             f(s.d_dmask); f(s.d_table_z); f(s.d_prefix); f(s.d_urec); f(s.d_nu); f(s.d_live); f(s.d_best_key); f(s.d_items); f(s.d_tile_ub); f(s.d_prune_thr);
             f(s.d_prune_i1); f(s.d_best); f(s.d_heavy); f(s.d_heavy_items); f(s.d_fine_items); f(s.d_rec_nslots); f(s.d_rec_slots); f(s.d_rec_cnt); f(s.d_rec);
-            f(s.d_cnt_row); f(s.d_cnt_cursor); f(s.d_dense_q);
+            f(s.d_cnt_row); f(s.d_cnt_cursor); f(s.d_dense_q); f(s.d_quarter_ub); f(s.d_rec_qmask);
         }
         void release_all() { each(*this, [](auto &b) { b.release(); }); }
         uint64_t bytes() const {
@@ -554,6 +558,7 @@
     size_t heavy = 0, heavy_items = 0, fine_items = 0;
     size_t rec_nslots = 0, rec_slots = 0, rec_cnt = 0, rec = 0, cnt_row = 0, cnt_cursor = 0;
     size_t dense_q = 0;
+    size_t quarter_ub = 0, rec_qmask = 0;
     ScratchNeed &set_queries(const rtx_index *ix, size_t B) {
         const size_t nt = ix->ntiles;
         t = nrows = order = best_key = prune_thr = prune_i1 = rec_nslots = cnt_row = B;
@@ -566,7 +571,8 @@
         heavy = B + 1u;
         heavy_items = HeavyItemsLayout(B, ix->u_ntiles).total();
         fine_items = FineItemsLayout(B, ix->f_ntiles).total();
-        rec_slots = rec_cnt = B * kRecMaxSlots;
+        rec_slots = rec_cnt = rec_qmask = B * kRecMaxSlots;
+        quarter_ub = B * nt * 4u;
         rec = B * ix->rec_slots() * ix->rec_seg_len;
         cnt_cursor = 4;
         return *this;
diff --git a/raxtax_amd/csrc/rtx_kernels.hpp b/raxtax_amd/csrc/rtx_kernels.hpp
--- a/raxtax_amd/csrc/rtx_kernels.hpp
+++ b/raxtax_amd/csrc/rtx_kernels.hpp
@@ -220,6 +220,7 @@
     uint32_t stride;
     uint32_t seg_len;
     uint32_t *flags_out;
+    uint8_t *qmask;
 };
 
 struct HitParams {
@@ -270,6 +271,9 @@
     unsigned long long *fine_stats;
     RecordRef rec;
     const uint32_t *cnt_row;
+    const uint32_t *qbitmap;
+    unsigned long long *quarter_stats;
+    uint16_t *bounds_quarter_ub;
 };
 struct Bounds2Params {
     const uint32_t *abitmap;
@@ -281,6 +285,7 @@
     const uint32_t *t;
     uint16_t *tile_ub;
     uint32_t tile_ub_stride;
+    uint16_t *quarter_ub;
     uint32_t *best_key;
     uint32_t delta_ct, delta_cm, delta_lo, delta_hi;
     uint8_t *heavy;
@@ -307,6 +312,7 @@
     const uint16_t *tile_ub;
     const uint32_t *best_key;
     uint32_t tile_ub_stride, ntiles, nq;
+    const uint16_t *quarter_ub;
     uint64_t n_refs;
     uint64_t n_total;
     uint32_t ref_base;
@@ -345,6 +351,7 @@
 struct ProbTables;
 void launch_prune(hipStream_t s, const PruneParams &p, const ProbTables &tb, uint32_t nq);
 void launch_block_major_build(hipStream_t s, const uint32_t *bitmap, uint32_t n_rows1, uint32_t ntiles, uint32_t stride_bytes, uint8_t *cbitmap);
+void launch_quarter_major_build(hipStream_t s, const uint32_t *bitmap, uint32_t n_rows1, uint32_t ntiles, uint32_t *qbitmap);
 
 struct ProbTables {
     double *cmf;
diff --git a/raxtax_amd/csrc/rtx_math.hpp b/raxtax_amd/csrc/rtx_math.hpp
--- a/raxtax_amd/csrc/rtx_math.hpp
+++ b/raxtax_amd/csrc/rtx_math.hpp
@@ -26,6 +26,16 @@
     const uint32_t L = tile_lanes(stride_bytes, tile);
     const uint32_t c = rl >> 3, l = c % L, g = c / L;
     word = tile * 256u + l * 4u + (g >> 2);
+    bit = (g & 3u) * 8u + (rl & 7u);
+}
+RTX_HD uint32_t quarter_word(uint32_t lane) { return (lane & 15u) * 4u + (lane >> 4); }
+RTX_HD size_t quarter_bitmap_word(uint32_t tile, uint32_t quarter, uint32_t row, uint32_t lane, uint32_t n_rows1) {
+    return (((size_t)tile * 4u + quarter) * n_rows1 + row) * 64u + quarter_word(lane);
+}
+RTX_HD void quarter_slot(uint32_t rl, uint32_t &quarter, uint32_t &word, uint32_t &bit) {
+    const uint32_t c = rl >> 3, l = c & 63u, g = c >> 6;
+    quarter = g >> 2;
+    word = quarter_word(l);
     bit = (g & 3u) * 8u + (rl & 7u);
 }
 
diff --git a/raxtax_amd/csrc/rtx_prune.hip b/raxtax_amd/csrc/rtx_prune.hip
--- a/raxtax_amd/csrc/rtx_prune.hip
+++ b/raxtax_amd/csrc/rtx_prune.hip
@@ -400,6 +400,14 @@
             const uint32_t ka = n_rec[0] + (uint32_t)__popcll(ba & lt), kb = n_rec[1] + (uint32_t)__popcll(bb2 & lt);
             if (la && ka < kRecMaxSlots) p.rec.slots[(size_t)(pair * 2u) * kRecMaxSlots + ka] = (uint16_t)T;
             if (lb && kb < kRecMaxSlots) p.rec.slots[(size_t)(pair * 2u + 1u) * kRecMaxSlots + kb] = (uint16_t)T;
+            if (p.rec.qmask && p.quarter_ub) {
+                auto qmask_of = [&](uint32_t q, uint32_t u) -> uint8_t {
+                    const uint2 v = *reinterpret_cast<const uint2 *>(p.quarter_ub + ((size_t)q * p.tile_ub_stride + T) * 4u);
+                    return (uint8_t)(((v.x & 0xFFFFu) > u ? 1u : 0u) | ((v.x >> 16) > u ? 2u : 0u) | ((v.y & 0xFFFFu) > u ? 4u : 0u) | ((v.y >> 16) > u ? 8u : 0u));
+                };
+                if (la && ka < kRecMaxSlots) p.rec.qmask[(size_t)(pair * 2u) * kRecMaxSlots + ka] = qmask_of(pair * 2u, thr[0]);
+                if (lb && kb < kRecMaxSlots) p.rec.qmask[(size_t)(pair * 2u + 1u) * kRecMaxSlots + kb] = qmask_of(pair * 2u + 1u, thr[1]);
+            }
             n_rec[0] += (uint32_t)__popcll(ba);
             n_rec[1] += (uint32_t)__popcll(bb2);
         }
@@ -468,6 +476,14 @@
     hipLaunchKernelGGL(block_major_build_kernel, dim3(n_rows1, ntiles), dim3(256), 0, s, bitmap, n_rows1, stride_bytes, cbitmap);
 }
 
+__global__ __launch_bounds__(256) void quarter_major_build_kernel(const uint32_t *__restrict__ bitmap, uint32_t n_rows1, uint32_t *__restrict__ qbitmap) {
+    const uint32_t row = blockIdx.x, tile = blockIdx.y, word = threadIdx.x;
+    qbitmap[quarter_bitmap_word(tile, word & 3u, row, word >> 2, n_rows1)] = bitmap[((size_t)tile * n_rows1 + row) * 256u + word];
+}
+void launch_quarter_major_build(hipStream_t s, const uint32_t *bitmap, uint32_t n_rows1, uint32_t ntiles, uint32_t *qbitmap) {
+    hipLaunchKernelGGL(quarter_major_build_kernel, dim3(n_rows1, ntiles), dim3(256), 0, s, bitmap, n_rows1, qbitmap);
+}
+
 void launch_prune(hipStream_t s, const PruneParams &p, const ProbTables &tb, uint32_t nq) {
     const uint32_t pairs = (nq + 1u) / 2u;
     hipLaunchKernelGGL(prune_kernel, dim3((pairs + kPruneWavesPerBlock - 1u) / kPruneWavesPerBlock), dim3(64 * kPruneWavesPerBlock),
```

Result: slower. 12.80 million (-3.7%).
